# cvg/pixel-perfect-sfm

Measured on AMD Instinct MI355X. Metric: featuremetric residuals+Jacobians evaluated/sec (1M obs), higher is better.
Workload: dtype f32 horizontal / f64 vertical+normalisation on f16 patches; 1 GPU; BASELINE.json configs[2]: synthetic 200 cams / 200000 points / 1000000 obs featuremetric BA residual+Jacobian evaluation, 128-ch fp16 16x16 patches, SIMPLE_RADIAL, fused six-scalar Jacobian reduction; n_obs=1000000, channels=128, patch=16, obs_per_gpu=1000000, partition=none

## Files before the change

### include/pixsfm_hip.h

```cpp
#ifndef PIXSFM_HIP_H_
#define PIXSFM_HIP_H_

#include <stddef.h>
#include <stdint.h>

#ifdef __cplusplus
extern "C" {
#endif

#define PXR_KPAD 12
#define PXR_OBS_REC 8

enum { PXR_OK = 0, PXR_EINVAL = -1, PXR_EHIP = -2, PXR_ENOMEM = -3, PXR_EUNSUPPORTED = -4,
       PXR_ENUMERIC = -5 };
enum { PXR_F16 = 0, PXR_F32 = 1, PXR_F64 = 2, PXR_U8 = 3  };
enum { PXR_SIMPLE_PINHOLE = 0, PXR_PINHOLE = 1, PXR_SIMPLE_RADIAL = 2, PXR_RADIAL = 3,
       PXR_OPENCV = 4, PXR_OPENCV_FISHEYE = 5, PXR_FULL_OPENCV = 6, PXR_FOV = 7,
       PXR_SIMPLE_RADIAL_FISHEYE = 8, PXR_RADIAL_FISHEYE = 9, PXR_THIN_PRISM_FISHEYE = 10 };
enum { PXR_LOSS_TRIVIAL = 0, PXR_LOSS_CAUCHY = 1, PXR_LOSS_HUBER = 2, PXR_LOSS_SOFTL1 = 3 };

typedef struct pxr_ctx pxr_ctx;
typedef struct pxr_arena pxr_arena;

typedef struct {
  int32_t l2_normalize;
  int32_t use_float_simd;
  int32_t check_bounds;
} pxr_interp_cfg;

typedef struct {
  int32_t type;
  double a;
} pxr_loss;

int pxr_version(void);
const char* pxr_last_error(void);
int pxr_ctx_create(int device, void* stream, pxr_ctx** out);
int pxr_ctx_destroy(pxr_ctx* ctx);
int pxr_ctx_sync(pxr_ctx* ctx);
int pxr_malloc(pxr_ctx* ctx, size_t bytes, void** d_ptr);
int pxr_free(pxr_ctx* ctx, void* d_ptr);
int pxr_memcpy_h2d(pxr_ctx* ctx, void* d_dst, const void* h_src, size_t bytes);
int pxr_memcpy_d2h(pxr_ctx* ctx, void* h_dst, const void* d_src, size_t bytes);
int pxr_memset(pxr_ctx* ctx, void* d_dst, int value, size_t bytes);
int pxr_timer_start(pxr_ctx* ctx);
int pxr_timer_stop(pxr_ctx* ctx, double* ms);

int pxr_arena_create(pxr_ctx* ctx, int dtype, int C, int H, int W, int64_t n_patches,
                     void* d_data_or_null ,
                     pxr_arena** out);
int pxr_arena_destroy(pxr_arena* a);
int pxr_arena_upload(pxr_arena* a, int64_t first, int64_t count, const void* h_patches,
                     const int32_t* h_corners, const double* h_scales);
int pxr_arena_upload_gather(pxr_arena* a, int64_t first, int64_t count, const void* const* h_patch_ptrs,
                            const int32_t* h_corners, const double* h_scales);
int pxr_arena_extract(pxr_ctx* ctx, pxr_arena* a, int64_t first, int64_t n, const void* d_fmap,
                      int src_dtype, int h, int w, const double* d_keypoints, double image_w,
                      double image_h, int l2_normalize);
int pxr_dsift_dense(pxr_ctx* ctx, const void* d_image, int image_dtype, int h, int w, int spatial_bin_size, int rootsift,
                    double clipval, float* d_out);
int pxr_dsift_extract(pxr_ctx* ctx, pxr_arena* a, int64_t first, int64_t n, const void* d_image, int image_dtype, int h,
                      int w, int spatial_bin_size, int rootsift, double clipval, const double* d_keypoints, double image_w,
                      double image_h, int l2_normalize);
void* pxr_arena_data(pxr_arena* a);
int32_t* pxr_arena_corners(pxr_arena* a);
double* pxr_arena_scales(pxr_arena* a);
int64_t pxr_arena_size(pxr_arena* a);

typedef struct {
  int64_t n_obs;
  const int32_t* d_obs_image;
  const int32_t* d_obs_point;
  const int64_t* d_obs_patch;
  int32_t n_images;
  const int32_t* d_image_camera;
  const double* d_qvec;
  const double* d_tvec;
  int32_t n_cameras;
  const int32_t* d_cam_model;
  const double* d_cam_params;
  int64_t n_points;
  const double* d_xyz;
  const double* d_refs;
} pxr_ba_view;

int pxr_ba_eval(pxr_ctx* ctx, pxr_arena* arena, const pxr_ba_view* view,
                const pxr_interp_cfg* cfg, int with_jacobian, double* d_rec, double* d_r,
                double* d_gx, double* d_gy);

int pxr_ba_projection_jacobian(pxr_ctx* ctx, const pxr_ba_view* view, double* d_P);

int pxr_ba_cost(pxr_ctx* ctx, const double* d_rec, int64_t n_obs, const pxr_loss* loss,
                double* h_cost);


enum { PXR_TERM_CONVERGENCE = 0, PXR_TERM_NO_CONVERGENCE = 1, PXR_TERM_FAILURE = 2 };

typedef struct {
  int32_t max_iterations;
  double function_tolerance;
  double gradient_tolerance;
  double parameter_tolerance;
  double initial_radius;
  double max_radius;
  double min_radius;
  double min_relative_decrease;
  double min_lm_diagonal;
  double max_lm_diagonal;
  int32_t max_consecutive_invalid_steps;
  int32_t jacobi_scaling;
  int32_t use_inner_iterations;
  double inner_iteration_tolerance;
  int32_t linear_solver;
  int32_t max_linear_solver_iterations;
  double eta;
  double linear_r_tolerance;
} pxr_lm_options;
enum { PXR_LINEAR_AUTO = 0, PXR_LINEAR_DIRECT = 1, PXR_LINEAR_ITERATIVE = 2 };
#define PXR_MAX_IMAGES_DIRECT 1000

typedef struct {
  int32_t iterations;
  int32_t num_successful;
  int32_t termination;
  int32_t num_camera_unknowns;
  int64_t num_point_unknowns;
  double initial_cost, final_cost, final_radius;
  double total_ms;
  double setup_ms;
  int32_t linear_solver;
  int32_t collective_kib;
  int64_t linear_iterations;
  int32_t accumulation;
  int32_t initial_us;
} pxr_lm_summary;

typedef struct {
  int32_t iteration;
  int32_t step_is_valid;
  int32_t step_is_successful;
  double cost;
  double cost_change;
  double relative_decrease;
  double trust_region_radius;
  double step_norm;
} pxr_iteration_summary;
typedef int (*pxr_iteration_callback)(const pxr_iteration_summary* summary, void* user);
int pxr_set_iteration_callback(pxr_ctx* ctx, pxr_iteration_callback fn , void* user);

int pxr_set_deterministic(pxr_ctx* ctx, int on);
int pxr_get_deterministic(pxr_ctx* ctx);

int pxr_set_gram_cache(pxr_ctx* ctx, int on);
int pxr_get_gram_cache(pxr_ctx* ctx);
int pxr_ba_eval_gram(pxr_ctx* ctx, pxr_arena* arena, const pxr_ba_view* view, const pxr_interp_cfg* cfg, int reset,
                     double* d_rec, int32_t* h_rebuilt);

#define PXR_COMM_ID_BYTES 128
int pxr_comm_unique_id(void* h_id );
int pxr_comm_init(pxr_ctx* ctx, const void* h_id, int rank, int nranks);
int pxr_comm_destroy(pxr_ctx* ctx);
int pxr_comm_set_rank(pxr_ctx* ctx, int rank, int nranks);
int pxr_comm_rank(pxr_ctx* ctx, int* rank, int* nranks);
int pxr_comm_allreduce_sum(pxr_ctx* ctx, double* d_buf, int64_t count);
int pxr_comm_force(pxr_ctx* ctx, int on);
int pxr_comm_stats(pxr_ctx* ctx, int64_t* calls, int64_t* bytes, int reset);

typedef int (*pxr_allreduce_fn)(void* user, double* d_buf, int64_t count);

int pxr_ba_solve(pxr_ctx* ctx, pxr_arena* arena, const pxr_ba_view* view, const pxr_interp_cfg* cfg,
                 const pxr_loss* loss, const uint8_t* h_pose_const, const uint8_t* h_tvec_const_mask,
                 const uint16_t* h_cam_const_mask, const uint8_t* h_point_const,
                 const pxr_lm_options* options, pxr_allreduce_fn allreduce, void* allreduce_user,
                 pxr_lm_summary* summary);

int pxr_ba_geom_eval(pxr_ctx* ctx, const pxr_ba_view* view, const double* d_obs_xy, double* d_rec, double* d_res);

int pxr_ba_solve_geometric(pxr_ctx* ctx, const pxr_ba_view* view, const double* d_obs_xy, const pxr_loss* loss,
                           const uint8_t* h_pose_const, const uint8_t* h_tvec_const_mask,
                           const uint16_t* h_cam_const_mask, const uint8_t* h_point_const,
                           const pxr_lm_options* options, pxr_allreduce_fn allreduce, void* allreduce_user,
                           pxr_lm_summary* summary);

typedef struct {
  int64_t n_tracks;
  const int64_t* d_track_offsets;
  int64_t n_obs;
  const int32_t* d_obs_image;
  const double* d_obs_xy;
  int32_t n_images;
  const int32_t* d_image_camera;
  const double* d_qvec;
  const double* d_tvec;
  int32_t n_cameras;
  const int32_t* d_cam_model;
  const double* d_cam_params;
} pxr_tri_view;

typedef struct {
  double min_tri_angle;
  double max_angle_error;
  double max_reproj_error;
  int32_t min_track_len;
  int32_t max_hypotheses;
} pxr_tri_options;

int pxr_image_to_world(pxr_ctx* ctx, int64_t n, const int32_t* d_cam_index, int32_t n_cameras, const int32_t* d_cam_model,
                       const double* d_cam_params, const double* d_xy, double* d_uv, uint8_t* d_ok);

int pxr_triangulate_tracks(pxr_ctx* ctx, const pxr_tri_view* view, const pxr_tri_options* options, double* d_xyz,
                           int32_t* d_status, int32_t* d_n_inliers, uint8_t* d_obs_inlier, double* d_obs_err);
int pxr_triangulate_tracks_timed(pxr_ctx* ctx, const pxr_tri_view* view, const pxr_tri_options* options, double* d_xyz,
                                 int32_t* d_status, int32_t* d_n_inliers, uint8_t* d_obs_inlier, double* d_obs_err,
                                 double* h_kernel_ms);

int pxr_ba_compute_references(pxr_ctx* ctx, pxr_arena* arena, const pxr_ba_view* view,
                              const pxr_interp_cfg* cfg, const pxr_loss* loss, int iters,
                              double* d_refs_out, int64_t* d_ref_obs_out, double* d_robust_mean_out,
                              double* d_obs_desc_out );

int pxr_costmap_extract(pxr_ctx* ctx, pxr_arena* features, pxr_arena* costmaps, int64_t first_out, int64_t n,
                        const int64_t* d_patch, const int32_t* d_ref_index, const double* d_refs,
                        const pxr_loss* loss, int as_gradientfield, int apply_sqrt);

int pxr_costmap_extract_ex(pxr_ctx* ctx, pxr_arena* features, pxr_arena* costmaps, int64_t first_out, int64_t n,
                           const int64_t* d_patch, const int32_t* d_ref_index, const double* d_refs,
                           const pxr_loss* loss, int as_gradientfield, int apply_sqrt, const pxr_interp_cfg* cfg,
                           double upsampling_factor, int compute_cross_derivative);
int pxr_arena_set_upsampling(pxr_arena* a, double upsampling_factor);
double pxr_arena_upsampling(pxr_arena* a);

int pxr_interpolate(pxr_ctx* ctx, pxr_arena* arena, const pxr_interp_cfg* cfg, int64_t n, const double* d_kp,
                    const int64_t* d_patch, double* d_desc, double* d_J );

int pxr_nearest_references(pxr_ctx* ctx, pxr_arena* arena, const pxr_interp_cfg* cfg, int64_t n,
                           const double* d_kp, const int64_t* d_patch, const int64_t* d_cand_ptr,
                           const int64_t* d_cand_index, const double* d_cand_desc, int64_t* d_best,
                           double* d_best_dist, double* d_out_desc);

typedef struct {
  int64_t n_nodes;
  double* d_kp;
  const int64_t* d_node_patch;
  const uint8_t* d_node_const;
  int64_t n_edges;
  const int32_t* d_edge_src;
  const int32_t* d_edge_dst;
  const double* d_edge_w;
  int32_t n_problems;
  const int64_t* d_prob_node_ptr;
  const int32_t* d_prob_nodes;
  const int64_t* d_prob_edge_ptr;
  const int32_t* d_prob_edges;
  int64_t n_unary;
  const int32_t* d_unary_node;
  const double* d_unary_ref;
  const double* d_unary_w;
  const int64_t* d_prob_unary_ptr;
  const int32_t* d_prob_unary;
  const int32_t* d_prob_group;
} pxr_ka_view;

int pxr_ka_eval(pxr_ctx* ctx, pxr_arena* arena, const pxr_ka_view* view, const pxr_interp_cfg* cfg,
                const pxr_loss* loss, double* d_cost, double* d_r, double* d_J1, double* d_J2);

int pxr_ka_solve(pxr_ctx* ctx, pxr_arena* arena, const pxr_ka_view* view, const pxr_interp_cfg* cfg,
                 const pxr_loss* loss, double bound, const pxr_lm_options* options,
                 pxr_lm_summary* h_summaries, pxr_lm_summary* total);

int pxr_graph_track_labels(int64_t n_nodes, const int32_t* node_image, int64_t n_edges,
                           const int64_t* edge_src, const int64_t* edge_dst, const double* edge_sim,
                           int64_t* track_labels , int64_t* n_tracks_out );
int pxr_graph_score_labels(int64_t n_nodes, int64_t n_edges, const int64_t* edge_src,
                           const int64_t* edge_dst, const double* edge_sim, const int64_t* track_labels,
                           double* scores );
int pxr_graph_root_labels(int64_t n_nodes, const int64_t* track_labels, const double* scores,
                          uint8_t* is_root );
int pxr_graph_labels_device(pxr_ctx* ctx, int64_t n_nodes, const int32_t* d_node_image, int64_t n_edges,
                            const int64_t* d_edge_src, const int64_t* d_edge_dst, const double* d_edge_sim,
                            int64_t* d_track_labels, double* d_scores, uint8_t* d_is_root, int64_t* h_n_tracks);
int pxr_ba_build_problem(int32_t n_images, const int32_t* image_camera, const int64_t* p2d_ptr, const int64_t* p2d_point3D,
                         int32_t n_cameras, const int32_t* cam_model, int64_t n_points, const int64_t* track_ptr,
                         const int32_t* track_image, const int32_t* track_p2d, const uint8_t* has_patch,
                         const uint8_t* in_setup, const uint8_t* const_pose, const uint8_t* tvec_mask,
                         const uint8_t* variable_point, const uint8_t* constant_point, const uint8_t* constant_camera,
                         int refine_focal_length, int refine_principal_point, int refine_extra_params, int refine_extrinsics,
                         int min_track_length, int skip_missing_patches, int64_t* n_obs, int32_t* obs_image, int32_t* obs_p2d,
                         int64_t* obs_point, uint8_t* image_in_problem, uint8_t* pose_is_const, uint8_t* tvec_mask_out,
                         int32_t* camera_mask, int8_t* point_role);

int pxr_ka_build_edges(int64_t n_nodes, const int32_t* node_image, const int32_t* node_feature,
                       int64_t n_edges, const int64_t* edge_src, const int64_t* edge_dst, const double* edge_sim,
                       const int64_t* track_labels, const uint8_t* root_labels, const int64_t* nodes_in_problem,
                       int64_t n_in_problem, int weight_by_sim, int root_edges_only,
                       double root_regularize_weight, int64_t* out_src, int64_t* out_dst, double* out_w,
                       int64_t* n_out);

int pxr_dense_spd_solve(pxr_ctx* ctx, double* d_a, int n, double* d_b, int* h_info);

#ifdef __cplusplus
}
#endif
#endif
```

### pixel-perfect-sfm_amd/csrc/pxr_ba_inner.hip

```cpp
#include <hip/hip_runtime.h>

#include <cstdlib>
#include <type_traits>
#include <vector>
#include <algorithm>

#include "pxr_device.h"
#include "pxr_gram.h"
#include "pxr_interp.h"
#include "pxr_internal.h"

namespace pxr {

struct InnerArgs {
  pxr_ba_view v;
  const void* arena; const int32_t* corners; const double* scales; int H, W;
  int l2_normalize, check_bounds;
  double up;
  pxr_loss loss;
  const int64_t* pt_ptr; const int64_t* pt_obs; const int* pt_var;
  double* xyz_out;
  double* cost_before;
  double* cost_pt;
  double* gram_G;
  int2* gram_cell;
  int gram_warm;
};

template <int LPO>
__device__ __forceinline__ double rows_sum(double v) {
  if (LPO == 1) return row8_sum(v);
  if (LPO == 8) v += __shfl_xor(v, 8);
  v += __shfl_xor(v, 16);
  v += __shfl_xor(v, 32);
  return v;
}

template <int C> struct InnerShape { static constexpr int PPW = C >= 64 ? 1 : 8, MAXO = C >= 64 ? 16 : 8, WPB = 1; };

template <typename ST, int C, bool FS>
__device__ __forceinline__ void inner_points_body(const InnerArgs& a, double (*sh_obs)[InnerShape<C>::MAXO][26]) {
  static_assert(C == 128 || C == 64 || C <= 4, "one observation per row of C / 8 lanes, or per lane (cost maps)");
  constexpr int PPW = InnerShape<C>::PPW, INNER_MAXO = InnerShape<C>::MAXO, GL = 64 / PPW, WPB = InnerShape<C>::WPB;
  constexpr int LPO = C >= 64 ? C / 8 : 1, ROWS = GL / LPO, CH = C >= 64 ? 8 : C;
  const int lane = (threadIdx.x & 63) % GL, row = lane / LPO, sub = lane % LPO;
  const int slot = (threadIdx.x >> 6) * PPW + (threadIdx.x & 63) / GL;
  const int64_t p = (int64_t)blockIdx.x * WPB * PPW + slot;
  if (p >= a.v.n_points) return;
  const int64_t o0 = a.pt_ptr[p];
  const int n = (int)(a.pt_ptr[p + 1] - o0);
  if (n == 0) return;
  const bool variable = a.pt_var[p] != 0;
  double X[3] = {a.v.d_xyz[3 * p], a.v.d_xyz[3 * p + 1], a.v.d_xyz[3 * p + 2]};
  const ST* arena = reinterpret_cast<const ST*>(a.arena);
  const size_t patch_elems = (size_t)a.H * a.W * C;
  double ref[CH];
#pragma unroll
  for (int ch = 0; ch < CH; ++ch) ref[ch] = a.v.d_refs ? a.v.d_refs[(size_t)p * C + sub * CH + ch] : 0.0;

  auto rsum = [](double v) { return LPO == 16 ? row16_sum(v) : (LPO == 8 ? row8_sum(v) : v); };
  for (int oi = row; oi < n && oi < INNER_MAXO; oi += ROWS) {
    if (sub == 0) {
      double* ob = sh_obs[slot][oi];
      const int64_t i = a.pt_obs[o0 + oi];
      const int img = a.v.d_obs_image[i], cam = a.v.d_image_camera[img];
      const int64_t pi = a.v.d_obs_patch[i];
#pragma unroll
      for (int j = 0; j < 4; ++j) ob[j] = a.v.d_qvec[4 * (size_t)img + j];
#pragma unroll
      for (int j = 0; j < 3; ++j) ob[4 + j] = a.v.d_tvec[3 * (size_t)img + j];
#pragma unroll
      for (int j = 0; j < PXR_KPAD; ++j) ob[7 + j] = a.v.d_cam_params[(size_t)cam * PXR_KPAD + j];
      ob[19] = a.scales[2 * pi]; ob[20] = a.scales[2 * pi + 1];
      ob[21] = (double)a.corners[2 * pi]; ob[22] = (double)a.corners[2 * pi + 1];
      ob[23] = (double)a.v.d_cam_model[cam]; ob[24] = (double)pi;
    }
  }
  __threadfence_block();
  __builtin_amdgcn_wave_barrier();

  auto eval = [&](const double* Xc, bool with_jac, double* Hn, double* gn) -> double {
    double cost = 0.0, acc[9] = {0, 0, 0, 0, 0, 0, 0, 0, 0};
    for (int chunk = 0; chunk < n; chunk += ROWS) {
      const int oi = chunk + row;
      const bool valid = oi < n;
      const int oc = valid ? oi : n - 1;
      double q[4], t[3], k[PXR_KPAD], sx, sy, cx, cy;
      int model;
      int64_t pi;
      if (oc < INNER_MAXO) {
        const double* ob = sh_obs[slot][oc];
#pragma unroll
        for (int j = 0; j < 4; ++j) q[j] = ob[j];
#pragma unroll
        for (int j = 0; j < 3; ++j) t[j] = ob[4 + j];
#pragma unroll
        for (int j = 0; j < PXR_KPAD; ++j) k[j] = ob[7 + j];
        sx = ob[19]; sy = ob[20]; cx = ob[21]; cy = ob[22];
        model = (int)ob[23]; pi = (int64_t)ob[24];
      } else {
        const int64_t i = a.pt_obs[o0 + oc];
        const int img = a.v.d_obs_image[i], cam = a.v.d_image_camera[img];
        pi = a.v.d_obs_patch[i];
#pragma unroll
        for (int j = 0; j < 4; ++j) q[j] = a.v.d_qvec[4 * (size_t)img + j];
#pragma unroll
        for (int j = 0; j < 3; ++j) t[j] = a.v.d_tvec[3 * (size_t)img + j];
#pragma unroll
        for (int j = 0; j < PXR_KPAD; ++j) k[j] = a.v.d_cam_params[(size_t)cam * PXR_KPAD + j];
        model = a.v.d_cam_model[cam];
        sx = a.scales[2 * pi]; sy = a.scales[2 * pi + 1];
        cx = (double)a.corners[2 * pi]; cy = (double)a.corners[2 * pi + 1];
      }
      double x, y, A[2][3], Pq[2][4], PX[2][3], Pk[2][PXR_KPAD];
      world_to_pixel_jac(model, k, q, t, Xc, x, y, A, Pq, PX, Pk);
      double u = x * sx - 0.5 - cx, v = y * sy - 0.5 - cy;
      if constexpr (C < 64) { u *= a.up; v *= a.up; sx *= a.up; sy *= a.up; }
      double f[CH], fr[CH], fc[CH];
      if constexpr (C >= 64)
        interp8<ST, LPO, true, FS>(arena + (size_t)pi * patch_elems, a.H, a.W, C, sub, u, v, a.l2_normalize != 0, f, fr, fc);
      else
        interp_small<ST, C>(arena + (size_t)pi * patch_elems, a.H, a.W, u, v, a.l2_normalize != 0, f, fr, fc);
      double s = 0, gcc = 0, gcr = 0, grr = 0, bc = 0, br = 0;
#pragma unroll
      for (int ch = 0; ch < CH; ++ch) {
        const double r = f[ch] - ref[ch];
        s = fma(r, r, s);
        gcc = fma(fc[ch], fc[ch], gcc); gcr = fma(fc[ch], fr[ch], gcr); grr = fma(fr[ch], fr[ch], grr);
        bc = fma(fc[ch], r, bc); br = fma(fr[ch], r, br);
      }
      s = rsum(s);
      double rho[3];
      loss_eval(a.loss.type, a.loss.a, 1.0, s, rho);
      if (valid) cost += 0.5 * rho[0];
      if (valid && a.check_bounds && !a.v.d_refs && !(u > 0.0 && u < (double)a.W && v > 0.0 && v < (double)a.H)) cost = __builtin_nan("");
      if (with_jac) {
        gcc = rsum(gcc) * sx * sx; gcr = rsum(gcr) * sx * sy; grr = rsum(grr) * sy * sy;
        bc = rsum(bc) * sx; br = rsum(br) * sy;
        double kappa = 0.0;
        if (s != 0.0 && rho[2] > 0.0) {
          const double D = 1.0 + 2.0 * s * rho[2] / rho[1];
          const double alpha = 1.0 - sqrt(D);
          kappa = (2.0 * alpha - alpha * alpha) / s;
        }
        const double w8 = valid ? rho[1] : 0.0;
        const double m00 = w8 * (gcc - kappa * bc * bc), m01 = w8 * (gcr - kappa * bc * br), m11 = w8 * (grr - kappa * br * br);
        const double b0 = w8 * bc, b1 = w8 * br;
        double me0[3], me1[3];
#pragma unroll
        for (int j = 0; j < 3; ++j) { me0[j] = m00 * PX[0][j] + m01 * PX[1][j]; me1[j] = m01 * PX[0][j] + m11 * PX[1][j]; }
        acc[0] += PX[0][0] * me0[0] + PX[1][0] * me1[0];
        acc[1] += PX[0][0] * me0[1] + PX[1][0] * me1[1];
        acc[2] += PX[0][0] * me0[2] + PX[1][0] * me1[2];
        acc[3] += PX[0][1] * me0[1] + PX[1][1] * me1[1];
        acc[4] += PX[0][1] * me0[2] + PX[1][1] * me1[2];
        acc[5] += PX[0][2] * me0[2] + PX[1][2] * me1[2];
#pragma unroll
        for (int j = 0; j < 3; ++j) acc[6 + j] += PX[0][j] * b0 + PX[1][j] * b1;
      }
    }
    cost = rows_sum<LPO>(cost);
    if (with_jac) {
#pragma unroll
      for (int j = 0; j < 6; ++j) Hn[j] = rows_sum<LPO>(acc[j]);
#pragma unroll
      for (int j = 0; j < 3; ++j) gn[j] = rows_sum<LPO>(acc[6 + j]);
    }
    return cost;
  };

  double H[6], g[3];
  double cost = eval(X, variable, H, g);
  if (lane == 0) { if (a.cost_pt) a.cost_pt[p] = cost; else atomicAdd(a.cost_before, cost); }
  if (!variable) return;
  double gmax = fmax(fabs(g[0]), fmax(fabs(g[1]), fabs(g[2])));
  if (gmax <= 1e-10) return;
  const double sc[3] = {1.0 / (1.0 + sqrt(H[0])), 1.0 / (1.0 + sqrt(H[3])), 1.0 / (1.0 + sqrt(H[5]))};
  auto scale_sys = [&]() {
    H[0] *= sc[0] * sc[0]; H[1] *= sc[0] * sc[1]; H[2] *= sc[0] * sc[2];
    H[3] *= sc[1] * sc[1]; H[4] *= sc[1] * sc[2]; H[5] *= sc[2] * sc[2];
    g[0] *= sc[0]; g[1] *= sc[1]; g[2] *= sc[2];
  };
  scale_sys();
  double radius = 1e4, decrease_factor = 2.0, diag[3] = {0, 0, 0};
  int invalid = 0;
  bool reuse_diag = false;
  for (int it = 0; it < 50; ++it) {
    if (radius < 1e-32) break;
    if (!reuse_diag) {
      diag[0] = fmin(fmax(H[0], 1e-6), 1e32); diag[1] = fmin(fmax(H[3], 1e-6), 1e32); diag[2] = fmin(fmax(H[5], 1e-6), 1e32);
    }
    const double a00 = H[0] + diag[0] / radius, a01 = H[1], a02 = H[2], a11 = H[3] + diag[1] / radius, a12 = H[4],
                 a22 = H[5] + diag[2] / radius;
    bool ok = a00 > 0.0;
    const double l00 = sqrt(a00), l10 = a01 / l00, l20 = a02 / l00;
    const double d1 = a11 - l10 * l10;
    ok = ok && d1 > 0.0;
    const double l11 = sqrt(d1), l21 = (a12 - l20 * l10) / l11;
    const double d2 = a22 - l20 * l20 - l21 * l21;
    ok = ok && d2 > 0.0;
    const double l22 = sqrt(d2);
    const double y0 = -g[0] / l00, y1 = (-g[1] - l10 * y0) / l11, y2 = (-g[2] - l20 * y0 - l21 * y1) / l22;
    double st[3];
    st[2] = y2 / l22; st[1] = (y1 - l21 * st[2]) / l11; st[0] = (y0 - l10 * st[1] - l20 * st[2]) / l00;
    double mcc = 0.0;
    if (ok) {
      const double dg = st[0] * g[0] + st[1] * g[1] + st[2] * g[2];
      const double dHd = st[0] * (H[0] * st[0] + H[1] * st[1] + H[2] * st[2]) + st[1] * (H[1] * st[0] + H[3] * st[1] + H[4] * st[2]) +
                         st[2] * (H[2] * st[0] + H[4] * st[1] + H[5] * st[2]);
      mcc = -dg - 0.5 * dHd;
      if (!(mcc > 0.0) || !isfinite(st[0]) || !isfinite(st[1]) || !isfinite(st[2])) ok = false;
    }
    if (!ok) {
      if (++invalid >= 5) break;
      radius *= 0.5; reuse_diag = true;
      continue;
    }
    invalid = 0;
    const double Xc[3] = {X[0] + st[0] * sc[0], X[1] + st[1] * sc[1], X[2] + st[2] * sc[2]};
    double Hc[6], gc[3];
    const double cand = eval(Xc, true, Hc, gc);
    const double s2 = (Xc[0] - X[0]) * (Xc[0] - X[0]) + (Xc[1] - X[1]) * (Xc[1] - X[1]) + (Xc[2] - X[2]) * (Xc[2] - X[2]);
    const double x2 = X[0] * X[0] + X[1] * X[1] + X[2] * X[2];
    if (sqrt(s2) <= 1e-8 * (sqrt(x2) + 1e-8)) break;
    const double cost_change = cost - cand;
    if (fabs(cost_change) <= 1e-6 * cost) break;
    const double rel = cost_change / mcc;
    if (rel > 1e-3) {
      X[0] = Xc[0]; X[1] = Xc[1]; X[2] = Xc[2];
      cost = cand;
#pragma unroll
      for (int j = 0; j < 6; ++j) H[j] = Hc[j];
#pragma unroll
      for (int j = 0; j < 3; ++j) g[j] = gc[j];
      gmax = fmax(fabs(g[0]), fmax(fabs(g[1]), fabs(g[2])));
      scale_sys();
      const double tmp = 2.0 * rel - 1.0;
      radius = fmin(1e16, radius / fmax(1.0 / 3.0, 1.0 - tmp * tmp * tmp));
      decrease_factor = 2.0; reuse_diag = false;
      if (gmax <= 1e-10) break;
    } else {
      radius /= decrease_factor; decrease_factor *= 2.0; reuse_diag = true;
    }
  }
  if (lane == 0) { a.xyz_out[3 * p] = X[0]; a.xyz_out[3 * p + 1] = X[1]; a.xyz_out[3 * p + 2] = X[2]; }
}

template <typename ST, int C, bool FS>
__global__ __launch_bounds__(64 * InnerShape<C>::WPB) void k_inner_points(const InnerArgs a) {
  __shared__ double sh_obs[InnerShape<C>::WPB * InnerShape<C>::PPW][InnerShape<C>::MAXO][26];
  inner_points_body<ST, C, FS>(a, sh_obs);
}

constexpr int IP_MAXPTS = 4, IP_MAXQ = 32, IP_OBS = 30;

struct InnerOwner {
  double X[3], Xc[3], cost, H[6], g[3], sc[3], radius, decrease_factor, diag[3], mcc, r2;
  int invalid, it, reuse_diag, live;
};

template <int C, int IP_SLOTS>
struct PackedLds {
  double ref[IP_MAXPTS][C];
  double obs[IP_MAXQ][IP_OBS];
  double res[IP_SLOTS][10];
  InnerOwner own[IP_MAXPTS];
};

__device__ __forceinline__ double inner_rsqrt(double x) {
  const double y0 = __builtin_amdgcn_rsq(x);
  const double e = fma(-(x * y0), y0, 1.0);
  return fma(y0 * e, fma(e, 0.375, 0.5), y0);
}
__device__ __forceinline__ double inner_rcp(double x) {
  double y = __builtin_amdgcn_rcp(x);
  y = fma(fma(-x, y, 1.0), y, y);
  return fma(fma(-x, y, 1.0), y, y);
}

__device__ __forceinline__ double quad_sum(double v) {
  v += dpp_f64<0xB1>(v);
  v += dpp_f64<0x4E>(v);
  return v;
}

__device__ __forceinline__ void inner_loss(int type, double a, double s, double rho[3]) {
  const double b = a * a;
  const double tiny = 2.2250738585072014e-308;
  switch (type) {
    case PXR_LOSS_CAUCHY: {
      const double c = inner_rcp(b), sum = 1.0 + s * c, inv = inner_rcp(sum);
      rho[0] = b * log(sum); rho[1] = fmax(tiny, inv); rho[2] = -c * (inv * inv);
      break;
    }
    case PXR_LOSS_HUBER:
      if (s > b) {
        const double ir = inner_rsqrt(s), r = s * ir;
        rho[0] = 2.0 * a * r - b; rho[1] = fmax(tiny, a * ir); rho[2] = -rho[1] * (0.5 * ir * ir);
      } else {
        rho[0] = s; rho[1] = 1.0; rho[2] = 0.0;
      }
      break;
    case PXR_LOSS_SOFTL1: {
      const double c = inner_rcp(b), sum = 1.0 + s * c, it = inner_rsqrt(sum), tmp = sum * it;
      rho[0] = 2.0 * b * (tmp - 1.0); rho[1] = fmax(tiny, it);
      rho[2] = -(c * rho[1]) * (0.5 * it * it);
      break;
    }
    default:
      rho[0] = s; rho[1] = 1.0; rho[2] = 0.0;
  }
}

__device__ __forceinline__ void inner_owner_update(InnerOwner& S, const double cand, const double (&Hc)[6], const double (&gc)[3],
                                                   const bool first, const bool has_obs, bool& active, double* cost_before,
                                                   double* cost_slot ) {
  if (first) {
    S.cost = cand;
    if (has_obs) { if (cost_slot) *cost_slot = cand; else atomicAdd(cost_before, cand); }
    if (active) {
      const double gmax = fmax(fabs(gc[0]), fmax(fabs(gc[1]), fabs(gc[2])));
      if (gmax <= 1e-10) active = false;
      const double s0 = 1.0 / (1.0 + sqrt(Hc[0])), s1 = 1.0 / (1.0 + sqrt(Hc[3])), s2 = 1.0 / (1.0 + sqrt(Hc[5]));
      S.sc[0] = s0; S.sc[1] = s1; S.sc[2] = s2;
      S.H[0] = Hc[0] * (s0 * s0); S.H[1] = Hc[1] * (s0 * s1); S.H[2] = Hc[2] * (s0 * s2);
      S.H[3] = Hc[3] * (s1 * s1); S.H[4] = Hc[4] * (s1 * s2); S.H[5] = Hc[5] * (s2 * s2);
      S.g[0] = gc[0] * s0; S.g[1] = gc[1] * s1; S.g[2] = gc[2] * s2;
    }
  } else if (active) {
// ... 313 lines not shown
struct GramPoint { int p, len; int64_t o0; };
struct GramSlot { int img, cam; int64_t patch; int64_t obs; };
__host__ __device__ inline size_t gram_entry_bytes(int maxo) { return sizeof(GramPoint) + sizeof(GramSlot) * (size_t)maxo; }
__global__ __launch_bounds__(256) void k_gram_table(int64_t n_list, int maxo, const GramPoint* __restrict__ pt_list, const int64_t* __restrict__ pt_obs,
                                                    const int32_t* __restrict__ obs_image, const int64_t* __restrict__ obs_patch,
                                                    const int32_t* __restrict__ image_camera, char* __restrict__ table) {
  const int64_t t = (int64_t)blockIdx.x * blockDim.x + threadIdx.x;
  const int64_t e = t / (maxo + 1);
  const int q = (int)(t % (maxo + 1)) - 1;
  if (e >= n_list) return;
  const GramPoint gp = pt_list[e];
  char* ent = table + (size_t)e * gram_entry_bytes(maxo);
  if (q < 0) { *reinterpret_cast<GramPoint*>(ent) = gp; return; }
  const int64_t i = pt_obs[gp.o0 + min(q, gp.len - 1)];
  const int img = obs_image[i];
  reinterpret_cast<GramSlot*>(ent + sizeof(GramPoint))[q] = GramSlot{img, image_camera[img], obs_patch[i], i};
}

__host__ __device__ inline size_t gram_lds_doubles(int maxo, int C) {
  return (size_t)maxo * (IG_GSTRIDE + 16 + IG_OBS) + C + (sizeof(InnerOwner) + 7) / 8;
}

template <typename ST, int C>
__global__ __launch_bounds__(64) __attribute__((amdgpu_waves_per_eu(PXR_GRAM_WAVES, PXR_GRAM_WAVES))) void k_inner_gram(const InnerArgs a, const char* __restrict__ table, const int maxo) {
  static_assert(C == 128 || C == 64, "feature patches");
  extern __shared__ __align__(16) double gsh[];
  double* const Gs = gsh;
  double* const Ds = Gs + (size_t)maxo * IG_GSTRIDE;
  double* const obs = Ds + (size_t)maxo * 16;
  double* const refd = obs + (size_t)maxo * IG_OBS;
  InnerOwner& S = *reinterpret_cast<InnerOwner*>(refd + C);
  const int lane = threadIdx.x;
#ifdef PXR_INNER_PROFILE
  long long gq_t = __builtin_amdgcn_s_memtime(), gq_acc[8] = {0, 0, 0, 0, 0, 0, 0, 0};
  int gq_rounds = 0, gq_builds = 0;
#define GQ_MARK(k) do { const long long n_ = __builtin_amdgcn_s_memtime(); gq_acc[k] += n_ - gq_t; gq_t = n_; } while (0)
#else
#define GQ_MARK(k) do { } while (0)
#endif
  const char* const ent = table + (size_t)blockIdx.x * gram_entry_bytes(maxo);
  const GramSlot* const slots = reinterpret_cast<const GramSlot*>(ent + sizeof(GramPoint));
  const GramPoint gp = *reinterpret_cast<const GramPoint*>(ent);
  const int64_t p = gp.p;
  const int L = gp.len;
  const bool variable = a.pt_var[p] != 0;
  bool active = variable, first = true;
  const ST* arena = reinterpret_cast<const ST*>(a.arena);
  const size_t patch_elems = (size_t)a.H * a.W * C;
  const bool l2 = a.l2_normalize != 0;

  const int sq = lane >> 2, part = lane & 3;
  const GramSlot sl = slots[min(sq, maxo - 1)];
  double refv[C / 64];
#pragma unroll
  for (int j = 0; j < C / 64; ++j) refv[j] = a.v.d_refs ? a.v.d_refs[(size_t)p * C + lane + 64 * j] : 0.0;
  const bool warm = a.gram_G != nullptr && a.gram_warm != 0;
  const int hi = lane < 24 ? lane : 23;
  double2 va0, va1, va2, va3, va4, va5, va6, va7, vb0, vb1, vb2, vb3, vb4, vb5, vb6, vb7;
#define IG_FETCH(Q0, J, VA, VB)                                                                                             \
  {                                                                                                                         \
    const int64_t oi = __shfl((int)sl.obs, 4 * min(Q0 + J, L - 1));                    \
    const double2* g = reinterpret_cast<const double2*>(a.gram_G + (size_t)oi * (IG_GDOUBLES + 16));                         \
    VA = g[lane]; VB = g[64 + hi];                                                                                          \
  }
#define IG_PUT(Q0, J, VA, VB)                                                                                               \
  if (Q0 + J < L) {                                                                                                         \
    double2* Gd = reinterpret_cast<double2*>(Gs + (size_t)(Q0 + J) * IG_GSTRIDE);                                           \
    Gd[lane] = VA;                                                                               \
    if (lane < 16) Gd[64 + lane] = VB;                                                                      \
    else if (lane < 24) reinterpret_cast<double2*>(Ds + (size_t)(Q0 + J) * 16)[lane - 16] = VB;                      \
  }
#define IG_FETCH8(Q0) IG_FETCH(Q0, 0, va0, vb0) IG_FETCH(Q0, 1, va1, vb1) IG_FETCH(Q0, 2, va2, vb2) IG_FETCH(Q0, 3, va3, vb3) \
                      IG_FETCH(Q0, 4, va4, vb4) IG_FETCH(Q0, 5, va5, vb5) IG_FETCH(Q0, 6, va6, vb6) IG_FETCH(Q0, 7, va7, vb7)
#define IG_PUT8(Q0) IG_PUT(Q0, 0, va0, vb0) IG_PUT(Q0, 1, va1, vb1) IG_PUT(Q0, 2, va2, vb2) IG_PUT(Q0, 3, va3, vb3) \
                    IG_PUT(Q0, 4, va4, vb4) IG_PUT(Q0, 5, va5, vb5) IG_PUT(Q0, 6, va6, vb6) IG_PUT(Q0, 7, va7, vb7)
  if (warm) { IG_FETCH8(0) }
  if (sq < L) {
    double* ob = obs + (size_t)sq * IG_OBS;
    const int img = sl.img, cam = sl.cam;
    const int64_t pi = sl.patch;
    if (part == 0) {
      double R[9];
      quat_to_rotation(a.v.d_qvec + 4 * (size_t)img, R);
#pragma unroll
      for (int m = 0; m < 9; ++m) ob[m] = R[m];
#pragma unroll
      for (int m = 0; m < 3; ++m) ob[9 + m] = a.v.d_tvec[3 * (size_t)img + m];
    } else if (part == 1) {
#pragma unroll
      for (int m = 0; m < 6; ++m) ob[12 + m] = a.v.d_cam_params[(size_t)cam * PXR_KPAD + m];
    } else if (part == 2) {
#pragma unroll
      for (int m = 6; m < PXR_KPAD; ++m) ob[12 + m] = a.v.d_cam_params[(size_t)cam * PXR_KPAD + m];
    } else {
      ob[24] = a.scales[2 * pi]; ob[25] = a.scales[2 * pi + 1];
      ob[26] = (double)a.corners[2 * pi]; ob[27] = (double)a.corners[2 * pi + 1];
      ob[28] = (double)a.v.d_cam_model[cam]; ob[29] = (double)pi;
      int2 cc = make_int2(-1000000, -1000000);
      if (warm) cc = a.gram_cell[sl.obs];
      ob[30] = (double)cc.x; ob[31] = (double)cc.y;
    }
  }
#pragma unroll
  for (int j = 0; j < C / 64; ++j) refd[lane + 64 * j] = refv[j];
  if (warm) {
    IG_PUT8(0)
#pragma unroll 1
    for (int q0 = 8; q0 < L; q0 += 8) { IG_FETCH8(q0) IG_PUT8(q0) }
  }
#undef IG_FETCH
#undef IG_PUT
#undef IG_FETCH8
#undef IG_PUT8
  if (lane == 0) {
#pragma unroll
    for (int m = 0; m < 3; ++m) { S.X[m] = a.v.d_xyz[3 * p + m]; S.Xc[m] = S.X[m]; }
    S.live = 1; S.radius = 1e4; S.decrease_factor = 2.0; S.invalid = 0; S.it = 0; S.reuse_diag = 0; S.mcc = 0.0;
  }
  __syncthreads();
  {
    double r2 = 0.0;
    for (int ch = lane; ch < C; ch += 64) r2 = fma(refd[ch], refd[ch], r2);
    r2 = rows_sum<16>(row16_sum(r2));
    if (lane == 0) S.r2 = r2;
  }

  const int sidx = lane >> 3, sub = lane & 7, ri = sub >> 1, ci = 2 * (sub & 1);
  GQ_MARK(0);

  while (true) {
    __syncthreads();
    double rs[10] = {0, 0, 0, 0, 0, 0, 0, 0, 0, 0};
#pragma unroll 1
    for (int k = 0; 8 * k < L; ++k) {
      const int q = 8 * k + sidx;
      const bool act = q < L;
      double* ob = obs + (size_t)(act ? q : L - 1) * IG_OBS;
      double R[9];
#pragma unroll
      for (int m = 0; m < 9; ++m) R[m] = ob[m];
      const double sx = ob[24], sy = ob[25], cx = ob[26], cy = ob[27];
      const int model = (int)ob[28];
      const double X0 = S.Xc[0], X1 = S.Xc[1], X2 = S.Xc[2];
      const double p0 = fma(R[0], X0, fma(R[1], X1, fma(R[2], X2, ob[9])));
      const double p1 = fma(R[3], X0, fma(R[4], X1, fma(R[5], X2, ob[10])));
      const double p2 = fma(R[6], X0, fma(R[7], X1, fma(R[8], X2, ob[11])));
      const double iz = inner_rcp(p2), un = p0 * iz, vn = p1 * iz;
      double x, y, Juv[2][2];
      camera_model_jac<false, false>(model, ob + 12, un, vn, x, y, Juv, nullptr);
      double PX[2][3];
#pragma unroll
      for (int r = 0; r < 2; ++r) {
        const double A0 = Juv[r][0] * iz, A1 = Juv[r][1] * iz, A2 = -(Juv[r][0] * un + Juv[r][1] * vn) * iz;
#pragma unroll
        for (int m = 0; m < 3; ++m) PX[r][m] = A0 * R[m] + A1 * R[3 + m] + A2 * R[6 + m];
      }
      const double u = x * sx - 0.5 - cx, v = y * sy - 0.5 - cy;
      const double rf = floor(v), cf = floor(u);
      const int row = texel_index(rf, a.H), col = texel_index(cf, a.W);
      const bool need = act && ((double)row != ob[30] || (double)col != ob[31]);
      unsigned long long todo = __ballot(need);
      GQ_MARK(1);
      if (todo != 0ull) {
        const int64_t pi = (int64_t)ob[29];
        const int pi_lo = (int)(pi & 0xffffffffll), pi_hi = (int)(pi >> 32);
        auto request = [&](GramTexels<ST, C>& tx, int src_lane) {
          const int row_t = __builtin_amdgcn_readlane(row, src_lane), col_t = __builtin_amdgcn_readlane(col, src_lane);
          const int64_t pi_t = ((int64_t)__builtin_amdgcn_readlane(pi_hi, src_lane) << 32) | (unsigned)__builtin_amdgcn_readlane(pi_lo, src_lane);
          tx.load(arena + (size_t)pi_t * patch_elems, a.H, a.W, row_t, col_t);
        };
        auto take = [&](GramTexels<ST, C>& tx) -> int {
          if (todo == 0ull) return -1;
          const int src = __ffsll((long long)todo) - 1;
          todo &= ~(0xffull << (src & ~7));
          request(tx, src);
          return src;
        };
        GramTexels<ST, C> t0, t1, t2;
        int s0 = take(t0), s1 = take(t1), s2 = take(t2);
        while (true) {
          if (s0 < 0) break;
          gram_contract<ST, C>(t0, refd, Gs + (size_t)(8 * k + (s0 >> 3)) * IG_GSTRIDE, Ds + (size_t)(8 * k + (s0 >> 3)) * 16);
          s0 = take(t0);
          if (s1 < 0) break;
          gram_contract<ST, C>(t1, refd, Gs + (size_t)(8 * k + (s1 >> 3)) * IG_GSTRIDE, Ds + (size_t)(8 * k + (s1 >> 3)) * 16);
          s1 = take(t1);
          if (s2 < 0) break;
          gram_contract<ST, C>(t2, refd, Gs + (size_t)(8 * k + (s2 >> 3)) * IG_GSTRIDE, Ds + (size_t)(8 * k + (s2 >> 3)) * 16);
          s2 = take(t2);
        }
        if (need && sub == 0) { ob[30] = (double)row; ob[31] = (double)col; }
        __syncthreads();
        if (a.gram_G) {
          unsigned long long wb = __ballot(need);
          while (wb != 0ull) {
            const int src = __ffsll((long long)wb) - 1;
            wb &= ~(0xffull << (src & ~7));
            const int slot = 8 * k + (src >> 3);
            const int64_t oi = slots[slot].obs;
            double2* g = reinterpret_cast<double2*>(a.gram_G + (size_t)oi * (IG_GDOUBLES + 16));
            const double2* Gd = reinterpret_cast<const double2*>(Gs + (size_t)slot * IG_GSTRIDE);
            g[lane] = Gd[lane];
            if (lane < 16) g[64 + lane] = Gd[64 + lane];
            else if (lane < 24) g[64 + lane] = reinterpret_cast<const double2*>(Ds + (size_t)slot * 16)[lane - 16];
            const int2 cl = make_int2(__builtin_amdgcn_readlane(row, src), __builtin_amdgcn_readlane(col, src));
            if (lane == 0) a.gram_cell[oi] = cl;
          }
        }
#ifdef PXR_INNER_PROFILE
        gq_builds += __popcll(__ballot(need)) / 8;
#endif
        GQ_MARK(2);
      }
      if (act) {
        double wu[4], dwu[4], wv[4], dwv[4];
        catmull_rom_weights(u - cf, wu, dwu);
        catmull_rom_weights(v - rf, wv, dwv);
        double ya[3], yb[3];
        gram_rows_times_weights(Gs + (size_t)q * IG_GSTRIDE, sub, wu, dwu, wv, dwv, ya, yb);
        const double2 d2 = *reinterpret_cast<const double2*>(Ds + (size_t)q * 16 + 2 * sub);
        const double wvo = pick4(wv, ri), dwvo = pick4(dwv, ri);
        const double wua = ci == 0 ? wu[0] : wu[2], wub = ci == 0 ? wu[1] : wu[3];
        const double dwua = ci == 0 ? dwu[0] : dwu[2], dwub = ci == 0 ? dwu[1] : dwu[3];
        const double oma = wvo * wua, omb = wvo * wub, omca = wvo * dwua, omcb = wvo * dwub, omra = dwvo * wua, omrb = dwvo * wub;
        const double Sgg = row8_sum(fma(oma, ya[0], omb * yb[0])), Sgc = row8_sum(fma(oma, ya[1], omb * yb[1]));
        const double Sgr = row8_sum(fma(oma, ya[2], omb * yb[2]));
        const double Scc = row8_sum(fma(omca, ya[1], omcb * yb[1])), Scr = row8_sum(fma(omca, ya[2], omcb * yb[2]));
        const double Srr = row8_sum(fma(omra, ya[2], omrb * yb[2]));
        const double Sfd = row8_sum(fma(oma, d2.x, omb * d2.y)), Scd = row8_sum(fma(omca, d2.x, omcb * d2.y));
        const double Srd = row8_sum(fma(omra, d2.x, omrb * d2.y));
        double s, gcc, gcr, grr, bc, br;
        if (l2) {
          const double ninv = inner_rsqrt(Sgg), n2inv = ninv * ninv;
          const double pc = Sgc * n2inv, pr = Sgr * n2inv;
          s = fmax(0.0, 1.0 - 2.0 * Sfd * ninv + S.r2);
          gcc = (Scc - Sgc * pc) * n2inv; gcr = (Scr - Sgc * pr) * n2inv; grr = (Srr - Sgr * pr) * n2inv;
          bc = -(Scd - Sfd * pc) * ninv; br = -(Srd - Sfd * pr) * ninv;
        } else {
          s = fmax(0.0, Sgg - 2.0 * Sfd + S.r2);
          gcc = Scc; gcr = Scr; grr = Srr; bc = Sgc - Scd; br = Sgr - Srd;
        }
        double rho[3];
        inner_loss(a.loss.type, a.loss.a, s, rho);
        double cq = 0.5 * rho[0];
        if (a.check_bounds && !a.v.d_refs && !(u > 0.0 && u < (double)a.W && v > 0.0 && v < (double)a.H)) cq = __builtin_nan("");
        gcc *= sx * sx; gcr *= sx * sy; grr *= sy * sy; bc *= sx; br *= sy;
        double kappa = 0.0;
        if (s != 0.0 && rho[2] > 0.0) {
          const double D = 1.0 + 2.0 * s * rho[2] * inner_rcp(rho[1]);
          const double alpha = 1.0 - sqrt(D);
          kappa = (2.0 * alpha - alpha * alpha) * inner_rcp(s);
        }
        const double w8 = rho[1];
        const double m00 = w8 * (gcc - kappa * bc * bc), m01 = w8 * (gcr - kappa * bc * br), m11 = w8 * (grr - kappa * br * br);
        const double b0 = w8 * bc, b1 = w8 * br;
        double me0[3], me1[3];
#pragma unroll
        for (int m = 0; m < 3; ++m) { me0[m] = m00 * PX[0][m] + m01 * PX[1][m]; me1[m] = m01 * PX[0][m] + m11 * PX[1][m]; }
        if (sub == 0) {
          rs[0] += cq;
          rs[1] += PX[0][0] * me0[0] + PX[1][0] * me1[0];
          rs[2] += PX[0][0] * me0[1] + PX[1][0] * me1[1];
          rs[3] += PX[0][0] * me0[2] + PX[1][0] * me1[2];
          rs[4] += PX[0][1] * me0[1] + PX[1][1] * me1[1];
          rs[5] += PX[0][1] * me0[2] + PX[1][1] * me1[2];
          rs[6] += PX[0][2] * me0[2] + PX[1][2] * me1[2];
#pragma unroll
          for (int m = 0; m < 3; ++m) rs[7 + m] += PX[0][m] * b0 + PX[1][m] * b1;
        }
      }
    }
    GQ_MARK(3);
#pragma unroll
    for (int m = 0; m < 10; ++m) {
      rs[m] += __shfl_xor(rs[m], 8); rs[m] += __shfl_xor(rs[m], 16); rs[m] += __shfl_xor(rs[m], 32);
    }
    GQ_MARK(4);
    if (lane == 0) {
      const double Hc[6] = {rs[1], rs[2], rs[3], rs[4], rs[5], rs[6]}, gc[3] = {rs[7], rs[8], rs[9]};
      inner_owner_update(S, rs[0], Hc, gc, first, true, active, a.cost_before, a.cost_pt ? a.cost_pt + p : nullptr);
    }
    first = false;
    GQ_MARK(5);
#ifdef PXR_INNER_PROFILE
    ++gq_rounds;
#endif
    if (__builtin_amdgcn_readfirstlane((int)active) == 0) break;
  }
#ifdef PXR_INNER_PROFILE
  if ((blockIdx.x == 1000 || blockIdx.x == 150000) && lane == 0)
    printf("[inner gram profile, wavefront %d, 100 MHz ticks x 10 ns] rounds %d builds %d  staging %lld  projection %lld  gram builds %lld  evaluation %lld  reduce %lld  owner LM %lld\n",
           (int)blockIdx.x, gq_rounds, gq_builds, gq_acc[0], gq_acc[1], gq_acc[2], gq_acc[3], gq_acc[4], gq_acc[5]);
#endif
  if (variable && lane == 0) { a.xyz_out[3 * p] = S.X[0]; a.xyz_out[3 * p + 1] = S.X[1]; a.xyz_out[3 * p + 2] = S.X[2]; }
}

struct GramWave { int npts, pad; int p[IP_MAXPTS]; int st[IP_MAXPTS + 1]; int pad2; };
static_assert(sizeof(GramWave) == 48, "table layout");
constexpr int GW_SLOTS = 16;
__host__ __device__ inline size_t gram_wave_bytes() { return sizeof(GramWave) + sizeof(GramSlot) * GW_SLOTS; }
#ifndef PXR_GW_GPAD
#define PXR_GW_GPAD 4
#endif
struct GramWaveLds {
  double G[GW_SLOTS][IG_GDOUBLES + PXR_GW_GPAD];
  double D[GW_SLOTS][16];
  double obs[GW_SLOTS][IG_OBS];
  double res[GW_SLOTS][10];
  double refbuf[128];
  InnerOwner own[IP_MAXPTS];
};

__global__ __launch_bounds__(256) void k_gram_wave_table(int64_t n_waves, const GramWave* __restrict__ waves, const int64_t* __restrict__ pt_ptr,
                                                         const int64_t* __restrict__ pt_obs, const int32_t* __restrict__ obs_image,
                                                         const int64_t* __restrict__ obs_patch, const int32_t* __restrict__ image_camera,
                                                         char* __restrict__ table) {
  const int64_t t = (int64_t)blockIdx.x * blockDim.x + threadIdx.x;
  const int64_t e = t / (GW_SLOTS + 1);
  const int q = (int)(t % (GW_SLOTS + 1)) - 1;
  if (e >= n_waves) return;
  const GramWave w = waves[e];
  char* ent = table + (size_t)e * gram_wave_bytes();
  if (q < 0) { *reinterpret_cast<GramWave*>(ent) = w; return; }
  const int L = w.st[w.npts];
  const int qc = min(q, L - 1);
  int j = 0;
  while (j + 1 < w.npts && qc >= w.st[j + 1]) ++j;
  const int64_t i = pt_obs[pt_ptr[w.p[j]] + (qc - w.st[j])];
  const int img = obs_image[i];
  reinterpret_cast<GramSlot*>(ent + sizeof(GramWave))[q] = GramSlot{img, image_camera[img], obs_patch[i], i};
}

__global__ __launch_bounds__(256) void k_gram_flag_slots(const InnerArgs a, const char* __restrict__ table, int64_t n_waves, int* __restrict__ dirty) {
  const int64_t t = (int64_t)blockIdx.x * blockDim.x + threadIdx.x;
  const int64_t e = t / GW_SLOTS;
  const int q = (int)(t % GW_SLOTS);
  if (e >= n_waves) return;
  const char* ent = table + (size_t)e * gram_wave_bytes();
  const GramWave* gw = reinterpret_cast<const GramWave*>(ent);
  const int npts = gw->npts, L = gw->st[npts];
  if (q >= L) return;
  int j = 0;
  while (j + 1 < npts && q >= gw->st[j + 1]) ++j;
  const int64_t p = gw->p[j];
  const GramSlot sl = reinterpret_cast<const GramSlot*>(ent + sizeof(GramWave))[q];
  double qv[4], tv[3], X[3], k[PXR_KPAD];
#pragma unroll
  for (int m = 0; m < 4; ++m) qv[m] = a.v.d_qvec[4 * (size_t)sl.img + m];
#pragma unroll
  for (int m = 0; m < 3; ++m) { tv[m] = a.v.d_tvec[3 * (size_t)sl.img + m]; X[m] = a.v.d_xyz[3 * (size_t)p + m]; }
#pragma unroll
  for (int m = 0; m < PXR_KPAD; ++m) k[m] = a.v.d_cam_params[(size_t)sl.cam * PXR_KPAD + m];
  double R[9];
  quat_to_rotation(qv, R);
  const double p0 = fma(R[0], X[0], fma(R[1], X[1], fma(R[2], X[2], tv[0])));
  const double p1 = fma(R[3], X[0], fma(R[4], X[1], fma(R[5], X[2], tv[1])));
  const double p2 = fma(R[6], X[0], fma(R[7], X[1], fma(R[8], X[2], tv[2])));
  const double iz = inner_rcp(p2), un = p0 * iz, vn = p1 * iz;
  double x, y, Juv[2][2];
  camera_model_jac<false, false>(a.v.d_cam_model[sl.cam], k, un, vn, x, y, Juv, nullptr);
  const double u = x * a.scales[2 * sl.patch] - 0.5 - (double)a.corners[2 * sl.patch];
  const double v = y * a.scales[2 * sl.patch + 1] - 0.5 - (double)a.corners[2 * sl.patch + 1];
  const int row = texel_index(floor(v), a.H), col = texel_index(floor(u), a.W);
  const int2 c = a.gram_cell[sl.obs];
  const bool miss = c.x != row || c.y != col;
  dirty[sl.obs] = miss ? 1 : 0;
  if (miss) a.gram_cell[sl.obs] = make_int2(row, col);
}

template <typename ST, int C>
__global__ __launch_bounds__(64) __attribute__((amdgpu_waves_per_eu(2, 2))) void k_inner_gram_packed(const InnerArgs a, const char* __restrict__ table) {
  static_assert(C == 128 || C == 64, "feature patches");
  __shared__ __align__(16) GramWaveLds lds;
  const int lane = threadIdx.x, sidx = lane >> 2, sub = lane & 3;
  const char* const ent = table + (size_t)blockIdx.x * gram_wave_bytes();
  const GramWave* const gw = reinterpret_cast<const GramWave*>(ent);
  const GramSlot* const slots = reinterpret_cast<const GramSlot*>(ent + sizeof(GramWave));
  const GramSlot sl = slots[sidx];
  const int npts = gw->npts, L = gw->st[npts];
  const int st1 = gw->st[1 < npts ? 1 : npts], st2 = gw->st[2 < npts ? 2 : npts], st3 = gw->st[3 < npts ? 3 : npts];
  const bool owner = lane < npts;
  const int64_t myp = gw->p[owner ? lane : 0];
  const int my_b = owner ? gw->st[lane] : 0, my_e = owner ? gw->st[lane + 1] : 0;
  const bool variable = owner && a.pt_var[myp] != 0;
  bool active = variable, first = true;
  const ST* arena = reinterpret_cast<const ST*>(a.arena);
  const size_t patch_elems = (size_t)a.H * a.W * C;
  const bool l2 = a.l2_normalize != 0;
  const bool warm = a.gram_G != nullptr && a.gram_warm != 0;
  const int q = sidx;
  const bool valid = q < L;
  const int jq = ((valid ? q : L - 1) >= st1) + ((valid ? q : L - 1) >= st2) + ((valid ? q : L - 1) >= st3);

  const int hi = lane < 24 ? lane : 23;
  double2 va0, va1, va2, va3, va4, va5, va6, va7, vb0, vb1, vb2, vb3, vb4, vb5, vb6, vb7;
#define GW_FETCH(Q0, J, VA, VB)                                                                                       \
  {                                                                                                                   \
    const int64_t oi = __shfl((int)sl.obs, 4 * min(Q0 + J, L - 1));              \
    const double2* g = reinterpret_cast<const double2*>(a.gram_G + (size_t)oi * (IG_GDOUBLES + 16));                   \
    VA = g[lane]; VB = g[64 + hi];                                                                                    \
  }
#define GW_PUT(Q0, J, VA, VB)                                                                                         \
  if (Q0 + J < L) {                                                                                                   \
    double2* Gd = reinterpret_cast<double2*>(lds.G[Q0 + J]);                                                          \
    Gd[lane] = VA;                                                                                                    \
    if (lane < 16) Gd[64 + lane] = VB;                                                                                \
    else if (lane < 24) reinterpret_cast<double2*>(lds.D[Q0 + J])[lane - 16] = VB;                                    \
  }
#define GW_FETCH8(Q0) GW_FETCH(Q0, 0, va0, vb0) GW_FETCH(Q0, 1, va1, vb1) GW_FETCH(Q0, 2, va2, vb2) GW_FETCH(Q0, 3, va3, vb3) \
                      GW_FETCH(Q0, 4, va4, vb4) GW_FETCH(Q0, 5, va5, vb5) GW_FETCH(Q0, 6, va6, vb6) GW_FETCH(Q0, 7, va7, vb7)
#define GW_PUT8(Q0) GW_PUT(Q0, 0, va0, vb0) GW_PUT(Q0, 1, va1, vb1) GW_PUT(Q0, 2, va2, vb2) GW_PUT(Q0, 3, va3, vb3) \
                    GW_PUT(Q0, 4, va4, vb4) GW_PUT(Q0, 5, va5, vb5) GW_PUT(Q0, 6, va6, vb6) GW_PUT(Q0, 7, va7, vb7)
  if (warm) { GW_FETCH8(0) }
  if (valid) {
    double* ob = lds.obs[q];
    const int img = sl.img, cam = sl.cam;
    const int64_t pi = sl.patch;
    if (sub == 0) {
      double R[9];
      quat_to_rotation(a.v.d_qvec + 4 * (size_t)img, R);
#pragma unroll
      for (int m = 0; m < 9; ++m) ob[m] = R[m];
#pragma unroll
      for (int m = 0; m < 3; ++m) ob[9 + m] = a.v.d_tvec[3 * (size_t)img + m];
    } else if (sub == 1) {
#pragma unroll
      for (int m = 0; m < 6; ++m) ob[12 + m] = a.v.d_cam_params[(size_t)cam * PXR_KPAD + m];
    } else if (sub == 2) {
#pragma unroll
      for (int m = 6; m < PXR_KPAD; ++m) ob[12 + m] = a.v.d_cam_params[(size_t)cam * PXR_KPAD + m];
    } else {
      ob[24] = a.scales[2 * pi]; ob[25] = a.scales[2 * pi + 1];
      ob[26] = (double)a.corners[2 * pi]; ob[27] = (double)a.corners[2 * pi + 1];
      ob[28] = (double)a.v.d_cam_model[cam]; ob[29] = (double)pi;
      int2 cc = make_int2(-1000000, -1000000);
      if (warm) cc = a.gram_cell[sl.obs];
      ob[30] = (double)cc.x; ob[31] = (double)cc.y;
    }
  }
  for (int j = 0; j < npts; ++j) {
    double r2 = 0.0;
    if (a.v.d_refs)
      for (int ch = lane; ch < C; ch += 64) { const double d = a.v.d_refs[(size_t)gw->p[j] * C + ch]; r2 = fma(d, d, r2); }
    r2 = rows_sum<16>(row16_sum(r2));
    if (lane == 0) lds.own[j].r2 = r2;
  }
  if (owner) {
    InnerOwner& S = lds.own[lane];
#pragma unroll
    for (int m = 0; m < 3; ++m) { S.X[m] = a.v.d_xyz[3 * myp + m]; S.Xc[m] = S.X[m]; }
    S.live = 1; S.radius = 1e4; S.decrease_factor = 2.0; S.invalid = 0; S.it = 0; S.reuse_diag = 0; S.mcc = 0.0;
  }
  if (warm) {
    GW_PUT8(0)
    if (L > 8) { GW_FETCH8(8) GW_PUT8(8) }
  }
#undef GW_FETCH
#undef GW_PUT
#undef GW_FETCH8
#undef GW_PUT8

  while (true) {
    __syncthreads();
    const bool act = valid && lds.own[jq].live != 0;
    double* ob = lds.obs[valid ? q : L - 1];
    double PX[2][3], u = 0.0, v = 0.0, rf = 0.0, cf = 0.0, sx = 1.0, sy = 1.0;
    int row = 0, col = 0;
    if (act) {
      double R[9];
#pragma unroll
      for (int m = 0; m < 9; ++m) R[m] = ob[m];
      sx = ob[24]; sy = ob[25];
      const double cx = ob[26], cy = ob[27];
      const int model = (int)ob[28];
      const double X0 = lds.own[jq].Xc[0], X1 = lds.own[jq].Xc[1], X2 = lds.own[jq].Xc[2];
      const double p0 = fma(R[0], X0, fma(R[1], X1, fma(R[2], X2, ob[9])));
      const double p1 = fma(R[3], X0, fma(R[4], X1, fma(R[5], X2, ob[10])));
      const double p2 = fma(R[6], X0, fma(R[7], X1, fma(R[8], X2, ob[11])));
      const double iz = inner_rcp(p2), un = p0 * iz, vn = p1 * iz;
      double x, y, Juv[2][2];
      camera_model_jac<false, false>(model, ob + 12, un, vn, x, y, Juv, nullptr);
#pragma unroll
      for (int r = 0; r < 2; ++r) {
        const double A0 = Juv[r][0] * iz, A1 = Juv[r][1] * iz, A2 = -(Juv[r][0] * un + Juv[r][1] * vn) * iz;
#pragma unroll
        for (int m = 0; m < 3; ++m) PX[r][m] = A0 * R[m] + A1 * R[3 + m] + A2 * R[6 + m];
      }
      u = x * sx - 0.5 - cx; v = y * sy - 0.5 - cy;
      rf = floor(v); cf = floor(u);
      row = texel_index(rf, a.H); col = texel_index(cf, a.W);
    }
    const bool need = act && ((double)row != ob[30] || (double)col != ob[31]);
    unsigned long long todo = __ballot(need);
    if (todo != 0ull) {
      const int64_t pi = (int64_t)ob[29];
      const int pi_lo = (int)(pi & 0xffffffffll), pi_hi = (int)(pi >> 32);
      const int pt_of_slot = gw->p[jq];
      const unsigned long long rebuilt = todo;
      double2 rr0 = make_double2(0.0, 0.0), rr1 = rr0, rr2 = rr0;
      auto take = [&](GramTexels<ST, C>& tx, double2& rr) -> int {
        if (todo == 0ull) return -1;
        const int src = __ffsll((long long)todo) - 1;
        todo &= ~(0xfull << (src & ~3));
        const int row_t = __builtin_amdgcn_readlane(row, src), col_t = __builtin_amdgcn_readlane(col, src);
        const int64_t pi_t = ((int64_t)__builtin_amdgcn_readlane(pi_hi, src) << 32) | (unsigned)__builtin_amdgcn_readlane(pi_lo, src);
        const int pt_t = __builtin_amdgcn_readlane(pt_of_slot, src);
        tx.load(arena + (size_t)pi_t * patch_elems, a.H, a.W, row_t, col_t);
        if (a.v.d_refs && 2 * lane < C) rr = *reinterpret_cast<const double2*>(a.v.d_refs + (size_t)pt_t * C + 2 * lane);
        return src;
      };
      auto build = [&](const GramTexels<ST, C>& tx, const double2& rr, int src) {
        __syncthreads();
        if (2 * lane < C) *reinterpret_cast<double2*>(&lds.refbuf[2 * lane]) = rr;
        __syncthreads();
        gram_contract<ST, C>(tx, lds.refbuf, lds.G[src >> 2], lds.D[src >> 2]);
      };
      GramTexels<ST, C> t0, t1, t2;
      int s0 = take(t0, rr0), s1 = take(t1, rr1), s2 = take(t2, rr2);
      while (true) {
        if (s0 < 0) break;
        build(t0, rr0, s0); s0 = take(t0, rr0);
        if (s1 < 0) break;
        build(t1, rr1, s1); s1 = take(t1, rr1);
        if (s2 < 0) break;
        build(t2, rr2, s2); s2 = take(t2, rr2);
      }
      if (need && sub == 0) { ob[30] = (double)row; ob[31] = (double)col; }
      __syncthreads();
      if (a.gram_G) {
        unsigned long long wb = rebuilt;
        while (wb != 0ull) {
          const int src = __ffsll((long long)wb) - 1;
          wb &= ~(0xfull << (src & ~3));
          const int slot = src >> 2;
          const int64_t oi = slots[slot].obs;
          double2* g = reinterpret_cast<double2*>(a.gram_G + (size_t)oi * (IG_GDOUBLES + 16));
          const double2* Gd = reinterpret_cast<const double2*>(lds.G[slot]);
          g[lane] = Gd[lane];
          if (lane < 16) g[64 + lane] = Gd[64 + lane];
          else if (lane < 24) g[64 + lane] = reinterpret_cast<const double2*>(lds.D[slot])[lane - 16];
          const int2 cl = make_int2(__builtin_amdgcn_readlane(row, src), __builtin_amdgcn_readlane(col, src));
          if (lane == 0) a.gram_cell[oi] = cl;
        }
      }
    }
    if (act) {
      double wu[4], dwu[4], wv[4], dwv[4];
      catmull_rom_weights(u - cf, wu, dwu);
      catmull_rom_weights(v - rf, wv, dwv);
      const int R = sub;
      const double wvR = pick4(wv, R), dwvR = pick4(dwv, R);
      double Sgg = 0, Sgc = 0, Sgr = 0, Scc = 0, Scr = 0, Srr = 0;
      const double* Gq = lds.G[q];
#pragma unroll
      for (int cb = 0; cb < 4; ++cb) {
        const bool T = cb < R;
        const double* blk = Gq + (T ? gram_block(cb, R) : gram_block(R, cb)) * 16;
        double e[16];
#pragma unroll
        for (int m = 0; m < 8; ++m) { const double2 t2 = *reinterpret_cast<const double2*>(blk + 2 * m); e[2 * m] = t2.x; e[2 * m + 1] = t2.y; }
        double zw[4], zd[4];
#pragma unroll
        for (int c = 0; c < 4; ++c) {
          zw[c] = fma(wu[3], e[12 + c], fma(wu[2], e[8 + c], fma(wu[1], e[4 + c], wu[0] * e[c])));
          zd[c] = fma(dwu[3], e[12 + c], fma(dwu[2], e[8 + c], fma(dwu[1], e[4 + c], dwu[0] * e[c])));
        }
        const double Bww = fma(zw[3], wu[3], fma(zw[2], wu[2], fma(zw[1], wu[1], zw[0] * wu[0])));
        const double Bwd_s = fma(zw[3], dwu[3], fma(zw[2], dwu[2], fma(zw[1], dwu[1], zw[0] * dwu[0])));
        const double Bdw_s = fma(zd[3], wu[3], fma(zd[2], wu[2], fma(zd[1], wu[1], zd[0] * wu[0])));
        const double Bdd = fma(zd[3], dwu[3], fma(zd[2], dwu[2], fma(zd[1], dwu[1], zd[0] * dwu[0])));
        const double Bwd = T ? Bdw_s : Bwd_s, Bdw = T ? Bwd_s : Bdw_s;
        const double wvC = wv[cb], dwvC = dwv[cb];
        Sgg = fma(wvR * wvC, Bww, Sgg);
        Sgc = fma(wvR * wvC, Bwd, Sgc);
        Sgr = fma(wvR * dwvC, Bww, Sgr);
        Scc = fma(wvR * wvC, Bdd, Scc);
        Scr = fma(wvR * dwvC, Bdw, Scr);
        Srr = fma(dwvR * dwvC, Bww, Srr);
      }
      const double* Dq = lds.D[q] + 4 * R;
      const double2 d01 = *reinterpret_cast<const double2*>(Dq), d23 = *reinterpret_cast<const double2*>(Dq + 2);
      const double dw = fma(wu[3], d23.y, fma(wu[2], d23.x, fma(wu[1], d01.y, wu[0] * d01.x)));
      const double dd = fma(dwu[3], d23.y, fma(dwu[2], d23.x, fma(dwu[1], d01.y, dwu[0] * d01.x)));
      double Sfd = wvR * dw, Scd = wvR * dd, Srd = dwvR * dw;
      Sgg = quad_sum(Sgg); Sgc = quad_sum(Sgc); Sgr = quad_sum(Sgr);
      Scc = quad_sum(Scc); Scr = quad_sum(Scr); Srr = quad_sum(Srr);
      Sfd = quad_sum(Sfd); Scd = quad_sum(Scd); Srd = quad_sum(Srd);
      double s, gcc, gcr, grr, bc, br;
      if (l2) {
        const double ninv = inner_rsqrt(Sgg), n2inv = ninv * ninv;
        const double pc = Sgc * n2inv, pr = Sgr * n2inv;
        s = fmax(0.0, 1.0 - 2.0 * Sfd * ninv + lds.own[jq].r2);
        gcc = (Scc - Sgc * pc) * n2inv; gcr = (Scr - Sgc * pr) * n2inv; grr = (Srr - Sgr * pr) * n2inv;
        bc = -(Scd - Sfd * pc) * ninv; br = -(Srd - Sfd * pr) * ninv;
      } else {
        s = fmax(0.0, Sgg - 2.0 * Sfd + lds.own[jq].r2);
        gcc = Scc; gcr = Scr; grr = Srr; bc = Sgc - Scd; br = Sgr - Srd;
      }
      double rho[3];
      inner_loss(a.loss.type, a.loss.a, s, rho);
      double cq = 0.5 * rho[0];
      if (a.check_bounds && !a.v.d_refs && !(u > 0.0 && u < (double)a.W && v > 0.0 && v < (double)a.H)) cq = __builtin_nan("");
      gcc *= sx * sx; gcr *= sx * sy; grr *= sy * sy; bc *= sx; br *= sy;
      double kappa = 0.0;
      if (s != 0.0 && rho[2] > 0.0) {
        const double Dc = 1.0 + 2.0 * s * rho[2] * inner_rcp(rho[1]);
        const double alpha = 1.0 - sqrt(Dc);
        kappa = (2.0 * alpha - alpha * alpha) * inner_rcp(s);
      }
      const double w8 = rho[1];
      const double m00 = w8 * (gcc - kappa * bc * bc), m01 = w8 * (gcr - kappa * bc * br), m11 = w8 * (grr - kappa * br * br);
      const double b0 = w8 * bc, b1 = w8 * br;
      double me0[3], me1[3];
#pragma unroll
      for (int m = 0; m < 3; ++m) { me0[m] = m00 * PX[0][m] + m01 * PX[1][m]; me1[m] = m01 * PX[0][m] + m11 * PX[1][m]; }
      if (sub == 0) {
        double* rs = lds.res[q];
        rs[0] = cq;
        rs[1] = PX[0][0] * me0[0] + PX[1][0] * me1[0];
        rs[2] = PX[0][0] * me0[1] + PX[1][0] * me1[1];
        rs[3] = PX[0][0] * me0[2] + PX[1][0] * me1[2];
        rs[4] = PX[0][1] * me0[1] + PX[1][1] * me1[1];
        rs[5] = PX[0][1] * me0[2] + PX[1][1] * me1[2];
        rs[6] = PX[0][2] * me0[2] + PX[1][2] * me1[2];
#pragma unroll
        for (int m = 0; m < 3; ++m) rs[7 + m] = PX[0][m] * b0 + PX[1][m] * b1;
      }
    }
    __syncthreads();
    double cand = 0.0, Hc[6] = {0, 0, 0, 0, 0, 0}, gc[3] = {0, 0, 0};
    if (owner && lds.own[lane].live != 0) {
      for (int slq = my_b; slq < my_e; ++slq) {
        const double* rs = lds.res[slq];
        cand += rs[0];
#pragma unroll
        for (int m = 0; m < 6; ++m) Hc[m] += rs[1 + m];
#pragma unroll
        for (int m = 0; m < 3; ++m) gc[m] += rs[7 + m];
      }
    }
    if (owner) inner_owner_update(lds.own[lane], cand, Hc, gc, first, my_e > my_b, active, a.cost_before, a.cost_pt ? a.cost_pt + myp : nullptr);
    first = false;
    if (__ballot(active) == 0) break;
  }
  if (variable) {
    const InnerOwner& S = lds.own[lane];
    a.xyz_out[3 * myp] = S.X[0]; a.xyz_out[3 * myp + 1] = S.X[1]; a.xyz_out[3 * myp + 2] = S.X[2];
  }
}

int launch_inner_iterations(pxr_ctx* ctx, pxr_arena* arena, const pxr_ba_view* view, const pxr_interp_cfg* cfg,
                            const pxr_loss* loss, const int64_t* d_pt_ptr, const int64_t* d_pt_obs,
                            const int* d_pt_var, double* d_cost_before, const InnerLists* lists, double* d_cost_per_point,
                            const GramCache* gram, bool gram_warm) {
  if (arena->C != 128 && arena->C != 64 && arena->C != 3 && arena->C != 1)
    return set_error(PXR_EUNSUPPORTED, "inner iterations: CHANNELS=%d not supported (128, 64; cost maps: 3, 1)", arena->C);
  InnerArgs a;
  a.v = *view;
  a.arena = arena->d_data; a.corners = arena->d_corners; a.scales = arena->d_scales;
  a.H = arena->H; a.W = arena->W; a.up = arena->up; a.l2_normalize = cfg->l2_normalize; a.check_bounds = cfg->check_bounds; a.loss = *loss;
  a.pt_ptr = d_pt_ptr; a.pt_obs = d_pt_obs; a.pt_var = d_pt_var;
  a.xyz_out = const_cast<double*>(view->d_xyz); a.cost_before = d_cost_before; a.cost_pt = d_cost_per_point;
  a.gram_G = gram ? gram->G : nullptr; a.gram_cell = gram ? static_cast<int2*>(gram->cell) : nullptr; a.gram_warm = gram_warm ? 1 : 0;
  const int ppb = arena->C >= 64 ? 1 : 8;
  const int threads = 64;
  const unsigned blocks = (unsigned)((view->n_points + ppb - 1) / ppb);
  if (blocks == 0) return PXR_OK;
#define INNER_LAUNCH(KERNEL, ST, CC)                                                                          \
  do {                                                                                                        \
    if (cfg->use_float_simd) hipLaunchKernelGGL((KERNEL<ST, CC, true>), dim3(blocks), dim3(threads), 0, ctx->stream, a);  \
    else hipLaunchKernelGGL((KERNEL<ST, CC, false>), dim3(blocks), dim3(threads), 0, ctx->stream, a);             \
  } while (0)
#define INNER_PACKED(ST, CC, NBLK, PPW, LIST)                                                                             \
  do {                                                                                                                    \
    if (cfg->use_float_simd) hipLaunchKernelGGL((k_inner_packed<ST, CC, true, 4>), dim3(NBLK), dim3(64), 0, ctx->stream, a, PPW, LIST);  \
    else hipLaunchKernelGGL((k_inner_packed<ST, CC, false, 4>), dim3(NBLK), dim3(64), 0, ctx->stream, a, PPW, LIST);         \
  } while (0)
#define INNER_BY_STORAGE(MACRO, ...)                                                    \
  do {                                                                                  \
    if (arena->dtype == PXR_F16 && arena->C == 128) MACRO(_Float16, 128, __VA_ARGS__);  \
    else if (arena->dtype == PXR_F16) MACRO(_Float16, 64, __VA_ARGS__);                 \
    else if (arena->C == 128) MACRO(float, 128, __VA_ARGS__);                           \
    else MACRO(float, 64, __VA_ARGS__);                                                 \
  } while (0)
#define INNER_GRAM(ST, CC, NBLK, MAXO)                                                                                    \
  hipLaunchKernelGGL((k_inner_gram<ST, CC>), dim3(NBLK), dim3(64), sizeof(double) * gram_lds_doubles(MAXO, CC), ctx->stream, a, \
                     static_cast<const char*>(lists->d_slots), MAXO)
#define INNER_GRAM_PACKED(ST, CC, NBLK) \
  hipLaunchKernelGGL((k_inner_gram_packed<ST, CC>), dim3(NBLK), dim3(64), 0, ctx->stream, a, static_cast<const char*>(lists->d_waves))
  if (arena->C <= 4) {
    if (arena->dtype == PXR_F16 && arena->C == 3) INNER_LAUNCH(k_inner_points, _Float16, 3);
    else if (arena->dtype == PXR_F16) INNER_LAUNCH(k_inner_points, _Float16, 1);
    else if (arena->dtype == PXR_F32 && arena->C == 3) INNER_LAUNCH(k_inner_points, float, 3);
    else if (arena->dtype == PXR_F32) INNER_LAUNCH(k_inner_points, float, 1);
    else if (arena->C == 3) INNER_LAUNCH(k_inner_points, double, 3);
    else INNER_LAUNCH(k_inner_points, double, 1);
  } else if (getenv("PXR_INNER_OLD")) {
    if (arena->dtype == PXR_F16 && arena->C == 128) INNER_LAUNCH(k_inner_points, _Float16, 128);
    else if (arena->dtype == PXR_F16) INNER_LAUNCH(k_inner_points, _Float16, 64);
    else if (arena->dtype == PXR_F32 && arena->C == 128) INNER_LAUNCH(k_inner_points, float, 128);
    else if (arena->dtype == PXR_F32) INNER_LAUNCH(k_inner_points, float, 64);
    else if (arena->C == 128) INNER_LAUNCH(k_inner_points, double, 128);
    else INNER_LAUNCH(k_inner_points, double, 64);
  } else if (arena->dtype != PXR_F64) {
    if (lists == nullptr || getenv("PXR_INNER_PACKED")) {
      const int64_t per16 = view->n_obs > 0 ? (16 * view->n_points) / view->n_obs : 1;
      const int ppw = (int)(per16 < 1 ? 1 : (per16 > IP_MAXPTS ? IP_MAXPTS : per16));
      const unsigned pblocks = (unsigned)((view->n_points + ppw - 1) / ppw);
      const int* no_list = nullptr;
      INNER_BY_STORAGE(INNER_PACKED, pblocks, ppw, no_list);
    } else {
      if (lists->n_waves > 0) {
        if (gram && !getenv("PXR_INNER_NO_PREBUILD")) {
          PXR_HIP(hipMemsetAsync(gram->list, 0, sizeof(int) * (size_t)view->n_obs, ctx->stream));
          const int64_t n_thr = lists->n_waves * GW_SLOTS;
          hipLaunchKernelGGL(k_gram_flag_slots, dim3((unsigned)((n_thr + 255) / 256)), dim3(256), 0, ctx->stream, a, static_cast<const char*>(lists->d_waves),
                             lists->n_waves, gram->list);
          if (int rc = gram_build_flagged(ctx, arena, view, *gram)) return rc;
          a.gram_warm = 1;
        }
        INNER_BY_STORAGE(INNER_GRAM_PACKED, (unsigned)lists->n_waves);
      }
      else if (lists->n_short > 0 && lists->d_slots) INNER_BY_STORAGE(INNER_GRAM, (unsigned)lists->n_short, lists->maxo_short);
      if (lists->n_long > 0) INNER_BY_STORAGE(INNER_PACKED, (unsigned)lists->n_long, 1, lists->d_long);
    }
  } else if (arena->dtype == PXR_F64 && arena->C == 128) INNER_LAUNCH(k_inner_points, double, 128);
  else INNER_LAUNCH(k_inner_points, double, 64);
#undef INNER_LAUNCH
#undef INNER_PACKED
#undef INNER_GRAM
#undef INNER_GRAM_PACKED
#undef INNER_BY_STORAGE
  return hip_check(hipGetLastError(), "k_inner_points launch");
}

size_t inner_wave_stage_bytes(int64_t n_pts) { return sizeof(GramWave) * (size_t)(n_pts + 1); }
int make_inner_lists(pxr_ctx* ctx, const int64_t* pt_ptr, int64_t n, void* h_wave_stage, size_t wave_stage_bytes, const pxr_ba_view* view,
                     const int64_t* d_pt_ptr, const int64_t* d_pt_obs, InnerLists* out) {
  hipStream_t st = ctx->stream;
  const bool one_point_kernel = getenv("PXR_INNER_GRAM1") != nullptr;
  std::vector<GramPoint> shorts;
  std::vector<GramWave> waves_pageable;
  GramWave* wv = wave_stage_bytes >= inner_wave_stage_bytes(n) ? static_cast<GramWave*>(h_wave_stage) : nullptr;
  int64_t n_wv = 0;
  std::vector<int> longs;
  int maxo = 1;
  const int max_pts = getenv("PXR_INNER_GRAM_PPW") ? std::max(1, std::min(IP_MAXPTS, atoi(getenv("PXR_INNER_GRAM_PPW")))) : IP_MAXPTS;
  if (one_point_kernel) shorts.reserve((size_t)n); else if (!wv) waves_pageable.reserve((size_t)n / 2 + 1);
  int64_t n_short = 0;
  GramWave cur{};
  auto flush = [&]() {
    if (cur.npts > 0) { if (wv) wv[n_wv] = cur; else waves_pageable.push_back(cur); ++n_wv; }
    cur = GramWave{};
  };
  for (int64_t p = 0; p < n; ++p) {
    const int64_t len = pt_ptr[p + 1] - pt_ptr[p];
    if (len <= 0) continue;
    if (len <= IG_MAXO) {
      ++n_short; maxo = std::max(maxo, (int)len);
      if (one_point_kernel) { shorts.push_back(GramPoint{(int)p, (int)len, pt_ptr[p]}); continue; }
      if (cur.npts == max_pts || cur.st[cur.npts] + (int)len > GW_SLOTS) flush();
      cur.p[cur.npts] = (int)p;
      cur.st[cur.npts + 1] = cur.st[cur.npts] + (int)len;
      ++cur.npts;
    } else longs.push_back((int)p);
  }
  flush();
  const GramWave* const waves = wv ? wv : waves_pageable.data();
  out->n_waves = n_wv; out->d_waves = nullptr; out->d_wave_heads = nullptr;
  out->n_short = n_short; out->n_long = (int64_t)longs.size(); out->maxo_short = maxo;
  out->d_short = nullptr; out->d_long = nullptr; out->d_slots = nullptr;
  if (!shorts.empty()) {
    out->d_short = solve_scratch(sizeof(GramPoint) * shorts.size(), &out->own_short);
    if (!out->d_short) return set_error(PXR_ENOMEM, "hipMalloc(inner lists)");
    if (int rc = hip_check(hipMemcpyAsync(out->d_short, shorts.data(), sizeof(GramPoint) * shorts.size(), hipMemcpyHostToDevice, st), "H2D")) return rc;
    out->d_slots = solve_scratch(gram_entry_bytes(maxo) * shorts.size(), &out->own_slots);
    if (!out->d_slots) return set_error(PXR_ENOMEM, "hipMalloc(inner table)");
    const int64_t n_thr = (int64_t)shorts.size() * (maxo + 1);
    hipLaunchKernelGGL(k_gram_table, dim3((unsigned)((n_thr + 255) / 256)), dim3(256), 0, st, (int64_t)shorts.size(), maxo,
                       static_cast<const GramPoint*>(out->d_short), d_pt_obs, view->d_obs_image, view->d_obs_patch, view->d_image_camera,
                       static_cast<char*>(out->d_slots));
  }
  if (n_wv > 0) {
    const size_t heads = (sizeof(GramWave) * (size_t)n_wv + 255) & ~(size_t)255;
    char* d_all = static_cast<char*>(solve_scratch(heads + gram_wave_bytes() * (size_t)n_wv, &out->own_heads));
    if (!d_all) return set_error(PXR_ENOMEM, "hipMalloc(inner wave table)");
    out->d_wave_heads = d_all; out->d_waves = d_all + heads;
    if (int rc = hip_check(hipMemcpyAsync(d_all, waves, sizeof(GramWave) * (size_t)n_wv, hipMemcpyHostToDevice, st), "H2D")) return rc;
    const int64_t n_thr2 = n_wv * (GW_SLOTS + 1);
    hipLaunchKernelGGL(k_gram_wave_table, dim3((unsigned)((n_thr2 + 255) / 256)), dim3(256), 0, st, n_wv,
                       reinterpret_cast<const GramWave*>(d_all), d_pt_ptr, d_pt_obs, view->d_obs_image, view->d_obs_patch, view->d_image_camera,
                       static_cast<char*>(out->d_waves));
  }
  if (!longs.empty()) {
    out->d_long = static_cast<int*>(solve_scratch(sizeof(int) * longs.size(), &out->own_long));
    if (!out->d_long) return set_error(PXR_ENOMEM, "hipMalloc(inner lists)");
    if (int rc = hip_check(hipMemcpyAsync(out->d_long, longs.data(), sizeof(int) * longs.size(), hipMemcpyHostToDevice, st), "H2D")) return rc;
  }
  return hip_check(hipStreamSynchronize(st), "inner lists upload");
}
void free_inner_lists(InnerLists* l) {
  if (l->d_short && l->own_short) (void)hipFree(l->d_short);
  if (l->d_long && l->own_long) (void)hipFree(l->d_long);
  if (l->d_slots && l->own_slots) (void)hipFree(l->d_slots);
  if (l->d_wave_heads && l->own_heads) (void)hipFree(l->d_wave_heads);
  l->d_short = nullptr; l->d_long = nullptr; l->d_slots = nullptr; l->d_waves = nullptr; l->d_wave_heads = nullptr;
}

}
```

### pixel-perfect-sfm_amd/csrc/pxr_ba_solve.hip

```cpp
#include <hip/hip_runtime.h>

#include <algorithm>
#include <chrono>
#include <cmath>
#include <cstdlib>
#include <cstring>
#include <limits>
#include <thread>
#include <vector>

#include "pxr_ba_pcg.h"
#include "pxr_ba_solve.h"
#include "pxr_device.h"
#include "pxr_internal.h"

namespace pxr {


constexpr int JAC_THREADS = 128;

__global__ __launch_bounds__(JAC_THREADS) void k_jac(const SolveDev d, const double* __restrict__ rec,
                                                     pxr_loss loss, double* __restrict__ L, double* __restrict__ W) {
  extern __shared__ double jstage[];
  const int lane = threadIdx.x & 63, wave = threadIdx.x >> 6;
// ... 635 lines not shown
    for (int j = 0; j < 3; ++j) { const double d = X1[3 * p + j] - X0[3 * p + j]; s += d * d; }
  if (limb_slot) { Limbs l; l.add(s); limbs_block_add(l, limb_slot, lsh); return; }
  s = wave_sum(s);
  if ((threadIdx.x & 63) == 0 && s != 0.0) atomicAdd(out, s);
}

__global__ void k_normalize_q(int n, double* __restrict__ q) {
  const int i = blockIdx.x * blockDim.x + threadIdx.x;
  if (i >= n) return;
  const double nn = sqrt(q[4 * i] * q[4 * i] + q[4 * i + 1] * q[4 * i + 1] + q[4 * i + 2] * q[4 * i + 2] + q[4 * i + 3] * q[4 * i + 3]);
  for (int j = 0; j < 4; ++j) q[4 * i + j] /= nn;
}

__global__ void k_count_above(int64_t n, const double* __restrict__ g, const double* __restrict__ scale, double tol,
                              double* __restrict__ out, long long* __restrict__ limb_slot) {
  const int64_t i = (int64_t)blockIdx.x * blockDim.x + threadIdx.x;
  double v = (i < n && !(fabs(g[i] / scale[i]) <= tol)) ? 1.0 : 0.0;
  v = wave_sum(v);
  if ((threadIdx.x & 63) == 0 && v != 0.0) {
    if (limb_slot) atomicAdd(reinterpret_cast<unsigned long long*>(limb_slot + 1), (unsigned long long)((long long)v << 20));
    else atomicAdd(out, v);
  }
}

__device__ __forceinline__ int64_t packed_row_offset(int n, int r) { return (int64_t)r * (n + 1) - (int64_t)r * (r - 1) / 2; }
__global__ __launch_bounds__(256) void k_pack_upper(int n, const double* __restrict__ S, double* __restrict__ packed) {
  const int r = blockIdx.x, len = n - r + 1;
  const double* src = S + (size_t)r * (n + 1) + r;
  double* dst = packed + packed_row_offset(n, r);
  for (int x = threadIdx.x; x < len; x += blockDim.x) dst[x] = src[x];
}
__global__ __launch_bounds__(256) void k_unpack_upper(int n, const double* __restrict__ packed, double* __restrict__ S) {
  const int r = blockIdx.x, len = n - r + 1;
  double* dst = S + (size_t)r * (n + 1) + r;
  const double* src = packed + packed_row_offset(n, r);
  for (int x = threadIdx.x; x < len; x += blockDim.x) dst[x] = src[x];
}

__global__ __launch_bounds__(256) void k_cost_limbs(const double* __restrict__ rec, int64_t n, pxr_loss loss, long long* __restrict__ slot) {
  __shared__ long long lsh[PXR_LIMBS * 4];
  Limbs l;
  for (int64_t i = (int64_t)blockIdx.x * 256 + threadIdx.x; i < n; i += (int64_t)gridDim.x * 256) {
    double rho[3];
    loss_eval(loss.type, loss.a, 1.0, rec[i * PXR_OBS_REC], rho);
    l.add(0.5 * rho[0]);
  }
  limbs_block_add(l, slot, lsh);
}
__global__ __launch_bounds__(256) void k_limb_accumulate(const double* __restrict__ x, int64_t n, long long* __restrict__ slot) {
  __shared__ long long lsh[PXR_LIMBS * 4];
  Limbs l;
  for (int64_t i = (int64_t)blockIdx.x * 256 + threadIdx.x; i < n; i += (int64_t)gridDim.x * 256) l.add(x[i]);
  limbs_block_add(l, slot, lsh);
}
__global__ void k_limbs_finish(const long long* __restrict__ limb, unsigned mask, double* __restrict__ scal) {
  const int i = threadIdx.x;
  if (i < 16 && ((mask >> i) & 1u)) scal[i] = limb_value(limb + i * PXR_LIMBS);
}
__global__ __launch_bounds__(1024) void k_diag_and_trace(int n, const double* __restrict__ U, double* __restrict__ diag,
                                                          const double* __restrict__ chunk_trace, int n_chunks, long long* __restrict__ trace_out) {
  __shared__ double sh[1024];
  for (int i = threadIdx.x; i < n; i += 1024) diag[i] = U[(size_t)i * n + i];
  double acc = 0.0;
  for (int i = threadIdx.x; i < n_chunks; i += 1024) acc += chunk_trace[i];
  sh[threadIdx.x] = acc;
  __syncthreads();
  for (int off = 512; off > 0; off >>= 1) {
    if ((int)threadIdx.x < off) sh[threadIdx.x] += sh[threadIdx.x + off];
    __syncthreads();
  }
  if (threadIdx.x == 0) {
    Limbs l; l.add(sh[0]);
    for (int k = 0; k < PXR_LIMBS; ++k) trace_out[k] = l.q[k];
  }
}
__global__ __launch_bounds__(1024) void k_finish_and_stats(int n, int n_slots, double* __restrict__ gcd, double det_scale,
                                                            const long long* __restrict__ trace_limbs, double* __restrict__ out4) {
  __shared__ double smax[1024], ssum[1024], smin[1024];
  double mx = 0.0, sm = 0.0, mn = 0.0;
  for (int i = threadIdx.x; i < n_slots; i += 1024) {
    const double v = accum_value(gcd[i], det_scale);
    gcd[i] = v;
    if (i < n) { mx = fmax(mx, v); mn = fmin(mn, v); sm += v; }
  }
  smax[threadIdx.x] = mx; ssum[threadIdx.x] = sm; smin[threadIdx.x] = mn;
  __syncthreads();
  for (int off = 512; off > 0; off >>= 1) {
    if ((int)threadIdx.x < off) {
      smax[threadIdx.x] = fmax(smax[threadIdx.x], smax[threadIdx.x + off]);
      smin[threadIdx.x] = fmin(smin[threadIdx.x], smin[threadIdx.x + off]);
      ssum[threadIdx.x] += ssum[threadIdx.x + off];
    }
    __syncthreads();
  }
  if (threadIdx.x == 0) { out4[0] = smax[0]; out4[1] = ssum[0]; out4[2] = smin[0]; out4[3] = limb_value(trace_limbs); }
}
__global__ void k_i64_split(int64_t n, const long long* __restrict__ in, double* __restrict__ out) {
  const int64_t i = (int64_t)blockIdx.x * blockDim.x + threadIdx.x;
  if (i >= n) return;
  const long long v = in[i];
  out[2 * i] = (double)(int)(v >> 32);
  out[2 * i + 1] = (double)(unsigned)(v & 0xffffffffll);
}
__global__ void k_i64_join(int64_t n, const double* __restrict__ in, long long* __restrict__ out) {
  const int64_t i = (int64_t)blockIdx.x * blockDim.x + threadIdx.x;
  if (i >= n) return;
  const unsigned long long hi = (unsigned long long)(long long)in[2 * i], lo = (unsigned long long)(long long)in[2 * i + 1];
  out[i] = (long long)((hi << 32) + lo);
}

__global__ void k_zero(int64_t n, double* __restrict__ x) {
  const int64_t i = (int64_t)blockIdx.x * blockDim.x + threadIdx.x;
  if (i < n) x[i] = 0.0;
}

__global__ __launch_bounds__(256) void k_build_descriptors(int64_t n_obs, const int32_t* __restrict__ obs_image,
                                                           const int32_t* __restrict__ obs_point,
                                                           const int32_t* __restrict__ image_camera,
                                                           const int64_t* __restrict__ pt_obs, const int64_t* __restrict__ img_obs,
                                                           const int64_t* __restrict__ pt_ptr, const int* __restrict__ pt_var,
                                                           const int* __restrict__ pose_off, const int* __restrict__ pose_dim,
                                                           const int* __restrict__ intr_off, const int* __restrict__ intr_dim,
                                                           int4* __restrict__ obs_cols, int* __restrict__ part_obs,
                                                           int4* __restrict__ so) {
  const int64_t o = (int64_t)blockIdx.x * blockDim.x + threadIdx.x;
  if (o >= n_obs) return;
  const int64_t j = pt_obs[o];
  const int im = obs_image[j], cm = image_camera[im];
  obs_cols[o] = make_int4(pose_off[im], pose_dim[im], intr_off[cm], intr_dim[cm]);
  part_obs[o] = (int)j;
  const int64_t i = img_obs[o];
  const int64_t pt = obs_point[i];
  so[o] = make_int4((int)i, (int)pt, (int)pt_ptr[pt], pt_var[pt] ? (int)(pt_ptr[pt + 1] - pt_ptr[pt]) : 0);
}

constexpr int COUNT_CHUNK = 4096;
__global__ __launch_bounds__(256) void k_count_indices(int64_t n_obs, const int32_t* __restrict__ obs_image,
                                                       const int32_t* __restrict__ obs_point, int n_img, int64_t n_pts,
                                                       unsigned long long* __restrict__ img_cnt, unsigned long long* __restrict__ pt_cnt,
                                                       int* __restrict__ flags) {
  extern __shared__ unsigned int sh_img[];
  for (int k = threadIdx.x; k < n_img; k += 256) sh_img[k] = 0u;
  __syncthreads();
  const int64_t i0 = (int64_t)blockIdx.x * COUNT_CHUNK, i1 = min(n_obs, i0 + COUNT_CHUNK);
  for (int64_t i = i0 + threadIdx.x; i < i1; i += 256) {
    const int im = obs_image[i], pt = obs_point[i];
    if (im < 0 || im >= n_img || pt < 0 || pt >= n_pts) { atomicOr(&flags[0], 1); continue; }
    atomicAdd(&sh_img[im], 1u);
    atomicAdd(&pt_cnt[pt + 1], 1ull);
    if (i > 0 && obs_point[i - 1] > pt) atomicOr(&flags[1], 1);
  }
  __syncthreads();
  for (int k = threadIdx.x; k < n_img; k += 256)
    if (sh_img[k]) atomicAdd(&img_cnt[k + 1], (unsigned long long)sh_img[k]);
}
constexpr int PT_SCAN_CHUNK = 2048;
__device__ __forceinline__ unsigned long long block_sum_256(unsigned long long v, unsigned long long* sh) {
  const int t = threadIdx.x;
  sh[t] = v;
  __syncthreads();
  for (int o = 128; o > 0; o >>= 1) { if (t < o) sh[t] += sh[t + o]; __syncthreads(); }
  const unsigned long long r = sh[0];
  __syncthreads();
  return r;
}
__global__ __launch_bounds__(256) void k_pt_scan_partials(int64_t n_pts, const unsigned long long* __restrict__ cnt, unsigned long long* __restrict__ part) {
  __shared__ unsigned long long sh[256];
  const int64_t p0 = (int64_t)blockIdx.x * PT_SCAN_CHUNK;
  unsigned long long s = 0;
  for (int j = threadIdx.x; j < PT_SCAN_CHUNK; j += 256) if (p0 + j < n_pts) s += cnt[p0 + j + 1];
  s = block_sum_256(s, sh);
  if (threadIdx.x == 0) part[blockIdx.x] = s;
}
__global__ __launch_bounds__(256) void k_pt_scan_apply(int64_t n_pts, const unsigned long long* __restrict__ cnt, const unsigned long long* __restrict__ part,
                                                       const uint8_t* __restrict__ pt_const, int64_t* __restrict__ pt_ptr, int* __restrict__ pt_var,
                                                       unsigned long long* __restrict__ n_var) {
  __shared__ unsigned long long sh[256];
  constexpr int PER = PT_SCAN_CHUNK / 256;
  const int t = threadIdx.x;
  unsigned long long base = 0;
  for (int g = t; g < (int)blockIdx.x; g += 256) base += part[g];
  base = block_sum_256(base, sh);
  const int64_t p0 = (int64_t)blockIdx.x * PT_SCAN_CHUNK + (int64_t)t * PER;
  unsigned long long c[PER], mine = 0;
  int nv = 0;
#pragma unroll
  for (int j = 0; j < PER; ++j) {
    c[j] = p0 + j < n_pts ? cnt[p0 + j + 1] : 0ull;
    mine += c[j];
  }
  sh[t] = mine;
  __syncthreads();
  for (int o = 1; o < 256; o <<= 1) {
    const unsigned long long add = t >= o ? sh[t - o] : 0ull;
    __syncthreads();
    sh[t] += add;
    __syncthreads();
  }
  unsigned long long run = base + sh[t] - mine;
#pragma unroll
  for (int j = 0; j < PER; ++j) {
    if (p0 + j >= n_pts) break;
    run += c[j];
    pt_ptr[p0 + j + 1] = (int64_t)run;
    const int v = (!pt_const[p0 + j] && c[j] > 0) ? 1 : 0;
    pt_var[p0 + j] = v; nv += v;
  }
  if (blockIdx.x == 0 && t == 0) pt_ptr[0] = 0;
  __syncthreads();
  const unsigned long long tot = block_sum_256((unsigned long long)nv, sh);
  if (t == 0 && tot) atomicAdd(n_var, tot);
}
__global__ void k_iota(int64_t n, int64_t* __restrict__ out) {
  const int64_t i = (int64_t)blockIdx.x * blockDim.x + threadIdx.x;
  if (i < n) out[i] = i;
}
constexpr int SORT_CHUNK = 4096, SORT_MAX_IMAGES = 8192;
__global__ __launch_bounds__(256) void k_sort_hist(int64_t n_obs, const int32_t* __restrict__ obs_image, int n_img,
                                                   int* __restrict__ hist) {
  extern __shared__ int sh_cnt[];
  for (int k = threadIdx.x; k < n_img; k += blockDim.x) sh_cnt[k] = 0;
  __syncthreads();
  const int64_t b0 = (int64_t)blockIdx.x * SORT_CHUNK, b1 = min(n_obs, b0 + SORT_CHUNK);
  for (int64_t i = b0 + threadIdx.x; i < b1; i += blockDim.x) atomicAdd(&sh_cnt[obs_image[i]], 1);
  __syncthreads();
  for (int k = threadIdx.x; k < n_img; k += blockDim.x) hist[(size_t)blockIdx.x * n_img + k] = sh_cnt[k];
}
__global__ void k_sort_offsets(int n_img, int n_chunks, const int64_t* __restrict__ img_ptr, int* __restrict__ hist) {
  const int k = blockIdx.x * blockDim.x + threadIdx.x;
  if (k >= n_img) return;
  int run = (int)img_ptr[k];
  for (int b = 0; b < n_chunks; ++b) {
    const int c = hist[(size_t)b * n_img + k];
    hist[(size_t)b * n_img + k] = run;
    run += c;
  }
}
__global__ __launch_bounds__(256) void k_sort_scatter(int64_t n_obs, const int32_t* __restrict__ obs_image, int n_img,
                                                      const int* __restrict__ hist, int64_t* __restrict__ img_obs) {
  extern __shared__ int sh_off[];
  int* keys = sh_off + n_img;
  for (int k = threadIdx.x; k < n_img; k += blockDim.x) sh_off[k] = hist[(size_t)blockIdx.x * n_img + k];
  const int64_t b0 = (int64_t)blockIdx.x * SORT_CHUNK, b1 = min(n_obs, b0 + SORT_CHUNK);
  for (int64_t r0 = b0; r0 < b1; r0 += 256) {
    const int64_t i = r0 + threadIdx.x;
    const int key = i < b1 ? obs_image[i] : -1;
    __syncthreads();
    keys[threadIdx.x] = key;
    __syncthreads();
    int before = 0, after = 0;
    if (key >= 0) {
      for (int t = 0; t < 256; ++t) {
        const int same = keys[t] == key;
        before += same & (t < (int)threadIdx.x);
        after += same & (t > (int)threadIdx.x);
      }
      img_obs[sh_off[key] + before] = i;
    }
    __syncthreads();
    if (key >= 0 && after == 0) sh_off[key] += before + 1;
  }
}

struct SolveArena { char* base = nullptr; size_t cap = 0, used = 0, wanted = 0; };
static thread_local SolveArena* g_solve_arena = nullptr;
void* solve_scratch(size_t bytes, bool* owned) {
  const size_t b = ((bytes ? bytes : 1) + 255) & ~(size_t)255;
  if (SolveArena* a = g_solve_arena) {
    a->wanted += b;
    if (a->used + b <= a->cap) { void* p = a->base + a->used; a->used += b; *owned = false; return p; }
  }
  void* p = nullptr;
  *owned = true;
  if (hipMalloc(&p, b) != hipSuccess) { (void)hipGetLastError(); return nullptr; }
  return p;
}
template <typename T>
struct DevBuf {
  T* p = nullptr;
  size_t n = 0;
  bool owned = true;
  int alloc(size_t count) {
    n = count;
    p = static_cast<T*>(solve_scratch(sizeof(T) * (count ? count : 1), &owned));
    return p ? PXR_OK : set_error(PXR_ENOMEM, "hipMalloc(solver buffer): %zu bytes", sizeof(T) * count);
  }
  int upload(const std::vector<T>& h, hipStream_t s) {
    int rc = alloc(h.size());
    if (rc) return rc;
    if (!h.empty()) return hip_check(hipMemcpyAsync(p, h.data(), sizeof(T) * h.size(), hipMemcpyHostToDevice, s), "H2D");
    return PXR_OK;
  }
  ~DevBuf() { if (p && owned) (void)hipFree(p); }
};

int chol_factor_solve(hipStream_t st, double* a, int n, int* d_info, double* linv_ws, double* x_out, bool zero_info = true);
size_t chol_workspace_doubles(int n);
size_t inner_wave_stage_bytes(int64_t n_pts);

int launch_inner_iterations(pxr_ctx* ctx, pxr_arena* arena, const pxr_ba_view* view, const pxr_interp_cfg* cfg,
                            const pxr_loss* loss, const int64_t* d_pt_ptr, const int64_t* d_pt_obs,
                            const int* d_pt_var, double* d_cost_before, const InnerLists* lists, double* d_cost_per_point,
                            const GramCache* gram, bool gram_warm);
int make_inner_lists(pxr_ctx* ctx, const int64_t* h_pt_ptr, int64_t n_pts, void* h_wave_stage, size_t wave_stage_bytes, const pxr_ba_view* view, const int64_t* d_pt_ptr, const int64_t* d_pt_obs,
                     InnerLists* out);
void free_inner_lists(InnerLists* l);

static inline unsigned nblk(int64_t n, int b = 256) { return (unsigned)((n + b - 1) / b); }

#define RC(call) do { int _rc = (call); if (_rc != PXR_OK) return _rc; } while (0)
#define LAUNCH_CHECK(name) RC(hip_check(hipGetLastError(), name))

}

static int ba_solve_impl(pxr_ctx* ctx, pxr_arena* arena, const pxr_ba_view* view, const pxr_interp_cfg* cfg, const double* d_obs_xy,
                         const pxr_loss* loss, const uint8_t* h_pose_const, const uint8_t* h_tvec_const_mask,
                         const uint16_t* h_cam_const_mask, const uint8_t* h_point_const,
                         const pxr_lm_options* opt, pxr_allreduce_fn allreduce, void* ar_user,
                         pxr_lm_summary* sum) {
  using namespace pxr;
  const bool geom = d_obs_xy != nullptr;
  PXR_REQUIRE(ctx && view && loss && opt && sum && (geom || (arena && cfg)), "pxr_ba_solve: NULL argument");
  PXR_REQUIRE(h_pose_const && h_tvec_const_mask && h_cam_const_mask && h_point_const,
              "pxr_ba_solve: NULL parameterisation array");
  PXR_REQUIRE(view->n_obs > 0, "pxr_ba_solve: problem has no residuals (bundle_optimizer.h:174-176)");
  PXR_HIP(hipSetDevice(ctx->device));
  hipStream_t st = ctx->stream;
  const auto t_setup0 = std::chrono::steady_clock::now();
  struct ArenaScope {
    pxr_ctx* ctx; SolveArena a; bool on;
    explicit ArenaScope(pxr_ctx* c) : ctx(c) {
      const char* e = std::getenv("PXR_BA_ARENA");
      on = !(e && e[0] == '0');
      a.base = static_cast<char*>(c->d_solve_arena); a.cap = c->solve_arena_bytes;
      if (on) g_solve_arena = &a;
    }
    ~ArenaScope() {
      g_solve_arena = nullptr;
      if (!on || a.wanted <= a.cap) return;
      (void)hipDeviceSynchronize();
      if (ctx->d_solve_arena) (void)hipFree(ctx->d_solve_arena);
      ctx->d_solve_arena = nullptr; ctx->solve_arena_bytes = 0;
      const size_t want = a.wanted + a.wanted / 16 + (1u << 20);
      if (hipMalloc(&ctx->d_solve_arena, want) == hipSuccess) ctx->solve_arena_bytes = want;
      else { (void)hipGetLastError(); ctx->d_solve_arena = nullptr; }
    }
  } arena_scope(ctx);
  const bool setup_verbose = std::getenv("PXR_VERBOSE") != nullptr;
  auto setup_mark = [&](const char* what) {
    if (setup_verbose)
      fprintf(stderr, "[pxr_ba_solve] setup: %-28s at %.2f ms\n", what,
              std::chrono::duration<double, std::milli>(std::chrono::steady_clock::now() - t_setup0).count());
  };
  const int64_t n_obs = view->n_obs, n_pts = view->n_points;
  const int n_img = view->n_images, n_cam = view->n_cameras;

  std::vector<int32_t> obs_image, obs_point, image_camera(n_img), cam_model(n_cam);
  std::vector<int64_t> img_cnt(n_img + 1, 0), pt_cnt;
  DevBuf<unsigned long long> d_cnt;
  DevBuf<int> d_flags;
  bool device_lists = n_img <= SORT_MAX_IMAGES && std::getenv("PXR_BA_SETUP_HOST") == nullptr;
  PXR_HIP(hipMemcpyAsync(image_camera.data(), view->d_image_camera, 4 * n_img, hipMemcpyDeviceToHost, st));
  PXR_HIP(hipMemcpyAsync(cam_model.data(), view->d_cam_model, 4 * n_cam, hipMemcpyDeviceToHost, st));
  setup_mark("camera tables read");
  if (device_lists) {
    int h_flags[2] = {0, 0};
    RC(d_cnt.alloc((size_t)n_img + 1 + (size_t)n_pts + 1 + 1)); RC(d_flags.alloc(2));
    setup_mark("counter buffers");
    PXR_HIP(hipMemsetAsync(d_cnt.p, 0, sizeof(unsigned long long) * d_cnt.n, st));
    PXR_HIP(hipMemsetAsync(d_flags.p, 0, sizeof(int) * 2, st));
    hipLaunchKernelGGL(k_count_indices, dim3((unsigned)((n_obs + COUNT_CHUNK - 1) / COUNT_CHUNK)), dim3(256), sizeof(unsigned int) * n_img, st, n_obs, view->d_obs_image,
                       view->d_obs_point, n_img, n_pts, d_cnt.p, d_cnt.p + n_img + 1, d_flags.p);
    static_assert(sizeof(unsigned long long) == sizeof(int64_t), "counter width");
    PXR_HIP(hipMemcpyAsync(img_cnt.data(), d_cnt.p, sizeof(int64_t) * (n_img + 1), hipMemcpyDeviceToHost, st));
    PXR_HIP(hipMemcpyAsync(h_flags, d_flags.p, sizeof(int) * 2, hipMemcpyDeviceToHost, st));
    PXR_HIP(hipStreamSynchronize(st));
    PXR_REQUIRE(h_flags[0] == 0, "pxr_ba_solve: an observation references an image / point out of range");
    if (h_flags[1]) {
      device_lists = false;
      std::fill(img_cnt.begin(), img_cnt.end(), 0);
    }
  }
  if (!device_lists) {
    pt_cnt.assign(n_pts + 1, 0);
    obs_image.resize(n_obs); obs_point.resize(n_obs);
    PXR_HIP(hipMemcpyAsync(obs_image.data(), view->d_obs_image, 4 * n_obs, hipMemcpyDeviceToHost, st));
    PXR_HIP(hipMemcpyAsync(obs_point.data(), view->d_obs_point, 4 * n_obs, hipMemcpyDeviceToHost, st));
  }
  PXR_HIP(hipStreamSynchronize(st));
  setup_mark(device_lists ? "counts on the host" : "index arrays on the host");
  static const int kNumParams[11] = {3, 4, 4, 5, 8, 8, 12, 5, 4, 5, 12};
  for (int c = 0; c < n_cam; ++c)
    PXR_REQUIRE(cam_model[c] >= 0 && cam_model[c] <= 10, "pxr_ba_solve: unsupported camera model id %d", cam_model[c]);
  if (!device_lists) {
    for (int64_t i = 0; i < n_obs; ++i) {
      PXR_REQUIRE(obs_image[i] >= 0 && obs_image[i] < n_img && obs_point[i] >= 0 && obs_point[i] < n_pts,
                  "pxr_ba_solve: observation %lld references image %d / point %d out of range", (long long)i,
                  obs_image[i], obs_point[i]);
      ++img_cnt[obs_image[i] + 1]; ++pt_cnt[obs_point[i] + 1];
    }
  }
  std::vector<int> pose_off(n_img), pose_dim(n_img), tmask(n_img), intr_off(n_cam), intr_dim(n_cam), cmask(n_cam), pt_var;
  int off = 0, dpose_max = 0, dintr_max = 0;
  for (int i = 0; i < n_img; ++i) {
    int d = 0;
    tmask[i] = h_tvec_const_mask[i] & 7;
    if (!h_pose_const[i]) d = 3 + (3 - __builtin_popcount(tmask[i]));
    pose_off[i] = off; pose_dim[i] = d; off += d;
    dpose_max = std::max(dpose_max, d);
  }
  for (int c = 0; c < n_cam; ++c) {
    const int K = kNumParams[cam_model[c]];
    cmask[c] = h_cam_const_mask[c] & ((1 << K) - 1);
    const int d = K - __builtin_popcount(cmask[c]);
    intr_off[c] = off; intr_dim[c] = d; off += d;
    dintr_max = std::max(dintr_max, d);
  }
  const int n_c = off;
  const int DC = std::max(1, dpose_max + dintr_max);
  const int LS = 11 + 2 * DC;
  PXR_REQUIRE(opt->linear_solver >= PXR_LINEAR_AUTO && opt->linear_solver <= PXR_LINEAR_ITERATIVE,
              "pxr_ba_solve: unknown linear_solver %d", opt->linear_solver);
  const bool iterative = n_c > 0 && (opt->linear_solver == PXR_LINEAR_ITERATIVE ||
                                     (opt->linear_solver == PXR_LINEAR_AUTO && n_img > PXR_MAX_IMAGES_DIRECT));
  sum->linear_solver = iterative ? PXR_LINEAR_ITERATIVE : PXR_LINEAR_DIRECT;
  sum->linear_iterations = 0; sum->collective_kib = 0;
  int64_t n_pvar = 0;
  if (!device_lists) {
    pt_var.resize(n_pts);
    for (int64_t p = 0; p < n_pts; ++p) { pt_var[p] = (!h_point_const[p] && pt_cnt[p + 1] > 0) ? 1 : 0; n_pvar += pt_var[p]; }
    PXR_REQUIRE(n_c > 0 || n_pvar > 0, "pxr_ba_solve: every parameter block is constant");
    for (int64_t p = 0; p < n_pts; ++p) pt_cnt[p + 1] += pt_cnt[p];
  }
  for (int i = 0; i < n_img; ++i) img_cnt[i + 1] += img_cnt[i];
  std::vector<int64_t> img_obs, pt_obs;
  if (!device_lists) {
    img_obs.resize(n_obs); pt_obs.resize(n_obs);
    std::vector<int64_t> ic(img_cnt.begin(), img_cnt.end() - 1), pc(pt_cnt.begin(), pt_cnt.end() - 1);
    for (int64_t i = 0; i < n_obs; ++i) { img_obs[ic[obs_image[i]]++] = i; pt_obs[pc[obs_point[i]]++] = i; }
  }
  setup_mark(device_lists ? "host prefix sums" : "host CSR (counts, fill)");
  std::vector<ImgChunk> chunks;
  const int64_t CH = 512;
  for (int i = 0; i < n_img; ++i)
    for (int64_t b = img_cnt[i]; b < img_cnt[i + 1]; b += CH)
      chunks.push_back({i, b, std::min(img_cnt[i + 1], b + CH)});

  std::vector<ImgChunk> schur_chunks;
  const int64_t SCH = 1024;
  for (int i = 0; i < n_img; ++i)
    for (int64_t b = img_cnt[i]; b < img_cnt[i + 1]; b += SCH)
      schur_chunks.push_back({i, b, std::min(img_cnt[i + 1], b + SCH)});
  PXR_REQUIRE(n_obs < ((int64_t)1 << 31), "pxr_ba_solve: more than 2^31 observations per rank");
  std::vector<int2> col_group;
  std::vector<int> group_size, group_cols;
  if (iterative) {
    PXR_REQUIRE(DC <= PCG_GS, "pxr_ba_solve: %d camera-side columns per observation exceed the preconditioner block size", DC);
    std::vector<int> cam_users(n_cam, 0);
    for (int i = 0; i < n_img; ++i) ++cam_users[image_camera[i]];
    col_group.assign(n_c, make_int2(-1, -1));
    auto open_group = [&]() { group_size.push_back(0); group_cols.resize(group_cols.size() + PCG_GS, 0); return (int)group_size.size() - 1; };
    auto add_cols = [&](int g, int first, int count) {
      for (int a = 0; a < count; ++a) {
        col_group[first + a] = make_int2(g, group_size[g]);
        group_cols[(size_t)g * PCG_GS + group_size[g]++] = first + a;
      }
    };
    for (int i = 0; i < n_img; ++i) {
      const int c = image_camera[i];
      const bool joint = cam_users[c] == 1 && intr_dim[c] > 0;
      if (pose_dim[i] == 0 && !joint) continue;
      const int g = open_group();
      add_cols(g, pose_off[i], pose_dim[i]);
      if (joint) add_cols(g, intr_off[c], intr_dim[c]);
    }
    for (int c = 0; c < n_cam; ++c)
      if (cam_users[c] != 1 && intr_dim[c] > 0) add_cols(open_group(), intr_off[c], intr_dim[c]);
    for (int c = 0; c < n_c; ++c) PXR_REQUIRE(col_group[c].x >= 0, "pxr_ba_solve: internal: column %d in no preconditioner block", c);
  }
  setup_mark("host structure (CSR, chunks)");
  DevBuf<int> d_pose_off, d_pose_dim, d_tmask, d_intr_off, d_intr_dim, d_cmask, d_pt_var;
  DevBuf<int64_t> d_img_obs, d_pt_ptr, d_pt_obs;
  DevBuf<ImgChunk> d_chunks, d_schur_chunks;
  DevBuf<int4> d_obs_cols, d_so;
  DevBuf<int> d_part_obs;
  RC(d_pose_off.upload(pose_off, st)); RC(d_pose_dim.upload(pose_dim, st)); RC(d_tmask.upload(tmask, st));
  RC(d_intr_off.upload(intr_off, st)); RC(d_intr_dim.upload(intr_dim, st)); RC(d_cmask.upload(cmask, st));
  RC(d_chunks.upload(chunks, st));
  DevBuf<uint8_t> d_pt_const;
  DevBuf<unsigned long long> d_pt_part;
  unsigned long long h_n_pvar = 0;
  if (!device_lists) { RC(d_pt_var.upload(pt_var, st)); RC(d_pt_ptr.upload(pt_cnt, st)); }
  if (device_lists) {
    const int n_parts = (int)((n_pts + PT_SCAN_CHUNK - 1) / PT_SCAN_CHUNK);
    unsigned long long* const d_pt_cnt = d_cnt.p + n_img + 1;
    RC(d_pt_var.alloc(n_pts)); RC(d_pt_ptr.alloc((size_t)n_pts + 1)); RC(d_pt_const.alloc(n_pts)); RC(d_pt_part.alloc(n_parts));
    PXR_HIP(hipMemcpyAsync(d_pt_const.p, h_point_const, (size_t)n_pts, hipMemcpyHostToDevice, st));
    hipLaunchKernelGGL(k_pt_scan_partials, dim3(n_parts), dim3(256), 0, st, n_pts, (const unsigned long long*)d_pt_cnt, d_pt_part.p);
    hipLaunchKernelGGL(k_pt_scan_apply, dim3(n_parts), dim3(256), 0, st, n_pts, (const unsigned long long*)d_pt_cnt, (const unsigned long long*)d_pt_part.p,
                       (const uint8_t*)d_pt_const.p, d_pt_ptr.p, d_pt_var.p, d_pt_cnt + n_pts + 1);
    PXR_HIP(hipMemcpyAsync(&h_n_pvar, d_pt_cnt + n_pts + 1, sizeof(h_n_pvar), hipMemcpyDeviceToHost, st));
    RC(d_img_obs.alloc(n_obs)); RC(d_pt_obs.alloc(n_obs));
    hipLaunchKernelGGL(k_iota, dim3(nblk(n_obs)), dim3(256), 0, st, n_obs, d_pt_obs.p);
    DevBuf<int64_t> d_img_ptr;
    DevBuf<int> d_hist;
    const int n_chunks = (int)((n_obs + SORT_CHUNK - 1) / SORT_CHUNK);
    RC(d_img_ptr.upload(img_cnt, st)); RC(d_hist.alloc((size_t)n_chunks * n_img));
    hipLaunchKernelGGL(k_sort_hist, dim3(n_chunks), dim3(256), sizeof(int) * n_img, st, n_obs, view->d_obs_image, n_img, d_hist.p);
    hipLaunchKernelGGL(k_sort_offsets, dim3((n_img + 255) / 256), dim3(256), 0, st, n_img, n_chunks, d_img_ptr.p, d_hist.p);
    hipLaunchKernelGGL(k_sort_scatter, dim3(n_chunks), dim3(256), sizeof(int) * (n_img + 256), st, n_obs, view->d_obs_image, n_img,
                       d_hist.p, d_img_obs.p);
    LAUNCH_CHECK("observation-list kernels");
    setup_mark("list kernels launched");
    PXR_HIP(hipStreamSynchronize(st));
    setup_mark("list kernels done");
    n_pvar = (int64_t)h_n_pvar;
    PXR_REQUIRE(n_c > 0 || n_pvar > 0, "pxr_ba_solve: every parameter block is constant");
  } else {
    RC(d_img_obs.upload(img_obs, st)); RC(d_pt_obs.upload(pt_obs, st));
  }
  RC(d_schur_chunks.upload(schur_chunks, st));
  RC(d_obs_cols.alloc(n_obs)); RC(d_so.alloc(n_obs)); RC(d_part_obs.alloc(n_obs));
  hipLaunchKernelGGL(k_build_descriptors, dim3(nblk(n_obs)), dim3(256), 0, st, n_obs, view->d_obs_image, view->d_obs_point,
                     view->d_image_camera, d_pt_obs.p, d_img_obs.p, d_pt_ptr.p, d_pt_var.p, d_pose_off.p, d_pose_dim.p,
                     d_intr_off.p, d_intr_dim.p, d_obs_cols.p, d_part_obs.p, d_so.p);
  LAUNCH_CHECK("k_build_descriptors");
  setup_mark("index uploads");
  const size_t nc1 = n_c ? n_c : 1;
  DevBuf<double> L, V, gp, Vd0, T, W, U, S , gcd , damp_c, scale_c, scale_p,
      delta_c, delta_p, rec_a, rec_b, q1, t1, k1, X1, scal;
  RC(L.alloc((size_t)n_obs * LS)); RC(V.alloc((size_t)n_pts * 6)); RC(gp.alloc((size_t)n_pts * 3));
  RC(Vd0.alloc((size_t)n_pts * 3)); RC(T.alloc((size_t)n_pts * 6));
  RC(W.alloc((size_t)n_obs * DC * 3));
  RC(U.alloc(iterative ? (size_t)n_img * DC * DC : nc1 * nc1)); RC(S.alloc(iterative ? 1 : (nc1 + 1) * (nc1 + 1)));
  RC(gcd.alloc(2 * nc1 + 8)); RC(damp_c.alloc(nc1));
  RC(scale_c.alloc(nc1)); RC(scale_p.alloc((size_t)n_pts * 3)); RC(delta_c.alloc(nc1)); RC(delta_p.alloc((size_t)n_pts * 3));
  RC(rec_a.alloc((size_t)n_obs * PXR_OBS_REC)); RC(rec_b.alloc((size_t)n_obs * PXR_OBS_REC));
  RC(q1.alloc((size_t)n_img * 4)); RC(t1.alloc((size_t)n_img * 3)); RC(k1.alloc((size_t)n_cam * PXR_KPAD)); RC(X1.alloc((size_t)n_pts * 3));
  RC(scal.alloc(16 + 16 * PXR_LIMBS + 1 + 4));
  double* scal_sum = scal.p; double* scal_rep = scal.p + 8;
  const int ldS = n_c + 1;
  double* rhs = S.p + n_c;
  DevBuf<double> xsol, linv;
  RC(xsol.alloc(nc1)); RC(linv.alloc(iterative ? 1 : chol_workspace_doubles(n_c)));
  DevBuf<int2> d_col_group; DevBuf<int> d_group_size, d_group_cols;
  DevBuf<double> pcg_u, pcg_mloc, pcg_g, pcg_vec, pcg_scal;
  PcgArgs pcg;
  if (iterative) {
    RC(d_col_group.upload(col_group, st)); RC(d_group_size.upload(group_size, st)); RC(d_group_cols.upload(group_cols, st));
    RC(pcg_u.alloc((size_t)n_pts * 3)); RC(pcg_mloc.alloc((size_t)n_img * DC * DC));
    RC(pcg_g.alloc(group_size.size() * PCG_GS * PCG_GS)); RC(pcg_vec.alloc(5 * nc1));
    RC(pcg_scal.alloc(16 + 8 * ((nc1 + 255) / 256)));
  }
  DevBuf<int> d_kchunk_ptr, d_schunk_ptr, d_col_ent_ptr;
  DevBuf<int2> d_col_ent;
  DevBuf<double> det_kpart, det_gimg, det_wpart, det_mpart;
  const int det_ne_max = DC * (DC + 1) / 2 + DC;
  if (ctx->deterministic && iterative) {
    auto first_chunks = [&](const std::vector<ImgChunk>& cs) {
      std::vector<int> ptr(n_img + 1, 0);
      for (const ImgChunk& c : cs) ++ptr[c.img + 1];
      for (int i = 0; i < n_img; ++i) ptr[i + 1] += ptr[i];
      return ptr;
    };
    const std::vector<int> kptr = first_chunks(chunks), sptr = first_chunks(schur_chunks);
    RC(d_kchunk_ptr.upload(kptr, st)); RC(d_schunk_ptr.upload(sptr, st));
    std::vector<int> ent_ptr(n_c + 1, 0);
    auto col_of = [&](int i, int a) { return a < pose_dim[i] ? pose_off[i] + a : intr_off[image_camera[i]] + (a - pose_dim[i]); };
    for (int i = 0; i < n_img; ++i)
      for (int a = 0; a < pose_dim[i] + intr_dim[image_camera[i]]; ++a) ++ent_ptr[col_of(i, a) + 1];
    for (int c = 0; c < n_c; ++c) ent_ptr[c + 1] += ent_ptr[c];
    std::vector<int2> ent(ent_ptr[n_c]);
    std::vector<int> fill(ent_ptr.begin(), ent_ptr.end() - 1);
    for (int i = 0; i < n_img; ++i)
      for (int a = 0; a < pose_dim[i] + intr_dim[image_camera[i]]; ++a) ent[fill[col_of(i, a)]++] = make_int2(i, a);
    RC(d_col_ent_ptr.upload(ent_ptr, st)); RC(d_col_ent.upload(ent, st));
    RC(det_kpart.alloc(std::max<size_t>(1, chunks.size()) * det_ne_max)); RC(det_gimg.alloc((size_t)n_img * DC));
    RC(det_wpart.alloc(std::max<size_t>(1, schur_chunks.size()) * DC)); RC(det_mpart.alloc(std::max<size_t>(1, schur_chunks.size()) * DC * DC));
    PXR_HIP(hipMemsetAsync(det_kpart.p, 0, sizeof(double) * det_kpart.n, st));
    PXR_HIP(hipMemsetAsync(det_wpart.p, 0, sizeof(double) * det_wpart.n, st));
    PXR_HIP(hipMemsetAsync(det_mpart.p, 0, sizeof(double) * det_mpart.n, st));
    PXR_HIP(hipStreamSynchronize(st));
  }
  double* diagU = gcd.p; double* gc = gcd.p + nc1;
  DevBuf<double> cb_flags;
  RC(cb_flags.alloc(2));
  int* d_info = reinterpret_cast<int*>(scal.p + 16 + 16 * PXR_LIMBS);

  setup_mark("work buffers allocated");
  double* cur_q = const_cast<double*>(view->d_qvec); double* cur_t = const_cast<double*>(view->d_tvec);
  double* cur_k = const_cast<double*>(view->d_cam_params); double* cur_X = const_cast<double*>(view->d_xyz);
  hipLaunchKernelGGL(k_normalize_q, dim3(nblk(n_img)), dim3(256), 0, st, n_img, cur_q);

  SolveDev dv;
  dv.v = *view;
  dv.pose_off = d_pose_off.p; dv.pose_dim = d_pose_dim.p; dv.tmask = d_tmask.p;
  dv.intr_off = d_intr_off.p; dv.intr_dim = d_intr_dim.p; dv.cmask = d_cmask.p; dv.pt_var = d_pt_var.p;
  dv.scale_c = scale_c.p; dv.scale_p = scale_p.p; dv.n_c = n_c; dv.DC = DC; dv.LS = LS; dv.ldS = ldS;
  pxr_ba_view cand_view = *view;
  cand_view.d_qvec = q1.p; cand_view.d_tvec = t1.p; cand_view.d_cam_params = k1.p; cand_view.d_xyz = X1.p;

  const bool multi = allreduce != nullptr || (ctx->comm != nullptr && (ctx->nranks > 1 || ctx->force_collective));
  auto ar = [&](double* buf, int64_t count) -> int {
    if (allreduce) {
      if (allreduce(ar_user, buf, count) != 0) return set_error(PXR_EHIP, "pxr_ba_solve: all-reduce callback failed");
      return PXR_OK;
    }
    return comm_allreduce_sum(ctx, buf, count);
  };
  DevBuf<double> S_packed;
  const int64_t packed_doubles = (int64_t)n_c * (n_c + 3) / 2;
  if (multi && !iterative && n_c > 0) RC(S_packed.alloc((size_t)packed_doubles));
  sum->collective_kib = (multi && !iterative) ? (int)((packed_doubles * 8 + 1023) / 1024) : 0;
  const bool det_fixed = ctx->deterministic && !iterative && opt->jacobi_scaling != 0;
  const bool det_iter = ctx->deterministic && iterative;
  const bool det = det_fixed || det_iter;
  sum->accumulation = det_fixed ? 1 : (det_iter ? 2 : 0); sum->initial_us = 0;
  const bool bcast = multi && ctx->nranks > 1 && !det;
  auto from_rank0 = [&](double* buf, int64_t count) -> int {
    if (!bcast) return PXR_OK;
    if (ctx->rank != 0) hipLaunchKernelGGL(k_zero, dim3(nblk(count)), dim3(256), 0, st, count, buf);
    return ar(buf, count);
  };
  struct { long long* p; } slimb;
  slimb.p = reinterpret_cast<long long*>(scal.p + 16);
  long long* const limb_arg = det ? slimb.p : nullptr;
  DevBuf<double> i64_halves;
  const bool native_i64 = allreduce == nullptr;
  if (det && multi && !native_i64) RC(i64_halves.alloc((size_t)2 * std::max<int64_t>({packed_doubles, 2 * (int64_t)nc1 + 8, 16 * PXR_LIMBS})));
  auto ar_i64 = [&](long long* buf, int64_t count) -> int {
    if (!multi || count <= 0) return PXR_OK;
    if (native_i64) return comm_allreduce_sum_i64(ctx, buf, count);
    hipLaunchKernelGGL(k_i64_split, dim3(nblk(count)), dim3(256), 0, st, count, (const long long*)buf, i64_halves.p);
    RC(ar(i64_halves.p, 2 * count));
    hipLaunchKernelGGL(k_i64_join, dim3(nblk(count)), dim3(256), 0, st, count, (const double*)i64_halves.p, buf);
    return PXR_OK;
  };
  auto zero_scalars = [&]() -> int {
    PXR_HIP(hipMemsetAsync(scal.p, 0, sizeof(double) * (16 + 16 * PXR_LIMBS + 1), st));
    return PXR_OK;
  };
  struct { double* p; } lin_stats;
  constexpr int kScalAll = 16 + 16 * PXR_LIMBS + 1 + 4;
  lin_stats.p = scal.p + (kScalAll - 4);
  if (!ctx->h_readback) PXR_HIP(hipHostMalloc(&ctx->h_readback, 4096, hipHostMallocDefault));
  static_assert(sizeof(double) * kScalAll <= 4096, "read-back buffer");
  double* const h_scal = static_cast<double*>(ctx->h_readback);
  std::memset(h_scal, 0, sizeof(double) * kScalAll);
  double* const h_lin_stats = h_scal + (kScalAll - 4);
  const int* const h_info_word = reinterpret_cast<const int*>(h_scal + 16 + 16 * PXR_LIMBS);
  const bool spin_wait = std::getenv("PXR_BLOCKING_WAIT") == nullptr;
  auto read_scal = [&](double* h16) -> int {
    if (det) {
      RC(ar_i64(slimb.p, 8 * PXR_LIMBS));
      hipLaunchKernelGGL(k_limbs_finish, dim3(1), dim3(64), 0, st, (const long long*)slimb.p, 0xffffu, scal.p);
    } else {
      hipLaunchKernelGGL(k_limbs_finish, dim3(1), dim3(64), 0, st, (const long long*)slimb.p, (1u << 0) | (1u << 4), scal.p);
      RC(ar(scal_sum, 8));
      RC(from_rank0(scal_rep, 8));
    }
    PXR_HIP(hipMemcpyAsync(h_scal, scal.p, sizeof(double) * kScalAll, hipMemcpyDeviceToHost, st));
    if (spin_wait) {
      PXR_HIP(hipEventRecord(ctx->ev_sync, st));
      hipError_t q;
      while ((q = hipEventQuery(ctx->ev_sync)) == hipErrorNotReady) {}
      PXR_HIP(q);
    } else PXR_HIP(hipStreamSynchronize(st));
    std::memcpy(h16, h_scal, sizeof(double) * 16);
    return PXR_OK;
  };
  DevBuf<double> det_part, chunk_trace;
  RC(det_part.alloc((size_t)n_pts + 8));
  RC(chunk_trace.alloc(chunks.size() + 1));
  auto det_scale_for = [](double md, double cost_now) {
    const double bound = 8.0 * std::max({md, std::sqrt(2.0 * md * std::max(cost_now, 0.0)), 1e-300});
    return std::ldexp(1.0, 62 - (int)std::ceil(std::log2(bound)));
  };
  double lin_md = 1.0;
  bool gram_cache = !geom && ctx->gram_cache && gram_eval_supported(arena, view) && cfg->use_float_simd == 0;
  bool gram_inner = !geom && opt->use_inner_iterations != 0 && arena->dtype != PXR_F64 && (arena->C == 128 || arena->C == 64) && !getenv("PXR_INNER_OLD") &&
                    !getenv("PXR_INNER_PACKED") && cfg->use_float_simd == 0;
  for (int c = 0; c < n_cam; ++c) gram_inner = gram_inner && cam_model[c] <= PXR_OPENCV;
  bool inner_cache = gram_inner && gram_eval_supported(arena, view) && !getenv("PXR_INNER_NO_CACHE");
  GramCache gram;
  if ((gram_cache || inner_cache) && gram_eval_prepare(ctx, arena, view, &gram) != PXR_OK) {
    gram_cache = false; inner_cache = false;
    (void)set_error(PXR_OK, "");
  }
  bool geom_ext = false;
  for (int c = 0; c < n_cam; ++c) geom_ext = geom_ext || cam_model[c] > PXR_OPENCV;
  setup_mark("Gram-matrix cache prepared");
  bool gram_warm = false;
  int n_evaluations = 0;
  bool cur_is_exact = true;
  auto evaluate = [&](const pxr_ba_view& v, double* rec) -> int {
    if (geom) RC(geom_eval(ctx, &v, d_obs_xy, rec, nullptr));
    else if (gram_cache && n_evaluations > 0) { RC(gram_evaluate(ctx, arena, &v, cfg, gram, rec)); gram_warm = true; }
    else RC(ba_eval_with_cost(ctx, arena, &v, cfg, 1, rec, nullptr, nullptr, nullptr, nullptr, nullptr));
    ++n_evaluations;
    hipLaunchKernelGGL(k_cost_limbs, dim3(1024), dim3(256), 0, st, (const double*)rec, n_obs, *loss, slimb.p + 0 * PXR_LIMBS);
    LAUNCH_CHECK("cost");
    return PXR_OK;
  };
  double lin_scale = 0.0;
  auto linearize = [&](const double* rec) -> int {
    hipLaunchKernelGGL(k_jac, dim3((unsigned)((n_obs + JAC_THREADS - 1) / JAC_THREADS)), dim3(JAC_THREADS),
                       sizeof(double) * (JAC_THREADS / 64) * 64 * (LS + 3 * DC + 1), st, dv, rec, *loss, L.p, W.p);
    hipLaunchKernelGGL(k_point, dim3(nblk(n_pts)), dim3(256), 0, st, dv, d_pt_ptr.p, d_pt_obs.p, L.p, V.p, gp.p);
    PXR_HIP(hipMemsetAsync(U.p, 0, sizeof(double) * U.n, st));
    PXR_HIP(hipMemsetAsync(gcd.p, 0, sizeof(double) * gcd.n, st));
    if (n_c > 0 && !chunks.empty()) {
      hipLaunchKernelGGL(k_img, dim3((unsigned)chunks.size()), dim3(256), sizeof(double) * ((size_t)IMG_BATCH * LS + 256), st, dv,
                         d_chunks.p, d_img_obs.p, L.p, U.p, gc, iterative ? 1 : 0, lin_scale, lin_scale != 0.0 ? chunk_trace.p : (double*)nullptr,
                         det_iter ? det_kpart.p : (double*)nullptr, det_ne_max);
      if (det_iter) {
        RC(pcg_blocks_from_partials(st, dv, d_kchunk_ptr.p, det_kpart.p, det_ne_max, U.p, det_gimg.p, d_col_ent_ptr.p, d_col_ent.p, diagU, gc));
        LAUNCH_CHECK("linearize kernels");
        RC(ar(gcd.p, 2 * (int64_t)nc1));
        return PXR_OK;
      }
      if (lin_scale != 0.0) {
        hipLaunchKernelGGL(k_diag_and_trace, dim3(1), dim3(1024), 0, st, n_c, (const double*)U.p, diagU, (const double*)chunk_trace.p, (int)chunks.size(),
                           reinterpret_cast<long long*>(gcd.p + 2 * nc1));
        RC(ar_i64(reinterpret_cast<long long*>(gcd.p), 2 * (int64_t)nc1 + PXR_LIMBS));
        hipLaunchKernelGGL(k_finish_and_stats, dim3(1), dim3(1024), 0, st, n_c, 2 * (int)nc1, gcd.p, lin_scale,
                           reinterpret_cast<const long long*>(gcd.p + 2 * nc1), lin_stats.p);
        LAUNCH_CHECK("linearize kernels");
        return PXR_OK;
      }
      if (iterative) RC(pcg_diag_from_blocks(st, dv, U.p, diagU));
      else hipLaunchKernelGGL(k_extract_diag, dim3(nblk(n_c)), dim3(256), 0, st, n_c, U.p, diagU);
    }
    LAUNCH_CHECK("linearize kernels");
    RC(ar(gcd.p, 2 * (int64_t)nc1));
    return PXR_OK;
  };
  auto lin_fits = [&](const double* stt, double md_made_for) {
    if (n_c == 0 || chunks.empty()) return true;
    const double mx = stt[0], sm = stt[1], mn = stt[2], tr = stt[3];
    if (!(std::isfinite(mx) && std::isfinite(sm) && std::isfinite(tr))) return false;
    if (mn < 0.0) return false;
    if (std::fabs(tr - sm) > std::ldexp(1.0, 61) / lin_scale) return false;
    return mx <= 8.0 * md_made_for;
  };
  bool lin_not_finite = false;
  auto linearize_checked = [&](const double* rec, double md_guess, double cost_now, bool refine = false) -> int {
    if (!det_fixed) return linearize(rec);
    for (int attempt = 0; attempt < 8; ++attempt) {
      lin_md = md_guess;
      lin_scale = det_scale_for(lin_md, cost_now);
      RC(linearize(rec));
      PXR_HIP(hipMemcpyAsync(h_lin_stats, lin_stats.p, sizeof(double) * 4, hipMemcpyDeviceToHost, st));
      PXR_HIP(hipStreamSynchronize(st));
      if (lin_fits(h_lin_stats, lin_md)) {
        if (refine && attempt == 0 && h_lin_stats[0] * 64.0 < md_guess) { md_guess = std::max(h_lin_stats[0], 1e-300); continue; }
        return PXR_OK;
      }
      if (!(std::isfinite(h_lin_stats[3]) && h_lin_stats[3] >= 0.0)) { lin_not_finite = true; return PXR_OK; }
      md_guess = std::max(h_lin_stats[3], 2.0 * md_guess);
    }
    return set_error(PXR_EINVAL, "pxr_ba_solve: the fixed-point grid of the deterministic mode could not be fitted");
  };
  auto refresh_damping = [&]() -> int {
    if (n_c > 0) hipLaunchKernelGGL(k_clamp, dim3(nblk(n_c)), dim3(256), 0, st, (int64_t)n_c, diagU, opt->min_lm_diagonal, opt->max_lm_diagonal, damp_c.p);
    hipLaunchKernelGGL(k_point_diag, dim3(nblk(n_pts)), dim3(256), 0, st, n_pts, V.p, Vd0.p);
    hipLaunchKernelGGL(k_clamp, dim3(nblk(n_pts * 3)), dim3(256), 0, st, n_pts * 3, Vd0.p, opt->min_lm_diagonal, opt->max_lm_diagonal, Vd0.p);
    LAUNCH_CHECK("damping kernels");
    return PXR_OK;
  };

  if (iterative) {
    pcg.st = st; pcg.dv = dv;
    pcg.chunks = d_schur_chunks.p; pcg.n_chunks = (int)schur_chunks.size(); pcg.so = d_so.p;
    pcg.pt_ptr = d_pt_ptr.p; pcg.part_obs = d_part_obs.p; pcg.obs_cols = d_obs_cols.p;
    pcg.W = W.p; pcg.T = T.p; pcg.gp = gp.p; pcg.gc = gc; pcg.damp_c = damp_c.p; pcg.Ublk = U.p;
    pcg.n_groups = (int)group_size.size(); pcg.col_group = d_col_group.p; pcg.group_size = d_group_size.p;
    pcg.group_cols = d_group_cols.p;
    pcg.u = pcg_u.p; pcg.Mloc = pcg_mloc.p; pcg.Gm = pcg_g.p;
    pcg.x = xsol.p; pcg.r = pcg_vec.p; pcg.p = pcg_vec.p + nc1; pcg.q = pcg_vec.p + 2 * nc1; pcg.z = pcg_vec.p + 3 * nc1;
    pcg.b = pcg_vec.p + 4 * nc1; pcg.cgs = pcg_scal.p; pcg.cg_part = pcg_scal.p + 16; pcg.d_fail = d_info;
    pcg.det = det_iter;
    if (det_iter) {
      pcg.chunk_ptr = d_schunk_ptr.p; pcg.col_ent_ptr = d_col_ent_ptr.p; pcg.col_ent = d_col_ent.p;
      pcg.wpart = det_wpart.p; pcg.mpart = det_mpart.p;
    }
  }
  const std::function<int(double*, int64_t)> ar_fn = ar;
  auto gradient_below_tolerance = [&](bool* below) -> int {
    double h[16];
    RC(zero_scalars());
    if (n_c > 0) hipLaunchKernelGGL(k_count_above, dim3(nblk(n_c)), dim3(256), 0, st, (int64_t)n_c, gc, scale_c.p, opt->gradient_tolerance, scal_rep + 4,
                                    det ? slimb.p + (8 + 4) * PXR_LIMBS : (long long*)nullptr);
    hipLaunchKernelGGL(k_count_above, dim3(nblk(n_pts * 3)), dim3(256), 0, st, n_pts * 3, gp.p, scale_p.p, opt->gradient_tolerance, scal_sum + 5,
                       det ? slimb.p + 5 * PXR_LIMBS : (long long*)nullptr);
    RC(read_scal(h));
    *below = h[5] == 0.0 && h[12] == 0.0;
    return PXR_OK;
  };

  struct InnerListsOwner { InnerLists l; ~InnerListsOwner() { free_inner_lists(&l); } } inner_lists;
  if (gram_inner) {
    const int64_t* h_pt_ptr = pt_cnt.data();
    std::vector<int64_t> pageable;
    void* wave_stage = nullptr;
    const size_t ptr_bytes = (sizeof(int64_t) * ((size_t)n_pts + 1) + 255) & ~(size_t)255, wave_bytes = inner_wave_stage_bytes(n_pts);
    if (device_lists) {
      int64_t* stage = (ptr_bytes + wave_bytes) <= ((size_t)1 << 28) ? static_cast<int64_t*>(setup_staging(ctx, ptr_bytes + wave_bytes)) : nullptr;
      if (stage) wave_stage = reinterpret_cast<char*>(stage) + ptr_bytes;
      else { pageable.resize((size_t)n_pts + 1); stage = pageable.data(); }
      PXR_HIP(hipMemcpyAsync(stage, d_pt_ptr.p, sizeof(int64_t) * ((size_t)n_pts + 1), hipMemcpyDeviceToHost, st));
      PXR_HIP(hipStreamSynchronize(st));
      h_pt_ptr = stage;
    }
    RC(make_inner_lists(ctx, h_pt_ptr, n_pts, wave_stage, wave_stage ? wave_bytes : 0, view, d_pt_ptr.p, d_pt_obs.p, &inner_lists.l));
  }
  setup_mark("inner-iteration tables");
  const auto t_loop0 = std::chrono::steady_clock::now();
  sum->setup_ms = std::chrono::duration<double, std::milli>(t_loop0 - t_setup0).count();
  sum->num_camera_unknowns = n_c; sum->num_point_unknowns = 3 * n_pvar;
  sum->iterations = 0; sum->num_successful = 0; sum->termination = PXR_TERM_NO_CONVERGENCE;
  const bool use_lds_schur = std::getenv("PXR_SCHUR_GLOBAL_ATOMICS") == nullptr;
  int CT = n_c > 0 ? std::min(n_c, (int)((128 * 1024 / 8 - DC) / DC)) : 1;
  int n_ctiles = n_c > 0 ? (n_c + CT - 1) / CT : 1;
  if (const char* e = std::getenv("PXR_SCHUR_CTILES")) n_ctiles = std::max(n_ctiles, std::min(std::max(1, n_c), std::atoi(e)));
  CT = n_c > 0 ? (n_c + n_ctiles - 1) / n_ctiles : 1;
  const size_t schur_shmem = sizeof(double) * ((size_t)DC * CT + DC + 3 * 1024);
  if (use_lds_schur && n_c > 0)
    PXR_HIP(hipFuncSetAttribute(reinterpret_cast<const void*>(DC <= 8 ? k_schur_lds<8> : (DC <= 16 ? k_schur_lds<16> : k_schur_lds<32>)),
                                hipFuncAttributeMaxDynamicSharedMemorySize, (int)schur_shmem));
  PXR_HIP(hipFuncSetAttribute(reinterpret_cast<const void*>(k_jac), hipFuncAttributeMaxDynamicSharedMemorySize,
                              (int)(sizeof(double) * (JAC_THREADS / 64) * 64 * (LS + 3 * DC + 1))));
  const bool verbose = std::getenv("PXR_VERBOSE") != nullptr;
  const bool phase_timing = std::getenv("PXR_PHASE_TIMING") != nullptr;
  double ph_ms[8] = {0, 0, 0, 0, 0, 0, 0, 0};
  auto ph_t0 = std::chrono::steady_clock::now();
  auto phase = [&](int k) {
    if (!phase_timing) return;
    (void)hipStreamSynchronize(st);
    const auto now = std::chrono::steady_clock::now();
    ph_ms[k] += std::chrono::duration<double, std::milli>(now - ph_t0).count();
    ph_t0 = now;
  };

  double hs[16];
  double* rec_cur = rec_a.p; double* rec_cand = rec_b.p;
  RC(zero_scalars());
  RC(evaluate(dv.v, rec_cur));
  RC(read_scal(hs));
  double cost = hs[0];
  sum->initial_cost = cost;
  if (!std::isfinite(cost)) {
    sum->final_cost = cost; sum->termination = PXR_TERM_FAILURE;
    sum->total_ms = std::chrono::duration<double, std::milli>(std::chrono::steady_clock::now() - t_loop0).count();
    return PXR_OK;
  }
  hipLaunchKernelGGL(k_fill, dim3(nblk(nc1)), dim3(256), 0, st, (int64_t)nc1, 1.0, scale_c.p);
  hipLaunchKernelGGL(k_fill, dim3(nblk(n_pts * 3)), dim3(256), 0, st, n_pts * 3, 1.0, scale_p.p);
  RC(linearize_checked(rec_cur, std::ldexp(1.0, 32), cost, !opt->jacobi_scaling));
  auto fail_not_finite = [&]() -> int {
    sum->final_cost = cost; sum->final_radius = opt->initial_radius; sum->termination = PXR_TERM_FAILURE;
    sum->total_ms = std::chrono::duration<double, std::milli>(std::chrono::steady_clock::now() - t_loop0).count();
    return PXR_OK;
  };
  if (lin_not_finite) return fail_not_finite();
  if (opt->jacobi_scaling) {
    if (n_c > 0) hipLaunchKernelGGL(k_jacobi_scale, dim3(nblk(n_c)), dim3(256), 0, st, (int64_t)n_c, diagU, scale_c.p);
    hipLaunchKernelGGL(k_point_diag, dim3(nblk(n_pts)), dim3(256), 0, st, n_pts, V.p, Vd0.p);
    hipLaunchKernelGGL(k_jacobi_scale, dim3(nblk(n_pts * 3)), dim3(256), 0, st, n_pts * 3, Vd0.p, scale_p.p);
    RC(linearize_checked(rec_cur, 1.0 / 8.0, cost));
    if (lin_not_finite) return fail_not_finite();
  }
  if (opt->gradient_tolerance > 0.0) {
    bool below = false;
    RC(gradient_below_tolerance(&below));
    if (below) {
      sum->termination = PXR_TERM_CONVERGENCE; sum->final_cost = cost; sum->final_radius = opt->initial_radius;
      sum->total_ms = std::chrono::duration<double, std::milli>(std::chrono::steady_clock::now() - t_loop0).count();
      return PXR_OK;
    }
  }
  double radius = opt->initial_radius, decrease_factor = 2.0;
  int invalid = 0;
  bool reuse_diag = false;
  bool inner_enabled = opt->use_inner_iterations != 0, inner_useful = false;
  PXR_HIP(hipStreamSynchronize(st));
  sum->initial_us = (int32_t)std::min<double>(2e9, 1e3 * std::chrono::duration<double, std::milli>(std::chrono::steady_clock::now() - t_loop0).count());
  bool any_cb = ctx->iter_cb != nullptr;
  if (multi) {
    double h = any_cb ? 1.0 : 0.0;
    PXR_HIP(hipMemcpyAsync(cb_flags.p, &h, sizeof(h), hipMemcpyHostToDevice, st));
    RC(ar(cb_flags.p, 1));
    PXR_HIP(hipMemcpyAsync(&h, cb_flags.p, sizeof(h), hipMemcpyDeviceToHost, st));
    PXR_HIP(hipStreamSynchronize(st));
    any_cb = h > 0.0;
  }
  auto notify = [&](int iteration, bool valid, bool successful, double cost_now, double change, double rel, double radius_next, double step) -> int {
    if (!any_cb) return 0;
    int rc = 0;
    if (ctx->iter_cb) {
      pxr_iteration_summary is;
      is.iteration = iteration; is.step_is_valid = valid; is.step_is_successful = successful; is.cost = cost_now; is.cost_change = change;
      is.relative_decrease = rel; is.trust_region_radius = radius_next; is.step_norm = step;
      rc = ctx->iter_cb(&is, ctx->iter_user);
    }
    if (multi) {
      double h[2] = {rc == 1 ? 1.0 : 0.0, rc == 2 ? 1.0 : 0.0};
      if (hipMemcpyAsync(cb_flags.p, h, sizeof(h), hipMemcpyHostToDevice, st) != hipSuccess || ar(cb_flags.p, 2) != PXR_OK ||
          hipMemcpyAsync(h, cb_flags.p, sizeof(h), hipMemcpyDeviceToHost, st) != hipSuccess || hipStreamSynchronize(st) != hipSuccess)
        return 1;
      rc = h[0] > 0.0 ? 1 : (h[1] > 0.0 ? 2 : 0);
    }
    return rc;
  };
  auto user_stop = [&](int rc) {
    if (rc == 1) { sum->termination = PXR_TERM_FAILURE; return true; }
    if (rc == 2) { sum->termination = PXR_TERM_CONVERGENCE; return true; }
    return false;
  };
  if (user_stop(notify(0, false, false, cost, 0.0, 0.0, radius, 0.0))) {
    sum->final_cost = cost; sum->final_radius = radius;
    sum->total_ms = std::chrono::duration<double, std::milli>(std::chrono::steady_clock::now() - t_loop0).count();
    return PXR_OK;
  }

  while (true) {
    if (sum->iterations >= opt->max_iterations) { sum->termination = PXR_TERM_NO_CONVERGENCE; break; }
    if (radius < opt->min_radius) { sum->termination = PXR_TERM_CONVERGENCE; break; }
    ++sum->iterations;
    phase(7);
    if (!reuse_diag) RC(refresh_damping());
    const double inv_radius = 1.0 / radius;
    hipLaunchKernelGGL(k_pinv, dim3(nblk(n_pts)), dim3(256), 0, st, n_pts, d_pt_var.p, V.p, Vd0.p, inv_radius, T.p, scal.p, 16 + 16 * PXR_LIMBS + 1);
    if (n_pts == 0) RC(zero_scalars());
    bool ok = true;
    double inexact_correction = 0.0;
    if (n_c > 0 && iterative) {
      PcgResult pr;
      RC(pcg_solve(pcg, inv_radius, opt, ar_fn, &pr));
      phase(2);
      sum->linear_iterations += pr.iterations;
      if (!pr.ok) ok = false;
      inexact_correction = 0.5 * pr.x_dot_r;
      PXR_HIP(hipMemsetAsync(d_info, 0, sizeof(int), st));
      hipLaunchKernelGGL(k_finish_camera_step, dim3(nblk(n_c)), dim3(256), 0, st, n_c, xsol.p, gc, damp_c.p, inv_radius, delta_c.p, scal_rep, limb_arg);
      RC(from_rank0(delta_c.p, n_c));
    } else if (n_c > 0) {
      const double schur_scale = det_fixed ? lin_scale : 0.0;
      hipLaunchKernelGGL(k_copy_upper_add_diag, dim3(nblk((int64_t)n_c * ldS)), dim3(256), 0, st, n_c, U.p, (const double*)nullptr, 0.0, (const double*)nullptr, S.p, 1, schur_scale);
      if (use_lds_schur) {
#define SCHUR_LAUNCH(GG)                                                                                              \
  hipLaunchKernelGGL(k_schur_lds<GG>, dim3((unsigned)schur_chunks.size(), (unsigned)n_ctiles), dim3(1024), schur_shmem, st, dv, \
                     d_schur_chunks.p, d_so.p, d_part_obs.p, d_obs_cols.p, W.p, T.p, gp.p, CT, S.p, rhs, schur_scale)
        if (DC <= 8) SCHUR_LAUNCH(8); else if (DC <= 16) SCHUR_LAUNCH(16); else SCHUR_LAUNCH(32);
#undef SCHUR_LAUNCH
      } else {
        hipLaunchKernelGGL(k_schur, dim3(nblk(n_obs * DC)), dim3(256), 0, st, dv, d_pt_ptr.p, d_pt_obs.p, W.p, T.p, gp.p, S.p, rhs, schur_scale);
      }
      LAUNCH_CHECK("schur kernels");
      phase(0);
      if (multi) {
        hipLaunchKernelGGL(k_pack_upper, dim3((unsigned)n_c), dim3(256), 0, st, n_c, S.p, S_packed.p);
        if (schur_scale != 0.0) RC(ar_i64(reinterpret_cast<long long*>(S_packed.p), packed_doubles));
        else RC(ar(S_packed.p, packed_doubles));
        hipLaunchKernelGGL(k_unpack_upper, dim3((unsigned)n_c), dim3(256), 0, st, n_c, S_packed.p, S.p);
        LAUNCH_CHECK("pack / unpack of the reduced camera system");
      }
      phase(1);
      hipLaunchKernelGGL(k_copy_upper_add_diag, dim3(nblk((int64_t)n_c * ldS)), dim3(256), 0, st, n_c, U.p, damp_c.p, inv_radius, gc, S.p, 0, schur_scale);
      RC(chol_factor_solve(st, S.p, n_c, d_info, linv.p, xsol.p, false));
      phase(2);
      hipLaunchKernelGGL(k_finish_camera_step, dim3(nblk(n_c)), dim3(256), 0, st, n_c, xsol.p, gc, damp_c.p, inv_radius, delta_c.p, scal_rep, limb_arg);
      RC(from_rank0(delta_c.p, n_c));
    }
    phase(3);
    double model_cost_change = 0, cand_cost = 0, step_norm = 0, x_norm = 0;
    if (ok) {
#define BACKSUB_LAUNCH(GG)                                                                                                          \
  hipLaunchKernelGGL(k_backsub<GG>, dim3(nblk((n_pts * GG + BACKSUB_PPG - 1) / BACKSUB_PPG)), dim3(256), 0, st, dv, d_pt_ptr.p, d_part_obs.p, d_obs_cols.p, W.p, T.p, gp.p, \
                     delta_c.p, Vd0.p, inv_radius, delta_p.p, scal_sum, limb_arg)
      if (DC <= 8) BACKSUB_LAUNCH(8); else if (DC <= 16) BACKSUB_LAUNCH(16); else BACKSUB_LAUNCH(32);
#undef BACKSUB_LAUNCH
      ParamPtrs out{q1.p, t1.p, k1.p, X1.p};
      const int64_t upd_blocks = nblk(((int64_t)n_img + n_cam + n_pts + UPDATE_IPT - 1) / UPDATE_IPT);
      hipLaunchKernelGGL(k_update, dim3((unsigned)upd_blocks), dim3(256), 0, st, dv, delta_c.p, delta_p.p, out, scal_rep, scal_sum, limb_arg);
      LAUNCH_CHECK("step kernels");
      const bool do_inner = inner_enabled;
      if (do_inner) {
        PXR_HIP(hipMemsetAsync(det_part.p, 0, sizeof(double) * (size_t)n_pts, st));
        if (geom) RC(launch_inner_geom(ctx, &cand_view, d_obs_xy, loss, d_pt_ptr.p, d_pt_obs.p, d_pt_var.p, scal_sum + 4, det_part.p, geom_ext));
        else {
          RC(launch_inner_iterations(ctx, arena, &cand_view, cfg, loss, d_pt_ptr.p, d_pt_obs.p, d_pt_var.p, scal_sum + 4, gram_inner ? &inner_lists.l : nullptr,
                                     det_part.p, (gram_cache || inner_cache) ? &gram : nullptr, gram_warm));
          gram_warm = true;
        }
        hipLaunchKernelGGL(k_limb_accumulate, dim3(256), dim3(256), 0, st, (const double*)det_part.p, n_pts, slimb.p + 4 * PXR_LIMBS);
        PXR_HIP(hipMemsetAsync(scal_sum + 2, 0, sizeof(double), st));
        PXR_HIP(hipMemsetAsync(slimb.p + 2 * PXR_LIMBS, 0, sizeof(long long) * PXR_LIMBS, st));
        hipLaunchKernelGGL(k_point_step_norm, dim3(nblk(n_pts)), dim3(256), 0, st, n_pts, d_pt_var.p, cur_X, X1.p, scal_sum + 2,
                           det ? slimb.p + 2 * PXR_LIMBS : (long long*)nullptr);
        LAUNCH_CHECK("inner iteration kernels");
      }
      phase(4);
      RC(evaluate(cand_view, rec_cand));
      RC(read_scal(hs));
      const int h_info = *h_info_word;
      if (det_fixed && !lin_fits(h_lin_stats, lin_md)) {
        RC(linearize_checked(rec_cur, std::max(h_lin_stats[3], 2.0 * lin_md), cost));
        if (lin_not_finite) { sum->termination = PXR_TERM_FAILURE; break; }
        --sum->iterations;
        continue;
      }
      if (n_c > 0 && h_info != 0) ok = false;
      phase(5);
      cand_cost = hs[0];
      model_cost_change = 0.5 * (hs[1] + hs[8]) + inexact_correction;
      step_norm = std::sqrt(hs[2] + hs[9]);
      x_norm = std::sqrt(hs[3] + hs[10]);
      if (!(model_cost_change > 0.0) || !std::isfinite(model_cost_change)) ok = false;
      if (!std::isfinite(cand_cost)) cand_cost = std::numeric_limits<double>::max();
      inner_useful = false;
      if (ok && do_inner && cand_cost < std::numeric_limits<double>::max()) {
        const double cost_before = hs[4];
        model_cost_change += cost_before - cand_cost;
        inner_useful = cand_cost < cost;
        inner_enabled = (1.0 - cand_cost / cost_before) > opt->inner_iteration_tolerance;
      }
    }
    if (verbose)
      fprintf(stderr, "[pxr_ba_solve] it %3d cost %.9e cand %.9e mcc %.3e radius %.3e |dx| %.3e %s\n", sum->iterations,
              cost, cand_cost, model_cost_change, radius, step_norm, ok ? "" : "INVALID");
    auto reevaluate_current = [&]() -> int {
      if (!(gram_cache && cur_is_exact && n_evaluations > 1)) return PXR_OK;
      double h2[16];
      RC(zero_scalars());
      RC(evaluate(dv.v, rec_cur));
      RC(read_scal(h2));
      if (std::isfinite(h2[0])) cost = h2[0];
      cur_is_exact = false;
      return PXR_OK;
    };
    if (!ok) {
      if (++invalid >= opt->max_consecutive_invalid_steps) { sum->termination = PXR_TERM_FAILURE; break; }
      radius *= 0.5; reuse_diag = true;
      if (user_stop(notify(sum->iterations, false, false, cost, 0.0, 0.0, radius, step_norm))) break;
      continue;
    }
    invalid = 0;
    if (step_norm <= opt->parameter_tolerance * (x_norm + opt->parameter_tolerance)) { sum->termination = PXR_TERM_CONVERGENCE; break; }
    const double cost_change = cost - cand_cost;
    if (std::fabs(cost_change) <= opt->function_tolerance * cost) { sum->termination = PXR_TERM_CONVERGENCE; break; }
    const double rel = cost_change / model_cost_change;
    if (inner_useful || rel > opt->min_relative_decrease) {
      {
        Copy4 c4{{q1.p, t1.p, k1.p, X1.p}, {cur_q, cur_t, cur_k, cur_X},
                 {(int64_t)4 * n_img, (int64_t)3 * n_img, (int64_t)PXR_KPAD * n_cam, (int64_t)3 * n_pts}};
        hipLaunchKernelGGL(k_copy4, dim3((unsigned)std::min<int64_t>(1024, nblk(3 * n_pts + 1))), dim3(256), 0, st, c4);
      }
      std::swap(rec_cur, rec_cand);
      cost = cand_cost;
      cur_is_exact = false;
      if (det_fixed) { lin_md = std::max(h_lin_stats[0], 1e-300); lin_scale = det_scale_for(lin_md, cost); }
      RC(linearize(rec_cur));
      phase(6);
      ++sum->num_successful;
      const double tmp = 2.0 * rel - 1.0;
      radius = radius / std::max(1.0 / 3.0, 1.0 - tmp * tmp * tmp);
      radius = std::min(opt->max_radius, radius);
      decrease_factor = 2.0; reuse_diag = false;
      if (opt->gradient_tolerance > 0.0) {
        bool below = false;
        RC(gradient_below_tolerance(&below));
        if (below) { sum->termination = PXR_TERM_CONVERGENCE; break; }
      }
      if (user_stop(notify(sum->iterations, true, true, cost, cost_change, rel, radius, step_norm))) break;
    } else {
      RC(reevaluate_current());
      radius = radius / decrease_factor; decrease_factor *= 2.0; reuse_diag = true;
      if (user_stop(notify(sum->iterations, true, false, cost, cost_change, rel, radius, step_norm))) break;
    }
  }
  PXR_HIP(hipStreamSynchronize(st));
  if (phase_timing)
    fprintf(stderr, "[pxr_ba_solve] phase ms over %d iterations: schur-build %.2f allreduce %.2f potrf %.2f potrs %.2f "
            "backsub+update %.2f eval+cost %.2f linearize %.2f other %.2f\n", sum->iterations, ph_ms[0], ph_ms[1],
            ph_ms[2], ph_ms[3], ph_ms[4], ph_ms[5], ph_ms[6], ph_ms[7]);
  sum->final_cost = cost; sum->final_radius = radius;
  sum->total_ms = std::chrono::duration<double, std::milli>(std::chrono::steady_clock::now() - t_loop0).count();
  return PXR_OK;
}

extern "C" int pxr_ba_solve(pxr_ctx* ctx, pxr_arena* arena, const pxr_ba_view* view, const pxr_interp_cfg* cfg,
                            const pxr_loss* loss, const uint8_t* h_pose_const, const uint8_t* h_tvec_const_mask,
                            const uint16_t* h_cam_const_mask, const uint8_t* h_point_const,
                            const pxr_lm_options* opt, pxr_allreduce_fn allreduce, void* ar_user,
                            pxr_lm_summary* sum) {
  PXR_REQUIRE(arena && cfg, "pxr_ba_solve: NULL argument");
  return ba_solve_impl(ctx, arena, view, cfg, nullptr, loss, h_pose_const, h_tvec_const_mask, h_cam_const_mask, h_point_const, opt,
                       allreduce, ar_user, sum);
}

extern "C" int pxr_ba_solve_geometric(pxr_ctx* ctx, const pxr_ba_view* view, const double* d_obs_xy, const pxr_loss* loss,
                                      const uint8_t* h_pose_const, const uint8_t* h_tvec_const_mask,
                                      const uint16_t* h_cam_const_mask, const uint8_t* h_point_const,
                                      const pxr_lm_options* opt, pxr_allreduce_fn allreduce, void* ar_user,
                                      pxr_lm_summary* sum) {
  PXR_REQUIRE(d_obs_xy, "pxr_ba_solve_geometric: the observed keypoints are missing");
  return ba_solve_impl(ctx, nullptr, view, nullptr, d_obs_xy, loss, h_pose_const, h_tvec_const_mask, h_cam_const_mask, h_point_const,
                       opt, allreduce, ar_user, sum);
}
```

### pixel-perfect-sfm_amd/csrc/pxr_internal.h

```cpp
#pragma once
#include <hip/hip_runtime.h>

#include <cstdarg>
#include <cstdio>
#include <string>

#include "pixsfm_hip.h"

struct pxr_ctx {
  int device = 0;
  hipStream_t stream = nullptr;
  hipEvent_t ev_start = nullptr, ev_stop = nullptr;
  hipEvent_t ev_sync = nullptr;
  void* h_readback = nullptr;
  void* h_setup = nullptr;
  size_t h_setup_bytes = 0;
  double* d_scratch = nullptr;
  size_t scratch_bytes = 0;
  int num_cus = 256;
  void* d_workspace = nullptr;
  size_t workspace_bytes = 0;
  void* d_workspace_mat = nullptr;
  size_t workspace_mat_bytes = 0;
  void* comm = nullptr;
  int rank = 0, nranks = 1;
  bool force_collective = false;
  int64_t collective_calls = 0;
  int64_t collective_bytes = 0;
  pxr_iteration_callback iter_cb = nullptr;
  void* iter_user = nullptr;
  void* h_stage[2] = {nullptr, nullptr};
  hipEvent_t ev_stage[2] = {nullptr, nullptr};
  size_t stage_bytes = 0;
  bool deterministic = true;
  bool gram_cache = true;
  void* d_gram = nullptr;
  size_t gram_bytes = 0;
  void* d_solve_arena = nullptr;
  size_t solve_arena_bytes = 0;
};

struct pxr_arena {
  pxr_ctx* ctx = nullptr;
  int dtype = PXR_F16, C = 0, H = 0, W = 0;
  int64_t n = 0;
  void* d_data = nullptr;
  bool owns_data = false;
  int32_t* d_corners = nullptr;
  double* d_scales = nullptr;
  double up = 1.0;
  size_t elem_size() const { return dtype == PXR_F16 ? 2 : (dtype == PXR_F32 ? 4 : 8); }
  size_t patch_bytes() const { return (size_t)H * W * C * elem_size(); }
};

namespace pxr {
int set_error(int code, const char* fmt, ...);
inline int hip_check(hipError_t e, const char* what) {
  if (e == hipSuccess) return PXR_OK;
  return set_error(PXR_EHIP, "%s: %s", what, hipGetErrorString(e));
}
void* setup_staging(pxr_ctx* ctx, size_t bytes);
int comm_allreduce_sum(pxr_ctx* ctx, double* d_buf, int64_t count, bool even_single_rank = false);
int comm_allreduce_sum_i64(pxr_ctx* ctx, long long* d_buf, int64_t count);
int ba_eval_with_cost(pxr_ctx* ctx, pxr_arena* arena, const pxr_ba_view* view, const pxr_interp_cfg* cfg,
                      int with_jacobian, double* d_rec, double* d_r, double* d_gx, double* d_gy,
                      const pxr_loss* loss, double* d_cost_sum);
int geom_eval(pxr_ctx* ctx, const pxr_ba_view* view, const double* d_obs_xy, double* d_rec, double* d_res);
int launch_inner_geom(pxr_ctx* ctx, const pxr_ba_view* view, const double* d_obs_xy, const pxr_loss* loss, const int64_t* d_pt_ptr,
                      const int64_t* d_pt_obs, const int* d_pt_var, double* d_cost_before, double* d_cost_per_point,
                      bool extended_models);
struct InnerLists {
  void* d_short = nullptr; int64_t n_short = 0; int maxo_short = 1;
  int* d_long = nullptr; int64_t n_long = 0;
  void* d_slots = nullptr;
  void* d_waves = nullptr; int64_t n_waves = 0;
  void* d_wave_heads = nullptr;
  bool own_short = true, own_long = true, own_slots = true, own_heads = true;
};
void* solve_scratch(size_t bytes, bool* owned);
struct GramCache {
  double* G = nullptr;
  void* cell = nullptr;
  int* list = nullptr;
  int* count = nullptr;
  double* r2 = nullptr;
  int64_t n_obs = 0;
};
bool gram_eval_supported(const pxr_arena* arena, const pxr_ba_view* view);
int gram_eval_prepare(pxr_ctx* ctx, pxr_arena* arena, const pxr_ba_view* view, GramCache* out);
int gram_evaluate(pxr_ctx* ctx, pxr_arena* arena, const pxr_ba_view* v, const pxr_interp_cfg* cfg, const GramCache& gc, double* rec);
int gram_build_flagged(pxr_ctx* ctx, pxr_arena* arena, const pxr_ba_view* v, const GramCache& gc);
}

#define PXR_HIP(call)                                        \
  do {                                                       \
    int _rc = pxr::hip_check((call), #call);                 \
    if (_rc != PXR_OK) return _rc;                           \
  } while (0)

#define PXR_REQUIRE(cond, ...)                               \
  do {                                                       \
    if (!(cond)) return pxr::set_error(PXR_EINVAL, __VA_ARGS__); \
  } while (0)
```

### pixel-perfect-sfm_amd/pixsfm_amd/_lib.py

```python
import ctypes as C
import os

HERE = os.path.dirname(os.path.abspath(__file__))
LIB_PATH = os.environ.get("PXR_HIP_LIB") or os.path.join(HERE, "libpixsfm_hip.so")

KPAD = 12
OBS_REC = 8
F16, F32, F64 = 0, 1, 2
U8 = 3
CAMERA_MODEL_IDS = {"SIMPLE_PINHOLE": 0, "PINHOLE": 1, "SIMPLE_RADIAL": 2, "RADIAL": 3, "OPENCV": 4, "OPENCV_FISHEYE": 5,
                    "FULL_OPENCV": 6, "FOV": 7, "SIMPLE_RADIAL_FISHEYE": 8, "RADIAL_FISHEYE": 9, "THIN_PRISM_FISHEYE": 10}
LOSS_IDS = {"trivial": 0, "cauchy": 1, "huber": 2, "soft_l1": 3}


class PixsfmHipError(RuntimeError):
    code = 0


PXR_EUNSUPPORTED = -4


class InterpCfg(C.Structure):
    _fields_ = [("l2_normalize", C.c_int32), ("use_float_simd", C.c_int32), ("check_bounds", C.c_int32)]


class Loss(C.Structure):
    _fields_ = [("type", C.c_int32), ("a", C.c_double)]


class BaView(C.Structure):
    _fields_ = [("n_obs", C.c_int64), ("d_obs_image", C.c_void_p), ("d_obs_point", C.c_void_p),
                ("d_obs_patch", C.c_void_p), ("n_images", C.c_int32), ("d_image_camera", C.c_void_p),
                ("d_qvec", C.c_void_p), ("d_tvec", C.c_void_p), ("n_cameras", C.c_int32),
                ("d_cam_model", C.c_void_p), ("d_cam_params", C.c_void_p), ("n_points", C.c_int64),
                ("d_xyz", C.c_void_p), ("d_refs", C.c_void_p)]


class LMOptions(C.Structure):
    _fields_ = [("max_iterations", C.c_int32), ("function_tolerance", C.c_double),
                ("gradient_tolerance", C.c_double), ("parameter_tolerance", C.c_double),
                ("initial_radius", C.c_double), ("max_radius", C.c_double), ("min_radius", C.c_double),
                ("min_relative_decrease", C.c_double), ("min_lm_diagonal", C.c_double),
                ("max_lm_diagonal", C.c_double), ("max_consecutive_invalid_steps", C.c_int32),
                ("jacobi_scaling", C.c_int32), ("use_inner_iterations", C.c_int32),
                ("inner_iteration_tolerance", C.c_double), ("linear_solver", C.c_int32),
                ("max_linear_solver_iterations", C.c_int32), ("eta", C.c_double), ("linear_r_tolerance", C.c_double)]


class LMSummary(C.Structure):
    _fields_ = [("iterations", C.c_int32), ("num_successful", C.c_int32), ("termination", C.c_int32),
                ("num_camera_unknowns", C.c_int32), ("num_point_unknowns", C.c_int64),
                ("initial_cost", C.c_double), ("final_cost", C.c_double), ("final_radius", C.c_double),
                ("total_ms", C.c_double), ("setup_ms", C.c_double), ("linear_solver", C.c_int32),
                ("collective_kib", C.c_int32), ("linear_iterations", C.c_int64), ("accumulation", C.c_int32),
                ("initial_us", C.c_int32)]

    def as_dict(self):
        return {k: getattr(self, k) for k, _ in self._fields_}


ALLREDUCE_FN = C.CFUNCTYPE(C.c_int, C.c_void_p, C.c_void_p, C.c_int64)


class KaView(C.Structure):
    _fields_ = [("n_nodes", C.c_int64), ("d_kp", C.c_void_p), ("d_node_patch", C.c_void_p),
                ("d_node_const", C.c_void_p), ("n_edges", C.c_int64), ("d_edge_src", C.c_void_p),
                ("d_edge_dst", C.c_void_p), ("d_edge_w", C.c_void_p), ("n_problems", C.c_int32),
                ("d_prob_node_ptr", C.c_void_p), ("d_prob_nodes", C.c_void_p), ("d_prob_edge_ptr", C.c_void_p),
                ("d_prob_edges", C.c_void_p), ("n_unary", C.c_int64), ("d_unary_node", C.c_void_p),
                ("d_unary_ref", C.c_void_p), ("d_unary_w", C.c_void_p), ("d_prob_unary_ptr", C.c_void_p),
                ("d_prob_unary", C.c_void_p), ("d_prob_group", C.c_void_p)]


class TriView(C.Structure):
    _fields_ = [("n_tracks", C.c_int64), ("d_track_offsets", C.c_void_p), ("n_obs", C.c_int64), ("d_obs_image", C.c_void_p),
                ("d_obs_xy", C.c_void_p), ("n_images", C.c_int32), ("d_image_camera", C.c_void_p), ("d_qvec", C.c_void_p),
                ("d_tvec", C.c_void_p), ("n_cameras", C.c_int32), ("d_cam_model", C.c_void_p), ("d_cam_params", C.c_void_p)]


class TriOptions(C.Structure):
    _fields_ = [("min_tri_angle", C.c_double), ("max_angle_error", C.c_double), ("max_reproj_error", C.c_double),
                ("min_track_len", C.c_int32), ("max_hypotheses", C.c_int32)]


_SIGNATURES = {
    "pxr_version": (C.c_int, []),
    "pxr_last_error": (C.c_char_p, []),
    "pxr_ctx_create": (C.c_int, [C.c_int, C.c_void_p, C.POINTER(C.c_void_p)]),
    "pxr_ctx_destroy": (C.c_int, [C.c_void_p]),
    "pxr_ctx_sync": (C.c_int, [C.c_void_p]),
    "pxr_malloc": (C.c_int, [C.c_void_p, C.c_size_t, C.POINTER(C.c_void_p)]),
    "pxr_free": (C.c_int, [C.c_void_p, C.c_void_p]),
    "pxr_memcpy_h2d": (C.c_int, [C.c_void_p, C.c_void_p, C.c_void_p, C.c_size_t]),
    "pxr_memcpy_d2h": (C.c_int, [C.c_void_p, C.c_void_p, C.c_void_p, C.c_size_t]),
    "pxr_memset": (C.c_int, [C.c_void_p, C.c_void_p, C.c_int, C.c_size_t]),
    "pxr_timer_start": (C.c_int, [C.c_void_p]),
    "pxr_timer_stop": (C.c_int, [C.c_void_p, C.POINTER(C.c_double)]),
    "pxr_arena_create": (C.c_int, [C.c_void_p, C.c_int, C.c_int, C.c_int, C.c_int, C.c_int64, C.c_void_p,
                                   C.POINTER(C.c_void_p)]),
    "pxr_arena_destroy": (C.c_int, [C.c_void_p]),
    "pxr_arena_upload": (C.c_int, [C.c_void_p, C.c_int64, C.c_int64, C.c_void_p, C.c_void_p, C.c_void_p]),
    "pxr_arena_upload_gather": (C.c_int, [C.c_void_p, C.c_int64, C.c_int64, C.c_void_p, C.c_void_p, C.c_void_p]),
    "pxr_arena_extract": (C.c_int, [C.c_void_p, C.c_void_p, C.c_int64, C.c_int64, C.c_void_p, C.c_int, C.c_int, C.c_int,
                                    C.c_void_p, C.c_double, C.c_double, C.c_int]),
    "pxr_dsift_dense": (C.c_int, [C.c_void_p, C.c_void_p, C.c_int, C.c_int, C.c_int, C.c_int, C.c_int, C.c_double, C.c_void_p]),
    "pxr_dsift_extract": (C.c_int, [C.c_void_p, C.c_void_p, C.c_int64, C.c_int64, C.c_void_p, C.c_int, C.c_int, C.c_int, C.c_int,
                                    C.c_int, C.c_double, C.c_void_p, C.c_double, C.c_double, C.c_int]),
    "pxr_arena_data": (C.c_void_p, [C.c_void_p]),
    "pxr_arena_corners": (C.c_void_p, [C.c_void_p]),
    "pxr_arena_scales": (C.c_void_p, [C.c_void_p]),
    "pxr_arena_size": (C.c_int64, [C.c_void_p]),
    "pxr_ba_eval": (C.c_int, [C.c_void_p, C.c_void_p, C.POINTER(BaView), C.POINTER(InterpCfg), C.c_int,
                              C.c_void_p, C.c_void_p, C.c_void_p, C.c_void_p]),
    "pxr_ba_eval_gram": (C.c_int, [C.c_void_p, C.c_void_p, C.POINTER(BaView), C.POINTER(InterpCfg), C.c_int, C.c_void_p,
                                   C.POINTER(C.c_int32)]),
    "pxr_ba_projection_jacobian": (C.c_int, [C.c_void_p, C.POINTER(BaView), C.c_void_p]),
    "pxr_ba_solve": (C.c_int, [C.c_void_p, C.c_void_p, C.POINTER(BaView), C.POINTER(InterpCfg), C.POINTER(Loss),
                               C.c_void_p, C.c_void_p, C.c_void_p, C.c_void_p, C.POINTER(LMOptions),
                               C.c_void_p, C.c_void_p, C.POINTER(LMSummary)]),
    "pxr_ba_geom_eval": (C.c_int, [C.c_void_p, C.POINTER(BaView), C.c_void_p, C.c_void_p, C.c_void_p]),
    "pxr_ba_solve_geometric": (C.c_int, [C.c_void_p, C.POINTER(BaView), C.c_void_p, C.POINTER(Loss),
                                         C.c_void_p, C.c_void_p, C.c_void_p, C.c_void_p, C.POINTER(LMOptions),
                                         C.c_void_p, C.c_void_p, C.POINTER(LMSummary)]),
    "pxr_image_to_world": (C.c_int, [C.c_void_p, C.c_int64, C.c_void_p, C.c_int32, C.c_void_p, C.c_void_p, C.c_void_p, C.c_void_p,
                                     C.c_void_p]),
    "pxr_triangulate_tracks": (C.c_int, [C.c_void_p, C.POINTER(TriView), C.POINTER(TriOptions), C.c_void_p, C.c_void_p, C.c_void_p,
                                         C.c_void_p, C.c_void_p]),
    "pxr_triangulate_tracks_timed": (C.c_int, [C.c_void_p, C.POINTER(TriView), C.POINTER(TriOptions), C.c_void_p, C.c_void_p,
                                               C.c_void_p, C.c_void_p, C.c_void_p, C.POINTER(C.c_double)]),
    "pxr_ba_compute_references": (C.c_int, [C.c_void_p, C.c_void_p, C.POINTER(BaView), C.POINTER(InterpCfg),
                                            C.POINTER(Loss), C.c_int, C.c_void_p, C.c_void_p, C.c_void_p, C.c_void_p]),
    "pxr_costmap_extract": (C.c_int, [C.c_void_p, C.c_void_p, C.c_void_p, C.c_int64, C.c_int64, C.c_void_p, C.c_void_p,
                                      C.c_void_p, C.POINTER(Loss), C.c_int, C.c_int]),
    "pxr_costmap_extract_ex": (C.c_int, [C.c_void_p, C.c_void_p, C.c_void_p, C.c_int64, C.c_int64, C.c_void_p, C.c_void_p,
                                         C.c_void_p, C.POINTER(Loss), C.c_int, C.c_int, C.POINTER(InterpCfg), C.c_double, C.c_int]),
    "pxr_arena_set_upsampling": (C.c_int, [C.c_void_p, C.c_double]),
    "pxr_arena_upsampling": (C.c_double, [C.c_void_p]),
    "pxr_interpolate": (C.c_int, [C.c_void_p, C.c_void_p, C.POINTER(InterpCfg), C.c_int64, C.c_void_p, C.c_void_p,
                                  C.c_void_p, C.c_void_p]),
    "pxr_nearest_references": (C.c_int, [C.c_void_p, C.c_void_p, C.POINTER(InterpCfg), C.c_int64, C.c_void_p, C.c_void_p,
                                         C.c_void_p, C.c_void_p, C.c_void_p, C.c_void_p, C.c_void_p, C.c_void_p]),
    "pxr_ka_eval": (C.c_int, [C.c_void_p, C.c_void_p, C.POINTER(KaView), C.POINTER(InterpCfg), C.POINTER(Loss),
                              C.c_void_p, C.c_void_p, C.c_void_p, C.c_void_p]),
    "pxr_ka_solve": (C.c_int, [C.c_void_p, C.c_void_p, C.POINTER(KaView), C.POINTER(InterpCfg), C.POINTER(Loss),
                               C.c_double, C.POINTER(LMOptions), C.c_void_p, C.POINTER(LMSummary)]),
    "pxr_dense_spd_solve": (C.c_int, [C.c_void_p, C.c_void_p, C.c_int, C.c_void_p, C.POINTER(C.c_int)]),
    "pxr_graph_track_labels": (C.c_int, [C.c_int64, C.c_void_p, C.c_int64, C.c_void_p, C.c_void_p, C.c_void_p, C.c_void_p,
                                         C.POINTER(C.c_int64)]),
    "pxr_graph_score_labels": (C.c_int, [C.c_int64, C.c_int64, C.c_void_p, C.c_void_p, C.c_void_p, C.c_void_p, C.c_void_p]),
    "pxr_graph_root_labels": (C.c_int, [C.c_int64, C.c_void_p, C.c_void_p, C.c_void_p]),
    "pxr_graph_labels_device": (C.c_int, [C.c_void_p, C.c_int64, C.c_void_p, C.c_int64, C.c_void_p, C.c_void_p, C.c_void_p,
                                          C.c_void_p, C.c_void_p, C.c_void_p, C.POINTER(C.c_int64)]),
    "pxr_ka_build_edges": (C.c_int, [C.c_int64, C.c_void_p, C.c_void_p, C.c_int64, C.c_void_p, C.c_void_p, C.c_void_p,
                                     C.c_void_p, C.c_void_p, C.c_void_p, C.c_int64, C.c_int, C.c_int, C.c_double,
                                     C.c_void_p, C.c_void_p, C.c_void_p, C.POINTER(C.c_int64)]),
    "pxr_ba_build_problem": (C.c_int, [C.c_int32, C.c_void_p, C.c_void_p, C.c_void_p, C.c_int32, C.c_void_p, C.c_int64, C.c_void_p,
                                       C.c_void_p, C.c_void_p, C.c_void_p, C.c_void_p, C.c_void_p, C.c_void_p, C.c_void_p, C.c_void_p,
                                       C.c_void_p, C.c_int, C.c_int, C.c_int, C.c_int, C.c_int, C.c_int, C.POINTER(C.c_int64),
                                       C.c_void_p, C.c_void_p, C.c_void_p, C.c_void_p, C.c_void_p, C.c_void_p, C.c_void_p, C.c_void_p]),
    "pxr_ba_cost": (C.c_int, [C.c_void_p, C.c_void_p, C.c_int64, C.POINTER(Loss), C.POINTER(C.c_double)]),
    "pxr_comm_unique_id": (C.c_int, [C.c_void_p]),
    "pxr_comm_init": (C.c_int, [C.c_void_p, C.c_void_p, C.c_int, C.c_int]),
    "pxr_comm_destroy": (C.c_int, [C.c_void_p]),
    "pxr_set_iteration_callback": (C.c_int, [C.c_void_p, C.c_void_p, C.c_void_p]),
    "pxr_set_deterministic": (C.c_int, [C.c_void_p, C.c_int]),
    "pxr_get_deterministic": (C.c_int, [C.c_void_p]),
    "pxr_set_gram_cache": (C.c_int, [C.c_void_p, C.c_int]),
    "pxr_get_gram_cache": (C.c_int, [C.c_void_p]),
    "pxr_comm_set_rank": (C.c_int, [C.c_void_p, C.c_int, C.c_int]),
    "pxr_comm_rank": (C.c_int, [C.c_void_p, C.POINTER(C.c_int), C.POINTER(C.c_int)]),
    "pxr_comm_allreduce_sum": (C.c_int, [C.c_void_p, C.c_void_p, C.c_int64]),
    "pxr_comm_force": (C.c_int, [C.c_void_p, C.c_int]),
    "pxr_comm_stats": (C.c_int, [C.c_void_p, C.POINTER(C.c_int64), C.POINTER(C.c_int64), C.c_int]),
}
LINEAR_AUTO, LINEAR_DIRECT, LINEAR_ITERATIVE = 0, 1, 2
COMM_ID_BYTES = 128

_lib = None


class IterationSummary(C.Structure):
    _fields_ = [("iteration", C.c_int32), ("step_is_valid", C.c_int32), ("step_is_successful", C.c_int32), ("cost", C.c_double),
                ("cost_change", C.c_double), ("relative_decrease", C.c_double), ("trust_region_radius", C.c_double), ("step_norm", C.c_double)]


ITERATION_CALLBACK = C.CFUNCTYPE(C.c_int, C.POINTER(IterationSummary), C.c_void_p)


def declared_symbols():
    return sorted(_SIGNATURES)


def load():
    global _lib
    if _lib is not None:
        return _lib
    if not os.path.exists(LIB_PATH):
        raise PixsfmHipError(
            "libpixsfm_hip.so not found at %s -- build it with `python -c 'import __graft_entry__ as g; "
            "g.build()'` (hipcc --offload-arch=gfx950). There is no CPU fallback." % LIB_PATH)
    try:
        import torch
    except ImportError:
        pass
    lib = C.CDLL(LIB_PATH)
    for name, (res, args) in _SIGNATURES.items():
        fn = getattr(lib, name)
        fn.restype = res
        fn.argtypes = args
    _lib = lib
    return lib


def check(rc, what=""):
    if rc != 0:
        msg = load().pxr_last_error()
        err = PixsfmHipError("%s failed (code %d): %s" % (what, rc, msg.decode() if msg else "?"))
        err.code = int(rc)
        raise err
```

Baseline: 1.432 billion residual_blocks/s.

## Shrink inner gram-packed LDS by keeping diagonal blocks in registers

Adds a compact LDS layout for the packed inner-iteration gram kernel, now the default. Only the off-diagonal Gram blocks are staged in shared memory per slot, while each lane keeps its own diagonal block and D terms in registers. The goal is to fit more wavefronts per CU by cutting LDS per workgroup. It also precomputes per-point reference self-dot products in a table instead of recomputing them per wave, writes rebuilt Grams straight to the global cache, and drops the texel prefetch depth from three to two. The cost is more register pressure, extra barriers per build, and a landing buffer that reuses the residual area.

```diff
diff --git a/include/pixsfm_hip.h b/include/pixsfm_hip.h
--- a/include/pixsfm_hip.h
+++ b/include/pixsfm_hip.h
@@ -155,6 +155,7 @@
 int pxr_get_gram_cache(pxr_ctx* ctx);
 int pxr_ba_eval_gram(pxr_ctx* ctx, pxr_arena* arena, const pxr_ba_view* view, const pxr_interp_cfg* cfg, int reset,
                      double* d_rec, int32_t* h_rebuilt);
+int pxr_inner_gram_occupancy(int dtype, int channels, int wide_layout, int* workgroups_per_cu, int* lds_bytes);
 
 #define PXR_COMM_ID_BYTES 128
 int pxr_comm_unique_id(void* h_id );
diff --git a/pixel-perfect-sfm_amd/csrc/pxr_ba_inner.hip b/pixel-perfect-sfm_amd/csrc/pxr_ba_inner.hip
--- a/pixel-perfect-sfm_amd/csrc/pxr_ba_inner.hip
+++ b/pixel-perfect-sfm_amd/csrc/pxr_ba_inner.hip
@@ -25,6 +25,7 @@
   double* gram_G;
   int2* gram_cell;
   int gram_warm;
+  const double* ref_r2;
 };
 
 template <int LPO>
@@ -944,7 +945,9 @@
 #ifndef PXR_GW_GPAD
 #define PXR_GW_GPAD 4
 #endif
-struct GramWaveLds {
+constexpr int GW_OFFD = 96;
+template <bool WIDE> struct GramWaveLds;
+template <> struct GramWaveLds<true> {
   double G[GW_SLOTS][IG_GDOUBLES + PXR_GW_GPAD];
   double D[GW_SLOTS][16];
   double obs[GW_SLOTS][IG_OBS];
@@ -952,6 +955,32 @@
   double refbuf[128];
   InnerOwner own[IP_MAXPTS];
 };
+template <> struct GramWaveLds<false> {
+  double G[GW_SLOTS][GW_OFFD + PXR_GW_GPAD];
+  double land[IG_GDOUBLES + 16];
+  double obs[GW_SLOTS][IG_OBS];
+  double res[GW_SLOTS][10];
+  InnerOwner own[IP_MAXPTS];
+};
+constexpr int GW_WAVES_PER_CU = 8;
+static_assert(sizeof(GramWaveLds<false>) * GW_WAVES_PER_CU <= 160 * 1024, "eight wavefronts per CU: 20 KB of LDS each");
+static_assert(sizeof(double) * GW_SLOTS * 10 >= sizeof(double) * 128, "the reference descriptor of a build lies on res");
+__device__ __forceinline__ constexpr int gram_offd_index(int b) { return b - 1 - (b >= 4 ? 1 : 0) - (b >= 7 ? 1 : 0); }
+
+template <int C>
+__device__ __forceinline__ double ref_self_dot(const double* __restrict__ refs, int64_t p, int lane) {
+  double r2 = 0.0;
+  if (refs)
+    for (int ch = lane; ch < C; ch += 64) { const double d = refs[(size_t)p * C + ch]; r2 = fma(d, d, r2); }
+  return rows_sum<16>(row16_sum(r2));
+}
+template <int C>
+__global__ __launch_bounds__(256) void k_ref_r2_table(int64_t n_points, const double* __restrict__ refs, double* __restrict__ r2) {
+  const int64_t p = (int64_t)blockIdx.x * 4 + (threadIdx.x >> 6);
+  if (p >= n_points) return;
+  const double v = ref_self_dot<C>(refs, p, threadIdx.x & 63);
+  if ((threadIdx.x & 63) == 0) r2[p] = v;
+}
 
 __global__ __launch_bounds__(256) void k_gram_wave_table(int64_t n_waves, const GramWave* __restrict__ waves, const int64_t* __restrict__ pt_ptr,
                                                          const int64_t* __restrict__ pt_obs, const int32_t* __restrict__ obs_image,
@@ -1010,10 +1039,10 @@
   if (miss) a.gram_cell[sl.obs] = make_int2(row, col);
 }
 
-template <typename ST, int C>
+template <typename ST, int C, bool WIDE>
 __global__ __launch_bounds__(64) __attribute__((amdgpu_waves_per_eu(2, 2))) void k_inner_gram_packed(const InnerArgs a, const char* __restrict__ table) {
   static_assert(C == 128 || C == 64, "feature patches");
-  __shared__ __align__(16) GramWaveLds lds;
+  __shared__ __align__(16) GramWaveLds<WIDE> lds;
   const int lane = threadIdx.x, sidx = lane >> 2, sub = lane & 3;
   const char* const ent = table + (size_t)blockIdx.x * gram_wave_bytes();
   const GramWave* const gw = reinterpret_cast<const GramWave*>(ent);
@@ -1053,7 +1082,34 @@
                       GW_FETCH(Q0, 4, va4, vb4) GW_FETCH(Q0, 5, va5, vb5) GW_FETCH(Q0, 6, va6, vb6) GW_FETCH(Q0, 7, va7, vb7)
 #define GW_PUT8(Q0) GW_PUT(Q0, 0, va0, vb0) GW_PUT(Q0, 1, va1, vb1) GW_PUT(Q0, 2, va2, vb2) GW_PUT(Q0, 3, va3, vb3) \
                     GW_PUT(Q0, 4, va4, vb4) GW_PUT(Q0, 5, va5, vb5) GW_PUT(Q0, 6, va6, vb6) GW_PUT(Q0, 7, va7, vb7)
-  if (warm) { GW_FETCH8(0) }
+  const int offd_piece = lane < 24 ? 8 + lane : (lane < 40 ? 16 + lane : (lane < 48 ? 24 + lane : 71));
+#define GW_FETCH_OFFD(Q0, J, VA)                                                                                      \
+  {                                                                                                                   \
+    const int64_t oi = __shfl((int)sl.obs, 4 * min(Q0 + J, L - 1));                                                   \
+    VA = reinterpret_cast<const double2*>(a.gram_G + (size_t)oi * (IG_GDOUBLES + 16))[offd_piece];                     \
+  }
+#define GW_PUT_OFFD(Q0, J, VA) \
+  if (Q0 + J < L && lane < GW_OFFD / 2) reinterpret_cast<double2*>(lds.G[Q0 + J])[lane] = VA;
+#define GW_FETCH8_OFFD(Q0) GW_FETCH_OFFD(Q0, 0, va0) GW_FETCH_OFFD(Q0, 1, va1) GW_FETCH_OFFD(Q0, 2, va2) GW_FETCH_OFFD(Q0, 3, va3) \
+                           GW_FETCH_OFFD(Q0, 4, va4) GW_FETCH_OFFD(Q0, 5, va5) GW_FETCH_OFFD(Q0, 6, va6) GW_FETCH_OFFD(Q0, 7, va7)
+#define GW_PUT8_OFFD(Q0) GW_PUT_OFFD(Q0, 0, va0) GW_PUT_OFFD(Q0, 1, va1) GW_PUT_OFFD(Q0, 2, va2) GW_PUT_OFFD(Q0, 3, va3) \
+                         GW_PUT_OFFD(Q0, 4, va4) GW_PUT_OFFD(Q0, 5, va5) GW_PUT_OFFD(Q0, 6, va6) GW_PUT_OFFD(Q0, 7, va7)
+  double dg[16], dD[4];
+#pragma unroll
+  for (int m = 0; m < 16; ++m) dg[m] = 0.0;
+  dD[0] = dD[1] = dD[2] = dD[3] = 0.0;
+  if constexpr (WIDE) {
+    if (warm) { GW_FETCH8(0) }
+  } else if (warm) {
+    GW_FETCH8_OFFD(0)
+    if (valid) {
+      const double2* g = reinterpret_cast<const double2*>(a.gram_G + (size_t)sl.obs * (IG_GDOUBLES + 16));
+#pragma unroll
+      for (int m = 0; m < 8; ++m) { const double2 t2 = g[gram_block(sub, sub) * 8 + m]; dg[2 * m] = t2.x; dg[2 * m + 1] = t2.y; }
+      const double2 d01 = g[IG_GDOUBLES / 2 + 2 * sub], d23 = g[IG_GDOUBLES / 2 + 2 * sub + 1];
+      dD[0] = d01.x; dD[1] = d01.y; dD[2] = d23.x; dD[3] = d23.y;
+    }
+  }
   if (valid) {
     double* ob = lds.obs[q];
     const int img = sl.img, cam = sl.cam;
@@ -1080,12 +1136,13 @@
       ob[30] = (double)cc.x; ob[31] = (double)cc.y;
     }
   }
-  for (int j = 0; j < npts; ++j) {
-    double r2 = 0.0;
-    if (a.v.d_refs)
-      for (int ch = lane; ch < C; ch += 64) { const double d = a.v.d_refs[(size_t)gw->p[j] * C + ch]; r2 = fma(d, d, r2); }
-    r2 = rows_sum<16>(row16_sum(r2));
-    if (lane == 0) lds.own[j].r2 = r2;
+  if (a.ref_r2) {
+    if (owner) lds.own[lane].r2 = a.ref_r2[myp];
+  } else {
+    for (int j = 0; j < npts; ++j) {
+      const double r2 = ref_self_dot<C>(a.v.d_refs, gw->p[j], lane);
+      if (lane == 0) lds.own[j].r2 = r2;
+    }
   }
   if (owner) {
     InnerOwner& S = lds.own[lane];
@@ -1093,10 +1150,19 @@
     for (int m = 0; m < 3; ++m) { S.X[m] = a.v.d_xyz[3 * myp + m]; S.Xc[m] = S.X[m]; }
     S.live = 1; S.radius = 1e4; S.decrease_factor = 2.0; S.invalid = 0; S.it = 0; S.reuse_diag = 0; S.mcc = 0.0;
   }
-  if (warm) {
-    GW_PUT8(0)
-    if (L > 8) { GW_FETCH8(8) GW_PUT8(8) }
-  }
+  if constexpr (WIDE) {
+    if (warm) {
+      GW_PUT8(0)
+      if (L > 8) { GW_FETCH8(8) GW_PUT8(8) }
+    }
+  } else if (warm) {
+    GW_PUT8_OFFD(0)
+    if (L > 8) { GW_FETCH8_OFFD(8) GW_PUT8_OFFD(8) }
+  }
+#undef GW_FETCH_OFFD
+#undef GW_PUT_OFFD
+#undef GW_FETCH8_OFFD
+#undef GW_PUT8_OFFD
 #undef GW_FETCH
 #undef GW_PUT
 #undef GW_FETCH8
@@ -1106,7 +1172,8 @@
     __syncthreads();
     const bool act = valid && lds.own[jq].live != 0;
     double* ob = lds.obs[valid ? q : L - 1];
-    double PX[2][3], u = 0.0, v = 0.0, rf = 0.0, cf = 0.0, sx = 1.0, sy = 1.0;
+    double PX[2][3], fu = 0.0, fv = 0.0, sx = 1.0, sy = 1.0;
+    bool outside = false;
     int row = 0, col = 0;
     if (act) {
       double R[9];
@@ -1128,9 +1195,11 @@
 #pragma unroll
         for (int m = 0; m < 3; ++m) PX[r][m] = A0 * R[m] + A1 * R[3 + m] + A2 * R[6 + m];
       }
-      u = x * sx - 0.5 - cx; v = y * sy - 0.5 - cy;
-      rf = floor(v); cf = floor(u);
+      const double u = x * sx - 0.5 - cx, v = y * sy - 0.5 - cy;
+      const double rf = floor(v), cf = floor(u);
       row = texel_index(rf, a.H); col = texel_index(cf, a.W);
+      fu = u - cf; fv = v - rf;
+      outside = a.check_bounds && !a.v.d_refs && !(u > 0.0 && u < (double)a.W && v > 0.0 && v < (double)a.H);
     }
     const bool need = act && ((double)row != ob[30] || (double)col != ob[31]);
     unsigned long long todo = __ballot(need);
@@ -1139,7 +1208,8 @@
       const int pi_lo = (int)(pi & 0xffffffffll), pi_hi = (int)(pi >> 32);
       const int pt_of_slot = gw->p[jq];
       const unsigned long long rebuilt = todo;
-      double2 rr0 = make_double2(0.0, 0.0), rr1 = rr0, rr2 = rr0;
+      double2 rr0 = make_double2(0.0, 0.0), rr1 = rr0;
+      [[maybe_unused]] double2 rr2 = rr0;
       auto take = [&](GramTexels<ST, C>& tx, double2& rr) -> int {
         if (todo == 0ull) return -1;
         const int src = __ffsll((long long)todo) - 1;
@@ -1152,24 +1222,61 @@
         return src;
       };
       auto build = [&](const GramTexels<ST, C>& tx, const double2& rr, int src) {
-        __syncthreads();
-        if (2 * lane < C) *reinterpret_cast<double2*>(&lds.refbuf[2 * lane]) = rr;
-        __syncthreads();
-        gram_contract<ST, C>(tx, lds.refbuf, lds.G[src >> 2], lds.D[src >> 2]);
+        if constexpr (WIDE) {
+          __syncthreads();
+          if (2 * lane < C) *reinterpret_cast<double2*>(&lds.refbuf[2 * lane]) = rr;
+          __syncthreads();
+          gram_contract<ST, C>(tx, lds.refbuf, lds.G[src >> 2], lds.D[src >> 2]);
+        } else {
+          double* const refbuf = &lds.res[0][0];
+          __syncthreads();
+          if (2 * lane < C) *reinterpret_cast<double2*>(&refbuf[2 * lane]) = rr;
+          __syncthreads();
+          gram_contract<ST, C>(tx, refbuf, lds.land, lds.land + IG_GDOUBLES);
+          __syncthreads();
+          const int slot = src >> 2;
+          const double2* ld = reinterpret_cast<const double2*>(lds.land);
+          if (lane < GW_OFFD / 2) reinterpret_cast<double2*>(lds.G[slot])[lane] = ld[offd_piece];
+          if (sidx == slot) {
+#pragma unroll
+            for (int m = 0; m < 8; ++m) { const double2 t2 = ld[gram_block(sub, sub) * 8 + m]; dg[2 * m] = t2.x; dg[2 * m + 1] = t2.y; }
+            const double2 d01 = ld[IG_GDOUBLES / 2 + 2 * sub], d23 = ld[IG_GDOUBLES / 2 + 2 * sub + 1];
+            dD[0] = d01.x; dD[1] = d01.y; dD[2] = d23.x; dD[3] = d23.y;
+          }
+          if (a.gram_G) {
+            const int64_t oi = slots[slot].obs;
+            double2* g = reinterpret_cast<double2*>(a.gram_G + (size_t)oi * (IG_GDOUBLES + 16));
+            g[lane] = ld[lane];
+            if (lane < 24) g[64 + lane] = ld[64 + lane];
+            const int2 cl = make_int2(__builtin_amdgcn_readlane(row, src), __builtin_amdgcn_readlane(col, src));
+            if (lane == 0) a.gram_cell[oi] = cl;
+          }
+        }
       };
-      GramTexels<ST, C> t0, t1, t2;
-      int s0 = take(t0, rr0), s1 = take(t1, rr1), s2 = take(t2, rr2);
-      while (true) {
-        if (s0 < 0) break;
-        build(t0, rr0, s0); s0 = take(t0, rr0);
-        if (s1 < 0) break;
-        build(t1, rr1, s1); s1 = take(t1, rr1);
-        if (s2 < 0) break;
-        build(t2, rr2, s2); s2 = take(t2, rr2);
+      if constexpr (WIDE) {
+        GramTexels<ST, C> t0, t1, t2;
+        int s0 = take(t0, rr0), s1 = take(t1, rr1), s2 = take(t2, rr2);
+        while (true) {
+          if (s0 < 0) break;
+          build(t0, rr0, s0); s0 = take(t0, rr0);
+          if (s1 < 0) break;
+          build(t1, rr1, s1); s1 = take(t1, rr1);
+          if (s2 < 0) break;
+          build(t2, rr2, s2); s2 = take(t2, rr2);
+        }
+      } else {
+        GramTexels<ST, C> t0, t1;
+        int s0 = take(t0, rr0), s1 = take(t1, rr1);
+        while (true) {
+          if (s0 < 0) break;
+          build(t0, rr0, s0); s0 = take(t0, rr0);
+          if (s1 < 0) break;
+          build(t1, rr1, s1); s1 = take(t1, rr1);
+        }
       }
       if (need && sub == 0) { ob[30] = (double)row; ob[31] = (double)col; }
       __syncthreads();
-      if (a.gram_G) {
+      if (WIDE && a.gram_G) {
         unsigned long long wb = rebuilt;
         while (wb != 0ull) {
           const int src = __ffsll((long long)wb) - 1;
@@ -1177,10 +1284,12 @@
           const int slot = src >> 2;
           const int64_t oi = slots[slot].obs;
           double2* g = reinterpret_cast<double2*>(a.gram_G + (size_t)oi * (IG_GDOUBLES + 16));
-          const double2* Gd = reinterpret_cast<const double2*>(lds.G[slot]);
-          g[lane] = Gd[lane];
-          if (lane < 16) g[64 + lane] = Gd[64 + lane];
-          else if (lane < 24) g[64 + lane] = reinterpret_cast<const double2*>(lds.D[slot])[lane - 16];
+          if constexpr (WIDE) {
+            const double2* Gd = reinterpret_cast<const double2*>(lds.G[slot]);
+            g[lane] = Gd[lane];
+            if (lane < 16) g[64 + lane] = Gd[64 + lane];
+            else if (lane < 24) g[64 + lane] = reinterpret_cast<const double2*>(lds.D[slot])[lane - 16];
+          }
           const int2 cl = make_int2(__builtin_amdgcn_readlane(row, src), __builtin_amdgcn_readlane(col, src));
           if (lane == 0) a.gram_cell[oi] = cl;
         }
@@ -1188,19 +1297,13 @@
     }
     if (act) {
       double wu[4], dwu[4], wv[4], dwv[4];
-      catmull_rom_weights(u - cf, wu, dwu);
-      catmull_rom_weights(v - rf, wv, dwv);
+      catmull_rom_weights(fu, wu, dwu);
+      catmull_rom_weights(fv, wv, dwv);
       const int R = sub;
       const double wvR = pick4(wv, R), dwvR = pick4(dwv, R);
       double Sgg = 0, Sgc = 0, Sgr = 0, Scc = 0, Scr = 0, Srr = 0;
       const double* Gq = lds.G[q];
-#pragma unroll
-      for (int cb = 0; cb < 4; ++cb) {
-        const bool T = cb < R;
-        const double* blk = Gq + (T ? gram_block(cb, R) : gram_block(R, cb)) * 16;
-        double e[16];
-#pragma unroll
-        for (int m = 0; m < 8; ++m) { const double2 t2 = *reinterpret_cast<const double2*>(blk + 2 * m); e[2 * m] = t2.x; e[2 * m + 1] = t2.y; }
+      auto block_forms = [&](const double (&e)[16], const bool T, double (&Bq)[4]) {
         double zw[4], zd[4];
 #pragma unroll
         for (int c = 0; c < 4; ++c) {
@@ -1211,19 +1314,57 @@
         const double Bwd_s = fma(zw[3], dwu[3], fma(zw[2], dwu[2], fma(zw[1], dwu[1], zw[0] * dwu[0])));
         const double Bdw_s = fma(zd[3], wu[3], fma(zd[2], wu[2], fma(zd[1], wu[1], zd[0] * wu[0])));
         const double Bdd = fma(zd[3], dwu[3], fma(zd[2], dwu[2], fma(zd[1], dwu[1], zd[0] * dwu[0])));
-        const double Bwd = T ? Bdw_s : Bwd_s, Bdw = T ? Bwd_s : Bdw_s;
+        Bq[0] = Bww; Bq[1] = T ? Bdw_s : Bwd_s; Bq[2] = T ? Bwd_s : Bdw_s; Bq[3] = Bdd;
+      };
+      auto accumulate = [&](const int cb, const double (&Bq)[4]) {
         const double wvC = wv[cb], dwvC = dwv[cb];
-        Sgg = fma(wvR * wvC, Bww, Sgg);
-        Sgc = fma(wvR * wvC, Bwd, Sgc);
-        Sgr = fma(wvR * dwvC, Bww, Sgr);
-        Scc = fma(wvR * wvC, Bdd, Scc);
-        Scr = fma(wvR * dwvC, Bdw, Scr);
-        Srr = fma(dwvR * dwvC, Bww, Srr);
-      }
-      const double* Dq = lds.D[q] + 4 * R;
-      const double2 d01 = *reinterpret_cast<const double2*>(Dq), d23 = *reinterpret_cast<const double2*>(Dq + 2);
-      const double dw = fma(wu[3], d23.y, fma(wu[2], d23.x, fma(wu[1], d01.y, wu[0] * d01.x)));
-      const double dd = fma(dwu[3], d23.y, fma(dwu[2], d23.x, fma(dwu[1], d01.y, dwu[0] * d01.x)));
+        Sgg = fma(wvR * wvC, Bq[0], Sgg);
+        Sgc = fma(wvR * wvC, Bq[1], Sgc);
+        Sgr = fma(wvR * dwvC, Bq[0], Sgr);
+        Scc = fma(wvR * wvC, Bq[3], Scc);
+        Scr = fma(wvR * dwvC, Bq[2], Scr);
+        Srr = fma(dwvR * dwvC, Bq[0], Srr);
+      };
+      double dw, dd;
+      if constexpr (WIDE) {
+#pragma unroll
+        for (int cb = 0; cb < 4; ++cb) {
+          const bool T = cb < R;
+          const double* blk = Gq + (T ? gram_block(cb, R) : gram_block(R, cb)) * 16;
+          double e[16], Bq[4];
+#pragma unroll
+          for (int m = 0; m < 8; ++m) { const double2 t2 = *reinterpret_cast<const double2*>(blk + 2 * m); e[2 * m] = t2.x; e[2 * m + 1] = t2.y; }
+          block_forms(e, T, Bq);
+          accumulate(cb, Bq);
+        }
+        const double* Dq = lds.D[q] + 4 * R;
+        const double2 d01 = *reinterpret_cast<const double2*>(Dq), d23 = *reinterpret_cast<const double2*>(Dq + 2);
+        dw = fma(wu[3], d23.y, fma(wu[2], d23.x, fma(wu[1], d01.y, wu[0] * d01.x)));
+        dd = fma(dwu[3], d23.y, fma(dwu[2], d23.x, fma(dwu[1], d01.y, dwu[0] * d01.x)));
+      } else {
+        double Bd[4], Bo[3][4];
+        block_forms(dg, false, Bd);
+#pragma unroll
+        for (int k = 0; k < 3; ++k) {
+          const int cb = k + (k >= R ? 1 : 0);
+          const bool T = cb < R;
+          const double* blk = Gq + gram_offd_index(T ? gram_block(cb, R) : gram_block(R, cb)) * 16;
+          double e[16];
+#pragma unroll
+          for (int m = 0; m < 8; ++m) { const double2 t2 = *reinterpret_cast<const double2*>(blk + 2 * m); e[2 * m] = t2.x; e[2 * m + 1] = t2.y; }
+          block_forms(e, T, Bo[k]);
+        }
+#pragma unroll
+        for (int cb = 0; cb < 4; ++cb) {
+          const int k = cb - (cb > R ? 1 : 0);
+          double Bq[4];
+#pragma unroll
+          for (int m = 0; m < 4; ++m) Bq[m] = cb == R ? Bd[m] : (k == 0 ? Bo[0][m] : (k == 1 ? Bo[1][m] : Bo[2][m]));
+          accumulate(cb, Bq);
+        }
+        dw = fma(wu[3], dD[3], fma(wu[2], dD[2], fma(wu[1], dD[1], wu[0] * dD[0])));
+        dd = fma(dwu[3], dD[3], fma(dwu[2], dD[2], fma(dwu[1], dD[1], dwu[0] * dD[0])));
+      }
       double Sfd = wvR * dw, Scd = wvR * dd, Srd = dwvR * dw;
       Sgg = quad_sum(Sgg); Sgc = quad_sum(Sgc); Sgr = quad_sum(Sgr);
       Scc = quad_sum(Scc); Scr = quad_sum(Scr); Srr = quad_sum(Srr);
@@ -1242,7 +1383,8 @@
       double rho[3];
       inner_loss(a.loss.type, a.loss.a, s, rho);
       double cq = 0.5 * rho[0];
-      if (a.check_bounds && !a.v.d_refs && !(u > 0.0 && u < (double)a.W && v > 0.0 && v < (double)a.H)) cq = __builtin_nan("");
+      if (outside) cq = __builtin_nan("");
+      if constexpr (!WIDE) { sx = ob[24]; sy = ob[25]; }
       gcc *= sx * sx; gcr *= sx * sy; grr *= sy * sy; bc *= sx; br *= sy;
       double kappa = 0.0;
       if (s != 0.0 && rho[2] > 0.0) {
@@ -1304,6 +1446,8 @@
   a.pt_ptr = d_pt_ptr; a.pt_obs = d_pt_obs; a.pt_var = d_pt_var;
   a.xyz_out = const_cast<double*>(view->d_xyz); a.cost_before = d_cost_before; a.cost_pt = d_cost_per_point;
   a.gram_G = gram ? gram->G : nullptr; a.gram_cell = gram ? static_cast<int2*>(gram->cell) : nullptr; a.gram_warm = gram_warm ? 1 : 0;
+  const bool gram_wide = getenv("PXR_INNER_GRAM_WIDE") != nullptr;
+  a.ref_r2 = lists && !getenv("PXR_INNER_NO_R2_TABLE") ? lists->d_ref_r2 : nullptr;
   const int ppb = arena->C >= 64 ? 1 : 8;
   const int threads = 64;
   const unsigned blocks = (unsigned)((view->n_points + ppb - 1) / ppb);
@@ -1328,8 +1472,11 @@
 #define INNER_GRAM(ST, CC, NBLK, MAXO)                                                                                    \
   hipLaunchKernelGGL((k_inner_gram<ST, CC>), dim3(NBLK), dim3(64), sizeof(double) * gram_lds_doubles(MAXO, CC), ctx->stream, a, \
                      static_cast<const char*>(lists->d_slots), MAXO)
-#define INNER_GRAM_PACKED(ST, CC, NBLK) \
-  hipLaunchKernelGGL((k_inner_gram_packed<ST, CC>), dim3(NBLK), dim3(64), 0, ctx->stream, a, static_cast<const char*>(lists->d_waves))
+#define INNER_GRAM_PACKED(ST, CC, NBLK)                                                                                                              \
+  do {                                                                                                                                                \
+    if (gram_wide) hipLaunchKernelGGL((k_inner_gram_packed<ST, CC, true>), dim3(NBLK), dim3(64), 0, ctx->stream, a, static_cast<const char*>(lists->d_waves));  \
+    else hipLaunchKernelGGL((k_inner_gram_packed<ST, CC, false>), dim3(NBLK), dim3(64), 0, ctx->stream, a, static_cast<const char*>(lists->d_waves));        \
+  } while (0)
   if (arena->C <= 4) {
     if (arena->dtype == PXR_F16 && arena->C == 3) INNER_LAUNCH(k_inner_points, _Float16, 3);
     else if (arena->dtype == PXR_F16) INNER_LAUNCH(k_inner_points, _Float16, 1);
@@ -1378,7 +1525,7 @@
 
 size_t inner_wave_stage_bytes(int64_t n_pts) { return sizeof(GramWave) * (size_t)(n_pts + 1); }
 int make_inner_lists(pxr_ctx* ctx, const int64_t* pt_ptr, int64_t n, void* h_wave_stage, size_t wave_stage_bytes, const pxr_ba_view* view,
-                     const int64_t* d_pt_ptr, const int64_t* d_pt_obs, InnerLists* out) {
+                     int channels, const int64_t* d_pt_ptr, const int64_t* d_pt_obs, InnerLists* out) {
   hipStream_t st = ctx->stream;
   const bool one_point_kernel = getenv("PXR_INNER_GRAM1") != nullptr;
   std::vector<GramPoint> shorts;
@@ -1409,7 +1556,7 @@
   }
   flush();
   const GramWave* const waves = wv ? wv : waves_pageable.data();
-  out->n_waves = n_wv; out->d_waves = nullptr; out->d_wave_heads = nullptr;
+  out->n_waves = n_wv; out->d_waves = nullptr; out->d_wave_heads = nullptr; out->d_ref_r2 = nullptr;
   out->n_short = n_short; out->n_long = (int64_t)longs.size(); out->maxo_short = maxo;
   out->d_short = nullptr; out->d_long = nullptr; out->d_slots = nullptr;
   if (!shorts.empty()) {
@@ -1425,9 +1572,17 @@
   }
   if (n_wv > 0) {
     const size_t heads = (sizeof(GramWave) * (size_t)n_wv + 255) & ~(size_t)255;
-    char* d_all = static_cast<char*>(solve_scratch(heads + gram_wave_bytes() * (size_t)n_wv, &out->own_heads));
+    const size_t tab = (gram_wave_bytes() * (size_t)n_wv + 255) & ~(size_t)255;
+    const bool with_r2 = view->d_refs != nullptr && (channels == 128 || channels == 64);
+    char* d_all = static_cast<char*>(solve_scratch(heads + tab + (with_r2 ? sizeof(double) * (size_t)n : 0), &out->own_heads));
     if (!d_all) return set_error(PXR_ENOMEM, "hipMalloc(inner wave table)");
     out->d_wave_heads = d_all; out->d_waves = d_all + heads;
+    if (with_r2) {
+      out->d_ref_r2 = reinterpret_cast<double*>(d_all + heads + tab);
+      const unsigned nb = (unsigned)((n + 3) / 4);
+      if (channels == 128) hipLaunchKernelGGL(k_ref_r2_table<128>, dim3(nb), dim3(256), 0, st, n, view->d_refs, out->d_ref_r2);
+      else hipLaunchKernelGGL(k_ref_r2_table<64>, dim3(nb), dim3(256), 0, st, n, view->d_refs, out->d_ref_r2);
+    }
     if (int rc = hip_check(hipMemcpyAsync(d_all, waves, sizeof(GramWave) * (size_t)n_wv, hipMemcpyHostToDevice, st), "H2D")) return rc;
     const int64_t n_thr2 = n_wv * (GW_SLOTS + 1);
     hipLaunchKernelGGL(k_gram_wave_table, dim3((unsigned)((n_thr2 + 255) / 256)), dim3(256), 0, st, n_wv,
@@ -1446,7 +1601,24 @@
   if (l->d_long && l->own_long) (void)hipFree(l->d_long);
   if (l->d_slots && l->own_slots) (void)hipFree(l->d_slots);
   if (l->d_wave_heads && l->own_heads) (void)hipFree(l->d_wave_heads);
-  l->d_short = nullptr; l->d_long = nullptr; l->d_slots = nullptr; l->d_waves = nullptr; l->d_wave_heads = nullptr;
-}
-
-}
+  l->d_short = nullptr; l->d_long = nullptr; l->d_slots = nullptr; l->d_waves = nullptr; l->d_wave_heads = nullptr; l->d_ref_r2 = nullptr;
+}
+
+}
+
+extern "C" int pxr_inner_gram_occupancy(int dtype, int channels, int wide_layout, int* workgroups_per_cu, int* lds_bytes) {
+  using namespace pxr;
+  PXR_REQUIRE(workgroups_per_cu && lds_bytes, "pxr_inner_gram_occupancy: NULL argument");
+  PXR_REQUIRE((dtype == PXR_F16 || dtype == PXR_F32) && (channels == 128 || channels == 64),
+              "pxr_inner_gram_occupancy: fp16 / fp32 storage, 128 / 64 channels");
+  const void* fn;
+#define OCC_PICK(ST, CC) fn = wide_layout ? reinterpret_cast<const void*>(k_inner_gram_packed<ST, CC, true>) : reinterpret_cast<const void*>(k_inner_gram_packed<ST, CC, false>)
+  if (dtype == PXR_F16 && channels == 128) OCC_PICK(_Float16, 128);
+  else if (dtype == PXR_F16) OCC_PICK(_Float16, 64);
+  else if (channels == 128) OCC_PICK(float, 128);
+  else OCC_PICK(float, 64);
+#undef OCC_PICK
+  PXR_HIP(hipOccupancyMaxActiveBlocksPerMultiprocessor(workgroups_per_cu, fn, 64, 0));
+  *lds_bytes = (int)(wide_layout ? sizeof(GramWaveLds<true>) : sizeof(GramWaveLds<false>));
+  return PXR_OK;
+}
diff --git a/pixel-perfect-sfm_amd/csrc/pxr_ba_solve.hip b/pixel-perfect-sfm_amd/csrc/pxr_ba_solve.hip
--- a/pixel-perfect-sfm_amd/csrc/pxr_ba_solve.hip
+++ b/pixel-perfect-sfm_amd/csrc/pxr_ba_solve.hip
@@ -961,8 +961,8 @@
                             const pxr_loss* loss, const int64_t* d_pt_ptr, const int64_t* d_pt_obs,
                             const int* d_pt_var, double* d_cost_before, const InnerLists* lists, double* d_cost_per_point,
                             const GramCache* gram, bool gram_warm);
-int make_inner_lists(pxr_ctx* ctx, const int64_t* h_pt_ptr, int64_t n_pts, void* h_wave_stage, size_t wave_stage_bytes, const pxr_ba_view* view, const int64_t* d_pt_ptr, const int64_t* d_pt_obs,
-                     InnerLists* out);
+int make_inner_lists(pxr_ctx* ctx, const int64_t* h_pt_ptr, int64_t n_pts, void* h_wave_stage, size_t wave_stage_bytes, const pxr_ba_view* view, int channels, const int64_t* d_pt_ptr,
+                     const int64_t* d_pt_obs, InnerLists* out);
 void free_inner_lists(InnerLists* l);
 
 static inline unsigned nblk(int64_t n, int b = 256) { return (unsigned)((n + b - 1) / b); }
@@ -1471,7 +1471,7 @@
       PXR_HIP(hipStreamSynchronize(st));
       h_pt_ptr = stage;
     }
-    RC(make_inner_lists(ctx, h_pt_ptr, n_pts, wave_stage, wave_stage ? wave_bytes : 0, view, d_pt_ptr.p, d_pt_obs.p, &inner_lists.l));
+    RC(make_inner_lists(ctx, h_pt_ptr, n_pts, wave_stage, wave_stage ? wave_bytes : 0, view, arena->C, d_pt_ptr.p, d_pt_obs.p, &inner_lists.l));
   }
   setup_mark("inner-iteration tables");
   const auto t_loop0 = std::chrono::steady_clock::now();
diff --git a/pixel-perfect-sfm_amd/csrc/pxr_internal.h b/pixel-perfect-sfm_amd/csrc/pxr_internal.h
--- a/pixel-perfect-sfm_amd/csrc/pxr_internal.h
+++ b/pixel-perfect-sfm_amd/csrc/pxr_internal.h
@@ -75,6 +75,7 @@
   void* d_slots = nullptr;
   void* d_waves = nullptr; int64_t n_waves = 0;
   void* d_wave_heads = nullptr;
+  double* d_ref_r2 = nullptr;
   bool own_short = true, own_long = true, own_slots = true, own_heads = true;
 };
 void* solve_scratch(size_t bytes, bool* owned);
diff --git a/pixel-perfect-sfm_amd/pixsfm_amd/_lib.py b/pixel-perfect-sfm_amd/pixsfm_amd/_lib.py
--- a/pixel-perfect-sfm_amd/pixsfm_amd/_lib.py
+++ b/pixel-perfect-sfm_amd/pixsfm_amd/_lib.py
@@ -114,6 +114,7 @@
                               C.c_void_p, C.c_void_p, C.c_void_p, C.c_void_p]),
     "pxr_ba_eval_gram": (C.c_int, [C.c_void_p, C.c_void_p, C.POINTER(BaView), C.POINTER(InterpCfg), C.c_int, C.c_void_p,
                                    C.POINTER(C.c_int32)]),
+    "pxr_inner_gram_occupancy": (C.c_int, [C.c_int, C.c_int, C.c_int, C.POINTER(C.c_int), C.POINTER(C.c_int)]),
     "pxr_ba_projection_jacobian": (C.c_int, [C.c_void_p, C.POINTER(BaView), C.c_void_p]),
     "pxr_ba_solve": (C.c_int, [C.c_void_p, C.c_void_p, C.POINTER(BaView), C.POINTER(InterpCfg), C.POINTER(Loss),
                                C.c_void_p, C.c_void_p, C.c_void_p, C.c_void_p, C.POINTER(LMOptions),
```

Result: no change. 1.435 billion residual_blocks/s (median of 2 runs) (+0.2%).
